# Ray0089/geometric-aware-dense-matching

Hardware: AMD Instinct MI355X
Metric: rgbd_crops_per_sec_geomatch_fwd (higher is better)
Workload: dtype bf16x3/f32acc

## Files before the change

### geometric_aware_dense_matching_amd/_lib.py

```python
import ctypes
import os
import subprocess

_PKG = os.path.dirname(os.path.abspath(__file__))
LIB_PATH = os.path.join(_PKG, "libgdm_hip.so")
CSRC = os.path.join(_PKG, "csrc")

_vp = ctypes.c_void_p
_i = ctypes.c_int
_f = ctypes.c_float
_sz = ctypes.c_size_t

GDM_RANSAC_MAX_H = 4096


class KnnJob(ctypes.Structure):
    _fields_ = [("support", _vp), ("query", _vp), ("idx", _vp), ("d2", _vp),
                ("support_bstride", ctypes.c_int64), ("query_bstride", ctypes.c_int64),
                ("S", ctypes.c_int32), ("Q", ctypes.c_int32), ("K", ctypes.c_int32), ("grid_w", ctypes.c_int32)]


class PwSeg(ctypes.Structure):
    _fields_ = [("x", _vp), ("idx", _vp), ("C", ctypes.c_int32), ("n_src", ctypes.c_int32)]


class PwJob(ctypes.Structure):
    _fields_ = [("x", _vp), ("wt", _vp), ("out", _vp), ("n", ctypes.c_int32)]


class CopyJob(ctypes.Structure):
    _fields_ = [("dst", _vp), ("src", _vp), ("sb", ctypes.c_int64), ("s1", ctypes.c_int64), ("s2", ctypes.c_int64),
                ("B", ctypes.c_int32), ("R1", ctypes.c_int32), ("R2", ctypes.c_int32), ("E", ctypes.c_int32)]


SIGNATURES = {
    "gdm_last_error": (ctypes.c_char_p, []),
    "gdm_version": (_i, []),
    "gdm_knn_batch": (None, [_vp, _sz, _sz, _sz, _vp, _sz, _sz, _vp]),
    "gdm_knn_batch_hip": (_i, [_vp, _vp, _i, _i, _i, _i, _vp, _vp, _vp]),
    "gdm_knn_jobs_workspace_bytes": (_sz, [ctypes.POINTER(KnnJob), _i, _i]),
    "gdm_knn_jobs_ws_hip": (_i, [ctypes.POINTER(KnnJob), _i, _i, _vp, _sz, _vp]),
    "gdm_ballquery_hip": (_i, [_i, _i, _i, _f, _i, _vp, _vp, _vp, _vp]),
    "gdm_furthestsampling_hip": (_i, [_i, _i, _i, _vp, _vp, _vp, _vp]),
    "gdm_interpolation_forward_hip": (_i, [_i, _i, _i, _i, _vp, _vp, _vp, _vp, _vp]),
    "gdm_interpolation_backward_hip": (_i, [_i, _i, _i, _i, _vp, _vp, _vp, _vp, _vp]),
    "gdm_labelstat_ballrange_hip": (_i, [_i, _i, _i, _f, _i, _vp, _vp, _vp, _vp, _vp]),
    "gdm_labelstat_idx_hip": (_i, [_i, _i, _i, _i, _i, _vp, _vp, _vp, _vp]),
    "gdm_group_gather_hip": (_i, [_vp, _vp, _i, _i, _i, _i, _i, _vp, _vp]),
    "gdm_group_gather_bwd2_hip": (_i, [_vp, ctypes.c_long, _vp, _i, _i, _i, _i, _i, _vp, _vp]),
    "gdm_gather_max_hip": (_i, [_vp, _vp, _i, _i, _i, _i, _i, _vp, _vp, _vp]),
    "gdm_gather_max_bwd_hip": (_i, [_vp, _vp, _i, _i, _i, _i, _vp, _vp]),
    "gdm_rel_pos_enc_hip": (_i, [_vp, _vp, _i, _i, _i, _vp, _vp]),
    "gdm_att_pool_hip": (_i, [_vp, _vp, _i, _i, _i, _i, _vp, _vp]),
    "gdm_att_pool_bwd_hip": (_i, [_vp, _vp, _vp, _i, _i, _i, _i, _vp, _vp, _vp]),
    "gdm_match_workspace_bytes": (_sz, [_i, _i, _i]),
    "gdm_match_hip": (_i, [_vp, _vp, _i, _i, _i, _i, _i, _vp, _vp, _vp, _vp, _sz, _vp]),
    "gdm_match_rows_bytes": (_sz, [_i]),
    "gdm_match_partial_bytes": (_sz, [_i, _i]),
    "gdm_match_pack_hip": (_i, [_vp, _i, _i, _i, _i, _vp, _vp]),
    "gdm_match_pack2_hip": (_i, [_vp, _i, _i, _vp, _vp, _i, _i, _vp, _i, _i, _vp]),
    "gdm_match_packed_hip": (_i, [_vp, _vp, _i, _i, _i, _vp, _vp, _vp, _vp, _sz, _vp]),
    "gdm_seg_mask_hip": (_i, [_vp, _i, _i, _vp, _vp, _vp]),
    "gdm_spline_aggregate_hip": (_i, [_vp, _vp, _vp, _vp, _vp, _vp, _i, _i, _i, _i, _vp, _vp]),
    "gdm_spline_aggregate_bwd_hip": (_i, [_vp, _vp, _vp, _vp, _i, _i, _i, _vp, _vp]),
    "gdm_spline_direct3_hip": (_i, [_vp, _vp, _vp, _vp, _vp, _vp, _vp, _i, _i, _i, _i, _i, _vp, _vp, _vp, _vp]),
    "gdm_gemm_grouped_hip": (_i, [_vp, _vp, _vp, _vp, _i, _i, _i, _i, _vp, _vp]),
    "gdm_spline_pairs_aggregate3_hip": (_i, [_vp, _vp, _vp, _vp, _vp, _vp, _i, _i, _i, _vp, _vp, _vp, _vp]),
    "gdm_upsample_bilinear_hip": (_i, [_vp, ctypes.c_long, _i, _i, _i, _i, _vp, _vp]),
    "gdm_upsample_bilinear_bwd_hip": (_i, [_vp, ctypes.c_long, _i, _i, _i, _i, _vp, _vp]),
    "gdm_topk_rows_hip": (_i, [_vp, ctypes.c_long, _i, _i, _vp, _vp, _vp]),
    "gdm_topk_negdist_hip": (_i, [_vp, _vp, _i, _i, _i, _vp, _vp]),
    "gdm_edge_feature_hip": (_i, [_vp, _vp, _i, _i, _i, _i, _vp, _vp]),
    "gdm_edge_feature_bwd_hip": (_i, [_vp, _vp, _i, _i, _i, _i, _vp, _vp]),
    "gdm_circle_rows_fwd_hip": (_i, [_vp, _i, _i, _vp, _vp, _vp, _vp, _f, _f, _f, _vp, _vp, _vp, _vp]),
    "gdm_circle_rows_bwd_hip": (_i, [_vp, _i, _i, _vp, _vp, _vp, _vp, _f, _f, _f, _vp, _vp, _vp, _vp, _vp]),
    "gdm_circle_match_rows_bytes": (_sz, [_i]),
    "gdm_circle_match_tp_bytes": (_sz, [_i]),
    "gdm_circle_match_pack_hip": (_i, [_vp, _i, _vp, _vp, _vp, _vp]),
    "gdm_circle_match_nbr_hip": (_i, [_vp, _i, _f, _vp, _vp]),
    "gdm_circle_match_visbits_hip": (_i, [_vp, _i, _i, _vp, _vp]),
    "gdm_circle_match_nbr_items_hip": (_i, [_vp, _i, _vp, _i, _vp, _vp]),
    "gdm_circle_match_fwd2_hip": (_i, [_vp, _vp, _vp, _vp, _vp, _i, _i, _vp, _vp, _vp, _vp, _i, _vp, _i, _f, _f, _vp, _vp, _vp, _vp]),
    "gdm_circle_match_bwd2_hip": (_i, [_vp, _vp, _vp, _vp, _vp, _i, _i, _vp, _vp, _vp, _vp, _i, _vp, _i, _f, _f, _vp, _vp, _vp, _vp, _vp, _vp]),
    "gdm_circle_match_bwd_parts": (_i, [_i, _i]),
    "gdm_lfa_stage_hip": (_i, [_vp] * 13 + [_i, _i, _i, _i, _i, _f, _vp, _vp]),
    "gdm_kabsch_stats_hip": (_i, [_vp, ctypes.c_long, _i, _i, _vp, _vp, _vp, _i, _i, _i, _vp, _vp]),
    "gdm_kabsch_solve_hip": (_i, [_vp, _i, _i, _vp, _vp, _vp]),
    "gdm_ransac_workspace_bytes": (_sz, [_i, _i, _i]),
    "gdm_ransac_pose_hip": (_i, [_vp, ctypes.c_long, _i, _i, _vp, _vp, _vp, _vp, _i, _i, _i, _i, _f, ctypes.c_double, ctypes.c_uint32, _i,
                                 _vp, _sz, _vp, _vp, _vp, _vp, _vp]),
    "gdm_icp_transform_hip": (_i, [_vp, ctypes.c_long, _i, _i, _vp, _i, _i, _vp, _vp]),
    "gdm_icp_update_hip": (_i, [_vp, ctypes.c_long, _i, _i, _vp, _vp, _vp, _vp, _i, _i, _i, _f, ctypes.c_double, _i, _vp, _vp, _vp, _vp,
                                _vp]),
    "gdm_targets_workspace_bytes": (_sz, [_i, _i, _i]),
    "gdm_hpr_visible_hip": (_i, [_vp, ctypes.c_long, _vp, _vp, _i, _i, _vp, _sz, _vp, _vp, _vp]),
    "gdm_pose_targets_hip": (_i, [_vp, ctypes.c_long, _i, _i, _vp, _vp, _vp, ctypes.c_long, _vp, _i, _i, _i, ctypes.c_double, _vp, _sz,
                                  _vp, _vp, _vp, _vp, _vp]),
    "gdm_affine_act_maxk_hip": (_i, [_vp, _vp, _vp, ctypes.c_long, _i, ctypes.c_long, _i, _i, _f, _vp, _vp]),
    "gdm_prelu1_hip": (_i, [_vp, _vp, ctypes.c_long, _vp, _vp]),
    "gdm_prelu1_bwd_hip": (_i, [_vp, _vp, _vp, ctypes.c_long, _vp, _vp, _vp]),
    "gdm_affine_act_hip": (_i, [_vp, _vp, _vp, _vp, _vp, _vp, ctypes.c_long, _i, ctypes.c_long, _i, _f, _vp, _vp]),
    "gdm_upconv3x3_gather_hip": (_i, [_vp, _vp, _vp, _i, _i, _i, _i, _i, _i, _i, _f, _vp, _vp]),
    "gdm_upconv3x3_gather2_hip": (_i, [_vp, _vp, _vp, _i, _i, _i, _i, _i, _i, _i, _f, _vp, _vp, _vp]),
    "gdm_upconv3x3_gather_bwd_hip": (_i, [_vp, _i, _i, _i, _i, _i, _i, _vp, _vp]),
    "gdm_upconv_fused64_weight_bytes": (_sz, []),
    "gdm_upconv_fused64_pack_weight_hip": (_i, [_vp, _vp, _vp]),
    "gdm_upconv_fused64_hip": (_i, [_vp, _vp, _vp, _vp, _i, _i, _i, _i, _i, _i, _i, _f, _vp, _vp]),
    "gdm_psp_combine2_hip": (_i, [_vp, _vp, _i, _vp, _i, _vp, _i, _vp, _i, _vp, _i, _i, _i, _i, _vp, _vp, _vp]),
    "gdm_gather_add_affine_act2_hip": (_i, [_vp, _vp, _vp, _vp, _vp, _i, _i, _i, _i, _i, _f, _vp, _vp, _i, _vp]),
    "gdm_conv1x1_gather_add_act2_hip": (_i, [_vp, _vp, _vp, _vp, _vp, _vp, _i, _i, _i, ctypes.c_long, _i, _f, _i, _vp, _vp]),
    "gdm_conv64_gather_add_act_mfma2_hip": (_i, [_vp, _vp, _vp, _vp, _vp, _vp, _i, _i, ctypes.c_long, _i, _f, _i, _i, _vp, _vp, _i, _vp]),
    "gdm_conv3x3_act_bytes": (_sz, [_i, _i, _i, _i]),
    "gdm_conv3x3_weight_bytes": (_sz, [_i, _i]),
    "gdm_conv3x3_pack_weight_hip": (_i, [_vp, _i, _i, _vp, _vp]),
    "gdm_conv3x3_pack_act_hip": (_i, [_vp, _i, _i, _i, _i, _vp, _vp]),
    "gdm_conv3x3_packed_hip": (_i, [_vp, _vp, _vp, _vp, _vp, _i, _i, _i, _i, _i, _i, _vp, _vp]),
    "gdm_conv3x3_strided_hip": (_i, [_vp, _vp, _vp, _vp, _vp, _i, _i, _i, _i, _i, _i, _i, _vp, _vp, _vp]),
    "gdm_conv1x1_strided_hip": (_i, [_vp, _vp, _vp, _vp, _i, _i, _i, _i, _i, _i, _i, _vp, _vp]),
    "gdm_affine_relu_maxpool_hip": (_i, [_vp, _vp, _vp, _i, _i, _i, _i, _vp, _vp]),
    "gdm_conv1x1_logsoftmax_hip": (_i, [_vp, _vp, _vp, _i, _i, ctypes.c_long, _vp, _vp]),
    "gdm_pack_rows64_hip": (_i, [_vp, _i, _vp, _vp]),
    "gdm_upconv_final_points_hip": (_i, [_vp, _vp, _vp, _vp, _vp, _i, _f, _vp, _vp, _i, _i, _i, _i, _i, _i, _vp, _vp]),
    "gdm_psp_pools_hip": (_i, [_vp, ctypes.c_long, _i, _i, _vp, _vp, _vp, _vp, _vp]),
    "gdm_psp_pools_bwd_hip": (_i, [_vp, _vp, _vp, _vp, ctypes.c_long, _i, _i, _vp, _vp]),
    "gdm_conv1x1_weight_bytes": (_sz, [_i, _i]),
    "gdm_conv1x1_pack_weight_hip": (_i, [_vp, _i, _i, _vp, _vp]),
    "gdm_conv_pack_weight_dgrad_hip": (_i, [_vp, _i, _i, _i, _vp, _vp]),
    "gdm_conv1x1_packed_hip": (_i, [_vp, _vp, _vp, _vp, _i, _i, _i, _i, _i, _i, _i, _vp, _vp]),
    "gdm_depth_to_xyz_hip": (_i, [_vp, _vp, _vp, _i, _i, _i, _i, _vp, _vp]),
    "gdm_bn_sums_len": (ctypes.c_long, [_i, _i, ctypes.c_long]),
    "gdm_bn_stats_hip": (_i, [_vp, _i, _i, ctypes.c_long, _vp, _vp]),
    "gdm_bn_fwd_apply_hip": (_i, [_vp, _vp, _i, _vp, _vp, _i, _i, ctypes.c_long, _f, _f, _i, _f, _vp, _vp, _vp, _vp, _vp]),
    "gdm_bn_bwd_reduce_hip": (_i, [_vp, _vp, _vp, _i, _i, ctypes.c_long, _i, _f, _vp, _vp]),
    "gdm_bn_bwd_apply_hip": (_i, [_vp, _vp, _vp, _i, _vp, _vp, _i, _i, ctypes.c_long, _i, _f, _vp, _vp, _vp, _vp]),
    "gdm_point_heads2_hip": (_i, [_vp, _vp, _i, _vp, _vp, _i, _i, _i, _i, _vp, _vp, _vp, _vp, _i, _i, _vp, _vp, _i, _vp, _vp, _vp]),
    "gdm_pointwise2_hip": (_i, [ctypes.POINTER(PwSeg), _i, _vp, _i, _vp, _vp, _i, _i, _i, _i, _f, _vp, _i, _i, _i, _vp]),
    "gdm_pointwise_jobs_hip": (_i, [ctypes.POINTER(PwJob), _i, _i, _i, _i, _vp]),
    "gdm_pointwise_chain2_hip": (_i, [_vp, _vp, _vp, _vp, _i, _f, _vp, _vp, _vp, _i, _f, _i, _i, _i, _i, _i, _vp, _vp, _vp]),
    "gdm_stem_weight_bytes": (_sz, []),
    "gdm_stem_pack_weight_hip": (_i, [_vp, _vp, _vp]),
    "gdm_stem_hip": (_i, [_vp, _vp, _vp, _vp, _i, _i, _i, _vp, _vp, _vp]),
    "gdm_wgrad_x_bytes": (_sz, [_i, _i, _i, _i]),
    "gdm_wgrad_go_bytes": (_sz, [_i, _i, _i, _i]),
    "gdm_wgrad_pack_x_hip": (_i, [_vp, _i, _i, _i, _i, _vp, _vp]),
    "gdm_wgrad_pack_go_hip": (_i, [_vp, _i, _i, _i, _i, _vp, _vp]),
    "gdm_wgrad_x1_bytes": (_sz, [_i, _i, _i]),
    "gdm_wgrad_pack_x1_hip": (_i, [_vp, _i, _i, _i, _vp, _vp]),
    "gdm_mfma_probe_hip": (_i, [_i, _i, _i, _vp, _vp]),
    "gdm_mfma_probe_lds_hip": (_i, [_i, _i, _i, _vp, _vp]),
    "gdm_wgrad_direct_hip": (_i, [_vp, ctypes.c_long, _vp, ctypes.c_long, _i, _i, _i, _i, _i, _vp, _vp, _vp]),
    "gdm_conv1x1_packed_wb_hip": (_i, [_vp, _vp, ctypes.c_long, _i, _i, _i, _i, _i, _vp, _vp]),
    "gdm_copy_jobs_hip": (_i, [ctypes.POINTER(CopyJob), _i, _vp]),
}

_lib = None


def _objects_state():
    st = {}
    for f in sorted(os.listdir(CSRC)):
        if f.endswith(".o"):
            st[f] = os.stat(os.path.join(CSRC, f)).st_mtime_ns
    return st


def build(verbose=False):
    import hashlib
    import json
    import time
    before = _objects_state()
    out = None if verbose else subprocess.DEVNULL
    t0 = time.time()
    subprocess.check_call(["make", "-C", CSRC, "-j4"], stdout=out)
    after = _objects_state()
    rebuilt = sorted(f for f, m in after.items() if before.get(f) != m)
    with open(LIB_PATH, "rb") as f:
        digest = hashlib.sha256(f.read()).hexdigest()[:16]
    rec = {"mode": "hipcc --offload-arch=gfx950 via csrc/Makefile (in-tree, ahead of time)", "recompiled": rebuilt,
           "up_to_date": sorted(set(after) - set(rebuilt)), "lib": os.path.basename(LIB_PATH), "lib_bytes": os.path.getsize(LIB_PATH),
           "lib_sha256_16": digest, "seconds": round(time.time() - t0, 1), "when": time.strftime("%Y-%m-%dT%H:%M:%S")}
    try:
        with open(os.path.join(CSRC, "build_record.json"), "w") as f:
            json.dump(rec, f, indent=1)
    except OSError:
        pass
    print("[gdm build] recompiled %d of %d translation units%s; %s %d bytes sha256 %s" %
          (len(rebuilt), len(after), (": " + " ".join(rebuilt)) if rebuilt else "", rec["lib"], rec["lib_bytes"], digest))
    return LIB_PATH


def build_record():
    import hashlib
    import json
    rec = {}
    try:
        with open(os.path.join(CSRC, "build_record.json")) as f:
            rec = json.load(f)
    except (OSError, ValueError):
        rec = {"mode": "prebuilt library (no build record travelled)"}
    try:
        with open(LIB_PATH, "rb") as f:
            rec["loaded_lib_sha256_16"] = hashlib.sha256(f.read()).hexdigest()[:16]
    except OSError:
        rec["loaded_lib_sha256_16"] = None
    rec.pop("up_to_date", None)
    if rec.get("lib_sha256_16") is not None:
        rec["record_matches_loaded_lib"] = rec["lib_sha256_16"] == rec["loaded_lib_sha256_16"]
    return rec


def lib():
    global _lib
    if _lib is None:
        if not os.path.exists(LIB_PATH):
            raise RuntimeError(
                "libgdm_hip.so is not built (%s). Run `python -c 'import __graft_entry__ as g; g.build()'` "
                "or `make -C geometric_aware_dense_matching_amd/csrc`. There is no CPU fallback." % LIB_PATH)
        import torch
        l = ctypes.CDLL(LIB_PATH)
        for name, (res, args) in SIGNATURES.items():
            fn = getattr(l, name)
            fn.restype = res
            fn.argtypes = args
        _lib = l
    return _lib


class GdmError(RuntimeError):
    pass


def check(rc, what):
    if rc != 0:
        msg = lib().gdm_last_error()
        raise GdmError("%s failed (rc=%d): %s" % (what, rc, msg.decode() if msg else "?"))
```

### geometric_aware_dense_matching_amd/cnn.py

```python
import math
import os

import torch
import torch.nn as nn
import torch.nn.functional as F

from . import ops, settings
from .layers import act_code, cached_gemm_weight, folded_bn, fused_eval




def bn_act(bn, x, relu=None):
    if ops.bn_train_supported(x, bn):
        return ops.batch_norm_act_train(x, bn, ops.ACT_RELU if relu is not None else ops.ACT_NONE)
    y = bn(x)
    return relu(y) if relu is not None else y


def _conv3x3(cin, cout, stride=1, dilation=1):
    return nn.Conv2d(cin, cout, kernel_size=3, stride=stride, padding=dilation, dilation=dilation, bias=False)


class BasicBlock(nn.Module):
    def __init__(self, inplanes, planes, stride=1, downsample=None, dilation=1):
        super().__init__()
        self.conv1 = _conv3x3(inplanes, planes, stride=stride, dilation=dilation)
        self.bn1 = nn.BatchNorm2d(planes)
        self.relu = nn.ReLU(inplace=True)
        self.conv2 = _conv3x3(planes, planes, stride=1, dilation=dilation)
        self.bn2 = nn.BatchNorm2d(planes)
        self.downsample = downsample

    @staticmethod
    def _packed_weight(conv):
        w = conv.weight
        key = (w._version, w.data_ptr())
        cache = conv.__dict__.get("_gdm_wpk")
        if cache is None or cache[0] != key:
            cache = (key, ops.conv3x3_pack_weight(w))
            conv.__dict__["_gdm_wpk"] = cache
        return cache[1]

    @staticmethod
    def _train_conv(conv, x):
        if (settings.USE_MFMA_CONV_TRAIN and conv.bias is None and tuple(conv.stride) == (1, 1)
                and ops.conv3x3_supported(x, conv.weight, conv.stride, conv.padding, conv.dilation)):
            return ops.conv3x3_train(x, conv.weight)
        return conv(x)

    def _mfma_ok(self, x):
        if tuple(self.conv1.stride) != (1, 1) and not settings.USE_MFMA_STRIDED:
            return False
        return (settings.USE_MFMA_CONV and ops.conv3x3_supported(x, self.conv1.weight, self.conv1.stride, self.conv1.padding, self.conv1.dilation)
                and ops.conv3x3_supported(x, self.conv2.weight, self.conv2.stride, self.conv2.padding, self.conv2.dilation)
                and self.conv2.weight.shape[1] == self.conv1.weight.shape[0])

    def forward(self, x):
        if fused_eval(x, self) and self._mfma_ok(x):
            s1, b1 = folded_bn(self.bn1)
            planes = self.conv1.weight.shape[0]
            stride = self.conv1.stride[0]
            xin = getattr(x, "_gdm_packed", None)
            if xin is None or xin.shape != tuple(x.shape):
                xin = x
            dconv = self.downsample[0] if self.downsample is not None else None
            own_ds = (settings.USE_MFMA_STRIDED and dconv is not None and isinstance(dconv, nn.Conv2d) and dconv.kernel_size == (1, 1) and dconv.bias is None
                      and dconv.stride == self.conv1.stride and dconv.padding == (0, 0)
                      and ops.gemm_supported(dconv.in_channels, dconv.out_channels, 64))
            if own_ds and not isinstance(xin, ops.PackedAct):
                xin = ops.conv3x3_pack_act(x)
            chain = (x.shape[0] * (x.shape[2] // stride) * (x.shape[3] // stride)) % 256 == 0
            mid = ops.conv3x3_bf16x3(xin, self._packed_weight(self.conv1), planes, s1, b1, ops.ACT_RELU, out_f32=not chain, out_packed=chain,
                                     stride=stride)
            mid = mid[1] if chain else mid
            s2, b2 = folded_bn(self.bn2)
            if self.downsample is None:
                res = x
            else:
                sd, bd = folded_bn(self.downsample[1])
                if own_ds:
                    wd, _ = cached_gemm_weight(dconv, "ds", lambda: dconv.weight.reshape(dconv.out_channels, dconv.in_channels), (dconv.weight,))
                    res = ops.conv1x1_packed2d(xin, wd, dconv.out_channels, sd, bd, ops.ACT_NONE, stride=stride)
                else:
                    res = ops.affine_act(dconv(x), sd, bd, ops.ACT_NONE)
            if not chain:
                return ops.conv3x3_bf16x3(mid, self._packed_weight(self.conv2), planes, s2, b2, ops.ACT_RELU, res)
            out, opk = ops.conv3x3_bf16x3(mid, self._packed_weight(self.conv2), planes, s2, b2, ops.ACT_RELU, res, out_packed=True)
            out._gdm_packed = opk
            return out
        if fused_eval(x, self):
            s1, b1 = folded_bn(self.bn1)
            out = ops.affine_act(self.conv1(x), s1, b1, ops.ACT_RELU)
            s2, b2 = folded_bn(self.bn2)
            if self.downsample is None:
                return ops.affine_act(self.conv2(out), s2, b2, ops.ACT_RELU, res=x)
            sd, bd = folded_bn(self.downsample[1])
            return ops.affine_act(self.conv2(out), s2, b2, ops.ACT_RELU, res=self.downsample[0](x), res_scale=sd, res_shift=bd)
        out = bn_act(self.bn1, self._train_conv(self.conv1, x), self.relu)
        out = bn_act(self.bn2, self._train_conv(self.conv2, out))
        residual = x if self.downsample is None else bn_act(self.downsample[1], self.downsample[0](x))
        out = out + residual
        return self.relu(out)


class ResNet18Trunk(nn.Module):
    def __init__(self):
        super().__init__()
        self.inplanes = 64
        self.conv1 = nn.Conv2d(3, 64, kernel_size=7, stride=2, padding=3, bias=False)
        self.bn1 = nn.BatchNorm2d(64)
        self.relu = nn.ReLU(inplace=True)
        self.maxpool = nn.MaxPool2d(kernel_size=3, stride=2, padding=1)
        self.layer1 = self._make_layer(64, 2, stride=1)
        self.layer2 = self._make_layer(128, 2, stride=2)
        self.layer3 = self._make_layer(256, 2, stride=1)
        self.layer4 = self._make_layer(512, 2, stride=1)
        self.fc = nn.Linear(512, 1000)
        for m in self.modules():
            if isinstance(m, nn.Conv2d):
                n = m.kernel_size[0] * m.kernel_size[1] * m.out_channels
                m.weight.data.normal_(0, math.sqrt(2.0 / n))
            elif isinstance(m, nn.BatchNorm2d):
                m.weight.data.fill_(1)
                m.bias.data.zero_()

    def _make_layer(self, planes, blocks, stride):
        downsample = None
        if stride != 1 or self.inplanes != planes:
            downsample = nn.Sequential(nn.Conv2d(self.inplanes, planes, kernel_size=1, stride=stride, bias=False),
                                       nn.BatchNorm2d(planes))
        layers = [BasicBlock(self.inplanes, planes, stride, downsample)]
        self.inplanes = planes
        for _ in range(1, blocks):
            layers.append(BasicBlock(self.inplanes, planes))
        return nn.Sequential(*layers)


class PSPModule(nn.Module):
    def __init__(self, features, out_features=1024, sizes=(1, 2, 3, 6)):
        super().__init__()
        self.stages = nn.ModuleList([nn.Sequential(nn.AdaptiveAvgPool2d(output_size=(s, s)),
                                                   nn.Conv2d(features, features, kernel_size=1, bias=False))
                                     for s in sizes])
        self.bottleneck = nn.Conv2d(features * (len(sizes) + 1), out_features, kernel_size=1)
        self.relu = nn.ReLU()

    def _split_weights(self):
        w = self.bottleneck.weight
        vs = [st[1].weight for st in self.stages]
        key = tuple((t._version, t.data_ptr()) for t in [w] + vs)
        cache = self.__dict__.get("_gdm_split")
        if cache is None or cache[0] != key:
            with torch.no_grad():
                F_ = vs[0].shape[0]
                w2 = w.view(w.shape[0], -1)
                ms = [(w2[:, k * F_:(k + 1) * F_] @ v.view(F_, F_)).contiguous() for k, v in enumerate(vs)]
                wf = w2[:, len(vs) * F_:].contiguous()
            cache = (key, ms, wf)
            self.__dict__["_gdm_split"] = cache
        return cache[1], cache[2]

    def _split_weights_t(self, ms):
        cache = self.__dict__.get("_gdm_split_t")
        if cache is None or cache[0] is not ms:
            with torch.no_grad():
                cache = (ms, [m.t().contiguous() for m in ms])
            self.__dict__["_gdm_split_t"] = cache
        return cache[1]

    def forward(self, feats):
        h, w = feats.size(2), feats.size(3)
        if fused_eval(feats, self) and len(self.stages) == 4 and feats.shape[0] * self.bottleneck.out_channels <= 65535:
            ms, wf = self._split_weights()
            B, Cin = feats.shape[0], feats.shape[1]
            def full_res():
                if settings.USE_MFMA_GEMM and ops.gemm_supported(Cin, wf.shape[0], h * w):
                    wpk, co = cached_gemm_weight(self, "wf", wf, (self.bottleneck.weight,))
                    return ops.gemm_bf16x3_map(feats, wpk, co)
                return ops.wx(wf, feats.reshape(B, Cin, h * w)).view(B, -1, h, w)

            def priors():
                sizes = [st[0].output_size[0] if isinstance(st[0].output_size, (tuple, list)) else st[0].output_size for st in self.stages]
                pools = ops.psp_pools(feats) if sizes == [1, 2, 3, 6] and ops.psp_pools_supported(h, w) else None
                ys = []
                mts = self._split_weights_t(ms) if settings.USE_POINTWISE else None
                if mts is not None and pools is not None and settings.USE_PSP_JOBS and Cin >= 32:
                    outs = ops.pointwise_jobs([p.reshape(B, Cin, -1) for p in pools], mts)
                    return [o.view(B, -1, p.shape[2], p.shape[3]) for o, p in zip(outs, pools)]
                for k, (st, m) in enumerate(zip(self.stages, ms)):
                    p = pools[k] if pools is not None else st[0](feats)
                    s_ = p.shape[2]
                    if mts is not None:
                        ys.append(ops.pointwise([p.reshape(B, Cin, s_ * s_)], mts[k]).view(B, -1, s_, s_))
                    else:
                        ys.append(ops.wx(m, p.reshape(B, Cin, s_ * s_)).view(B, -1, s_, s_))
                return ys

            if settings.USE_SIDE_STREAMS and "psp" in settings.SIDE_PARTS and not torch.is_grad_enabled():
                with ops.fork(feats.device, 3) as f:
                    f.use(feats)
                    ys = priors()
                g = full_res()
                f.join(*ys)
            else:
                g = full_res()
                ys = priors()
            return ops.psp_combine(g, ys, self.bottleneck.bias, packed=settings.USE_MFMA_GEMM and settings.USE_PACKED_PRODUCERS)
        sizes = [st[0].output_size[0] if isinstance(st[0].output_size, (tuple, list)) else st[0].output_size for st in self.stages]
        if (settings.USE_SPLIT_PSP_TRAIN and feats.is_cuda and feats.dtype == torch.float32 and sizes == [1, 2, 3, 6] and ops.psp_pools_supported(h, w)
                and (h * w) % 4 == 0 and feats.shape[0] * self.bottleneck.out_channels <= 65535 and h <= 64 and w <= 64):
            B, F_ = feats.shape[0], feats.shape[1]
            w2 = self.bottleneck.weight.view(self.bottleneck.out_channels, -1)
            g = ops.wx(w2[:, 4 * F_:], feats.reshape(B, F_, h * w)).view(B, -1, h, w)
            pools = ops.psp_pools(feats)
            ys = []
            for k, st in enumerate(self.stages):
                m = w2[:, k * F_:(k + 1) * F_] @ st[1].weight.view(F_, F_)
                ys.append(ops.wx(m, pools[k].reshape(B, F_, sizes[k] * sizes[k])).view(B, -1, sizes[k], sizes[k]))
            return ops.psp_combine_train(g, ys, self.bottleneck.bias)
        priors = [ops.upsample_bilinear(stage(feats), (h, w)) for stage in self.stages] + [feats]
        return self.relu(self.bottleneck(torch.cat(priors, 1)))


class Upsample2x(nn.Module):

    def forward(self, x):
        return ops.upsample_bilinear(x, (x.shape[2] * 2, x.shape[3] * 2))


class PSPUpsample(nn.Module):
    def __init__(self, cin, cout):
        super().__init__()
        self.conv = nn.Sequential(Upsample2x(), nn.Conv2d(cin, cout, 3, padding=1), nn.BatchNorm2d(cout), nn.PReLU())

    def _tap_major_weight(self):
        w = self.conv[1].weight
        key = (w._version, w.data_ptr())
        cache = self.__dict__.get("_gdm_wt")
        if cache is None or cache[0] != key:
            with torch.no_grad():
                wt = w.permute(2, 3, 0, 1).reshape(9 * w.shape[0], w.shape[1]).contiguous()
            cache = (key, wt)
            self.__dict__["_gdm_wt"] = cache
        return cache[1]

    def forward(self, x):
        if fused_eval(x, self):
            code = act_code(self.conv[3])
            conv = self.conv[1]
            if code is not None and x.shape[0] * conv.out_channels <= 65535 and conv.in_channels >= settings.UPCONV_MIN_CIN:
                Bx, Cin, Hx, Wx = x.shape
                if settings.USE_FUSED_UPCONV and Cin == 64 and conv.out_channels == 64 and Hx >= 2 and Wx >= 2 and Bx <= 65535:
                    w = conv.weight
                    key = (w._version, w.data_ptr())
                    cache = self.__dict__.get("_gdm_fused64")
                    if cache is None or cache[0] != key:
                        cache = (key, ops.upconv_fused64_pack_weight(w))
                        self.__dict__["_gdm_fused64"] = cache
                    scale, shift = folded_bn(self.conv[2], conv.bias)
                    return ops.upconv_fused64(x, cache[1], scale, shift, (Hx * 2, Wx * 2), code[0], code[1])
                if settings.USE_MFMA_GEMM and ops.gemm_supported(Cin, 9 * conv.out_channels, Hx * Wx):
                    wpk, c9 = cached_gemm_weight(self, "tap", self._tap_major_weight, (conv.weight,))
                    z = ops.gemm_bf16x3_map(x, wpk, c9)
                else:
                    z = ops.wx(self._tap_major_weight(), x.reshape(Bx, Cin, Hx * Wx)).view(Bx, -1, Hx, Wx)
                scale, shift = folded_bn(self.conv[2], conv.bias)
                return ops.upconv3x3_gather(z, scale, shift, conv.out_channels, (x.shape[2] * 2, x.shape[3] * 2), code[0], code[1],
                                            packed=settings.USE_MFMA_GEMM and settings.USE_PACKED_PRODUCERS and conv.out_channels % 128 == 0)
        act = self.conv[3]
        if x.is_cuda and isinstance(act, nn.PReLU) and act.weight.numel() == 1 and x.dtype == torch.float32:
            conv = self.conv[1]
            if settings.USE_LOWRES_UPCONV_TRAIN and ops.upconv_train_supported(x.shape[0], conv.out_channels) and conv.in_channels >= settings.UPCONV_MIN_CIN:
                Bx, Cin, Hx, Wx = x.shape
                w9 = conv.weight.permute(2, 3, 0, 1).reshape(9 * conv.out_channels, Cin)
                z = ops.wx(w9, x.reshape(Bx, Cin, Hx * Wx)).view(Bx, -1, Hx, Wx)
                y = bn_act(self.conv[2], ops.upconv3x3_gather_train(z, conv.bias, conv.out_channels, (Hx * 2, Wx * 2)))
            else:
                y = bn_act(self.conv[2], conv(self.conv[0](x)))
            if y.numel() % 4 == 0:
                return ops.prelu1(y, act.weight)
            return act(y)
        return self.conv(x)


class FinalStage(nn.Sequential):

    def forward(self, x):
        conv = self[0]
        if fused_eval(x, self) and conv.in_channels == 64 and conv.out_channels == 64 and x.shape[0] <= 65535:
            return ops.conv1x1_logsoftmax(x, conv.weight, conv.bias)
        if self.training and ops.conv1x1_train_supported(conv, x):
            return self[1](ops.conv1x1_train(conv, x))
        return nn.Sequential.forward(self, x)


class PSPNet(nn.Module):

    def __init__(self):
        super().__init__()
        self.feats = ResNet18Trunk()
        self.psp = PSPModule(512, 1024, (1, 2, 3, 6))
        self.drop_1 = nn.Dropout2d(p=0.3)
        self.up_1 = PSPUpsample(1024, 256)
        self.up_2 = PSPUpsample(256, 64)
        self.up_3 = PSPUpsample(64, 64)
        self.drop_2 = nn.Dropout2d(p=0.15)
        self.final = FinalStage(nn.Conv2d(64, 64, kernel_size=1), nn.LogSoftmax(dim=1))
```

### geometric_aware_dense_matching_amd/csrc/gdm_conv.hip

```cpp
#include "gdm_common.h"
#include <math.h>
#include <stdlib.h>

namespace {

typedef __attribute__((ext_vector_type(16))) float f32x16;
typedef __attribute__((ext_vector_type(8))) __bf16 bf16x8;
typedef __attribute__((ext_vector_type(4))) unsigned u32x4;

constexpr int ROWB = 512;
constexpr int CV_PIX = 256;
constexpr int CV_CO = 128;
constexpr int CV_PANEL = CV_CO * ROWB;
#ifndef GDM_CONV_TAP_INNER
#define GDM_CONV_TAP_INNER 1
#endif
#ifndef GDM_CONV16_PF
#define GDM_CONV16_PF 2
#endif
#ifndef GDM_CONV_GLDS
#define GDM_CONV_GLDS 1
#endif

__device__ __forceinline__ void split8(const float* v, unsigned (&hi)[4], unsigned (&lo)[4])
{
#pragma unroll
    for (int j = 0; j < 4; ++j) gdm_split2(v[2 * j], v[2 * j + 1], hi[j], lo[j]);
}

__global__ __launch_bounds__(256) void conv_pack_act_kernel(const float* __restrict__ x, int C, int H, int W,
                                                            unsigned char* __restrict__ out)
{
    __shared__ float t[128][65];
    const int b = blockIdx.z, chunk = blockIdx.y;
    const int nchunk = (C + 127) / 128;
    const int cvalid = min(128, C - chunk * 128);
    const int hw = H * W;
    const long plane = (long)(H + 2) * (W + 2);
    const int p0 = blockIdx.x * 64;
    const int lane = threadIdx.x & 63, w = threadIdx.x >> 6;
    const int p = min(p0 + lane, hw - 1);
    const float* xb = x + ((long)b * C + chunk * 128) * hw;
    for (int c = w; c < cvalid; c += 4) t[c][lane] = xb[(long)c * hw + p];
    __syncthreads();
    const int pp = p0 + lane;
    if (pp >= hw) return;
    const int y = pp / W, xx = pp - y * W;
    unsigned char* o = out + (((long)(b * nchunk + chunk) * 32) * plane + (long)(y + 1) * (W + 2) + xx + 1) * 16;
    for (int q = w; q * 8 < cvalid; q += 4) {
        float v[8];
#pragma unroll
        for (int j = 0; j < 8; ++j) v[j] = t[q * 8 + j][lane];
        unsigned hi[4], lo[4];
        split8(v, hi, lo);
        *reinterpret_cast<uint4*>(o + (long)q * plane * 16) = make_uint4(hi[0], hi[1], hi[2], hi[3]);
        *reinterpret_cast<uint4*>(o + (long)(16 + q) * plane * 16) = make_uint4(lo[0], lo[1], lo[2], lo[3]);
    }
}

__global__ __launch_bounds__(256) void conv_pack_w_kernel(const float* __restrict__ w, int Cout, int Cin, int taps, unsigned char* __restrict__ out,
                                                          int dgrad = 0)
{
    const int nchunk = (Cin + 127) / 128;
    const int CoutP = (Cout + 127) & ~127;
    const long item = (long)blockIdx.x * 256 + threadIdx.x;
    const long rows = (long)taps * nchunk * CoutP;
    if (item >= rows * 16) return;
    const int ch = (int)(item & 15);
    const long row = item >> 4;
    const int co = (int)(row % CoutP);
    const int tc = (int)(row / CoutP);
    const int chunk = tc % nchunk, tap = tc / nchunk;
    float v[8];
#pragma unroll
    for (int j = 0; j < 8; ++j) {
        const int ci = chunk * 128 + ch * 8 + j;
        const bool in = co < Cout && ci < Cin;
        v[j] = !in ? 0.f : dgrad ? w[((long)ci * Cout + co) * taps + (taps - 1 - tap)] : w[((long)co * Cin + ci) * taps + tap];
    }
    unsigned hi[4], lo[4];
    split8(v, hi, lo);
    unsigned char* r = out + row * ROWB;
    *reinterpret_cast<uint4*>(r + ch * 16) = make_uint4(hi[0], hi[1], hi[2], hi[3]);
    *reinterpret_cast<uint4*>(r + 256 + ch * 16) = make_uint4(lo[0], lo[1], lo[2], lo[3]);
}

__device__ __forceinline__ int swz(int col, int ch) { return col * ROWB + (((ch & 16) | ((ch ^ col) & 15)) << 4); }

typedef __attribute__((ext_vector_type(4))) float f32x4;

#ifndef GDM_CONV_NPH
#define GDM_CONV_NPH 2
#endif
#ifndef GDM_CONV16_LATE
#define GDM_CONV16_LATE 1
#endif
#ifndef GDM_CONV_MFMA_ORDER
#define GDM_CONV_MFMA_ORDER 0
#endif
constexpr int MF_NPH = GDM_CONV_NPH;
constexpr int MF_WPIX = 16 * MF_NPH;
constexpr int MF_WAVES = CV_PIX / MF_WPIX;
constexpr int MF_THREADS = MF_WAVES * 64;
constexpr int MF_TSTRIDE = 132;
constexpr int MF_SMEM = 2 * CV_PANEL > CV_PIX * MF_TSTRIDE * 4 ? 2 * CV_PANEL : CV_PIX * MF_TSTRIDE * 4;

template <int ACT, bool HAS_RES, int TAPS = 9, bool PIXMAJOR = false, int NKS = 8, int NCB = 8, int WV = MF_WAVES>
__global__ __launch_bounds__(MF_THREADS) void conv_mfma16_kernel(const unsigned char* __restrict__ xpk, const unsigned char* __restrict__ wpk,
                                                                 const float* __restrict__ scale, const float* __restrict__ shift,
                                                                 const float* __restrict__ res, int B, int Cin, int Cout, int H, int W,
                                                                 float* __restrict__ out, const int32_t* __restrict__ rowidx = nullptr,
                                                                 const int32_t* __restrict__ tile_co0 = nullptr,
                                                                 unsigned char* __restrict__ outpk = nullptr, int stride = 1,
                                                                 long wbstride = 0)
{
    extern __shared__ __attribute__((aligned(16))) unsigned char smem[];
    constexpr int NS = NKS / 2;
    constexpr int UG = (NCB % 2 == 0) ? 2 : 3;
    constexpr int NPR = NCB / UG;
    constexpr int PANEL = NCB * 16 * ROWB;
    constexpr int TST = NCB * 16 + 4;
    static_assert(NCB == 8 || (NCB == 4 && !PIXMAJOR) || (NCB == 9 && !PIXMAJOR && WV == 8),
                  "64-channel tiles: NCHW / packed output only; 144-channel tiles: NCHW fp32 output only (no packed output: a tile straddles 128-channel chunks)");
    constexpr int NPH = MF_NPH;
    const int tid = threadIdx.x, lane = tid & 63;
    const int wave = __builtin_amdgcn_readfirstlane(tid >> 6);
    const int l16 = lane & 15, kg = lane >> 4;
    const int nchunk = (Cin + 127) / 128;
    const int npanel = TAPS * nchunk;
    const int hw = H * W;
    const long ptot = rowidx ? (long)B : (long)B * hw;
    const unsigned bx = blockIdx.x, by = blockIdx.y;
    const long pix0 = (long)bx * (WV * MF_WPIX) + wave * MF_WPIX;
    const int co0 = tile_co0 ? __builtin_amdgcn_readfirstlane(tile_co0[bx]) : by * (NCB * 16);
    const long pc = min(pix0, ptot - MF_WPIX);
    const int b = (int)(pc / hw);
    const int prem = (int)(pc - (long)b * hw);
    const int Wi = W * stride;
    const long plane = (long)(H * stride + 2) * (Wi + 2);
    const long oplane = (long)(H + 2) * (W + 2);
    const __amdgpu_buffer_rsrc_t xr = __builtin_amdgcn_make_buffer_rsrc(const_cast<unsigned char*>(xpk), (short)0, 0x7ffffff0, 0x00020000);
    int avoff[NPH];
#pragma unroll
    for (int ph = 0; ph < NPH; ++ph) {
        const int pr = prem + 16 * ph;
        const int yy = pr / W, xx = pr - yy * W;
        const long pixbase = rowidx ? (long)max(rowidx[pc + l16 + 16 * ph], 0) : (long)(yy * stride) * (Wi + 2) + (long)(xx + l16) * stride;
        avoff[ph] = (int)(((long)kg * plane + pixbase) * 16);
    }

    u32x4 ahi[NS][NPH], alo[NS][NPH];
    struct Pan { int chunk, ky, kx; };
    auto pan_next = [&](Pan p) -> Pan {
        if (TAPS == 1) { ++p.chunk; return p; }
        if (GDM_CONV_TAP_INNER) {
            if (++p.kx == 3) { p.kx = 0; if (++p.ky == 3) { p.ky = 0; ++p.chunk; } }
        } else {
            if (++p.chunk == nchunk) { p.chunk = 0; if (++p.kx == 3) { p.kx = 0; ++p.ky; } }
        }
        return p;
    };
    const int a_base = (int)(((long)(rowidx ? 0 : b) * nchunk * 32) * plane * 16);
    const int a_chunk = (int)(32 * plane * 16), a_rowb = (Wi + 2) * 16;
    auto pan_a = [&](Pan p) -> int { return a_base + p.chunk * a_chunk + p.ky * a_rowb + p.kx * 16; };
    const int sstride = (int)(4 * plane * 16);
    const int lostride = (int)(16 * plane * 16);
    auto load_a = [&](int r, int S) {
#pragma unroll
        for (int ph = 0; ph < NPH; ++ph) {
            ahi[S][ph] = __builtin_bit_cast(u32x4, __builtin_amdgcn_raw_buffer_load_b128(xr, avoff[ph], r + S * sstride, 0));
            alo[S][ph] = __builtin_bit_cast(u32x4, __builtin_amdgcn_raw_buffer_load_b128(xr, avoff[ph], r + S * sstride + lostride, 0));
        }
    };
    constexpr int THREADS = WV * 64, WGPIX = WV * MF_WPIX;
    constexpr int HS = (NCB * 512 / THREADS) / 2;
    u32x4 stage[HS];
    const __amdgpu_buffer_rsrc_t wr = __builtin_amdgcn_make_buffer_rsrc(const_cast<unsigned char*>(wpk), (short)0, 0x7ffffff0, 0x00020000);
    const int w_base = (wbstride ? (int)(((long)bx * WGPIX / hw) * wbstride) : 0) + co0 * ROWB;
    const int w_panel = ((Cout + 127) & ~127) * ROWB;
    auto pan_w = [&](Pan p) -> int { return w_base + ((TAPS == 1) ? p.chunk : (p.ky * 3 + p.kx) * nchunk + p.chunk) * w_panel; };
    auto stage_load = [&](int src, int half) {
#pragma unroll
        for (int i = 0; i < HS; ++i)
            stage[i] = __builtin_bit_cast(u32x4, __builtin_amdgcn_raw_buffer_load_b128(wr, tid * 16, src + (half * HS + i) * THREADS * 16, 0));
    };
    auto stage_store = [&](int buf, int half) {
        unsigned char* base = smem + buf * PANEL;
#pragma unroll
        for (int i = 0; i < HS; ++i) {
            const int g = (half * HS + i) * THREADS + tid;
            *reinterpret_cast<u32x4*>(base + swz(g >> 5, g & 31)) = stage[i];
        }
    };
    constexpr bool GLDS = GDM_CONV_GLDS && WV == 8;
    constexpr int NPIECE = PANEL / 1024 / 8;
    int glds_voff = 0;
    if (GLDS) {
        const int hrow = lane >> 5, sl = lane & 31;
        const int col15 = (2 * wave + hrow) & 15;
        glds_voff = wave * 1024 + hrow * 512 + (((sl & 16) | ((sl ^ col15) & 15)) << 4);
    }
    typedef __attribute__((address_space(3))) void* lds_void_ptr;
    auto stage_glds = [&](int src, int buf) {
#pragma unroll
        for (int i = 0; i < NPIECE; ++i)
            __builtin_amdgcn_raw_ptr_buffer_load_lds(wr, (lds_void_ptr)(smem + buf * PANEL + (i * 8 + wave) * 1024), 16, glds_voff, src + i * 8192, 0, 0);
    };

    f32x4 acc[NPH][NCB];
#pragma unroll
    for (int ph = 0; ph < NPH; ++ph)
#pragma unroll
        for (int cb = 0; cb < NCB; ++cb)
#pragma unroll
            for (int i = 0; i < 4; ++i) acc[ph][cb][i] = 0.f;

    constexpr int LATE = GDM_CONV16_LATE < NS ? GDM_CONV16_LATE : NS;
    Pan pcur = {0, (TAPS == 1) ? 1 : 0, (TAPS == 1) ? 1 : 0};
    if (GLDS) {
        stage_glds(pan_w(pcur), 0);
    } else {
        stage_load(pan_w(pcur), 0);
        stage_store(0, 0);
        stage_load(pan_w(pcur), 1);
        stage_store(0, 1);
    }
    int rcur = pan_a(pcur);
#pragma unroll
    for (int S = 0; S < NS - LATE; ++S) load_a(rcur, S);
    Pan pnxt = npanel > 1 ? pan_next(pcur) : pcur;
    int rnext = pan_a(pnxt), wnext = pan_w(pnxt);
    for (int it = 0; it < npanel; ++it) {
        __syncthreads();
        const bool more = it + 1 < npanel;
        const unsigned char* base = smem + (it & 1) * PANEL;
        constexpr int PF = GDM_CONV16_PF;
        constexpr int NU = NPR * NS;
        u32x4 fh[PF + 1][UG], fl[PF + 1][UG];
        auto frag_load = [&](int un) {
            const int S = un / NPR, pr = un % NPR, slot = un % (PF + 1);
#pragma unroll
            for (int j = 0; j < UG; ++j) {
                const int col = (UG * pr + j) * 16 + l16;
                fh[slot][j] = *reinterpret_cast<const u32x4*>(base + swz(col, 4 * S + kg));
                fl[slot][j] = *reinterpret_cast<const u32x4*>(base + swz(col, 16 + 4 * S + kg));
            }
        };
#pragma unroll
        for (int un = 0; un < PF; ++un) frag_load(un);
#pragma unroll
        for (int u = 0; u < NU; ++u) {
            const int S = u / NPR, pr = u % NPR, slot = u % (PF + 1);
            if (u + PF < NU) frag_load(u + PF);
#if GDM_CONV_MFMA_ORDER == 0
#pragma unroll
            for (int ph = 0; ph < NPH; ++ph) {
                const bf16x8 ah = __builtin_bit_cast(bf16x8, ahi[S][ph]);
                const bf16x8 al = __builtin_bit_cast(bf16x8, alo[S][ph]);
#pragma unroll
                for (int j = 0; j < UG; ++j) {
                    f32x4 c = acc[ph][UG * pr + j];
                    c = __builtin_amdgcn_mfma_f32_16x16x32_bf16(ah, __builtin_bit_cast(bf16x8, fl[slot][j]), c, 0, 0, 0);
                    c = __builtin_amdgcn_mfma_f32_16x16x32_bf16(al, __builtin_bit_cast(bf16x8, fh[slot][j]), c, 0, 0, 0);
                    c = __builtin_amdgcn_mfma_f32_16x16x32_bf16(ah, __builtin_bit_cast(bf16x8, fh[slot][j]), c, 0, 0, 0);
                    acc[ph][UG * pr + j] = c;
                }
            }
#else
#pragma unroll
            for (int prod = 0; prod < 3; ++prod)
#pragma unroll
                for (int ph = 0; ph < NPH; ++ph)
#pragma unroll
                    for (int j = 0; j < UG; ++j) {
                        const bf16x8 av = __builtin_bit_cast(bf16x8, prod == 1 ? alo[S][ph] : ahi[S][ph]);
                        const bf16x8 bv = __builtin_bit_cast(bf16x8, prod == 0 ? fl[slot][j] : fh[slot][j]);
                        acc[ph][UG * pr + j] = __builtin_amdgcn_mfma_f32_16x16x32_bf16(av, bv, acc[ph][UG * pr + j], 0, 0, 0);
                    }
#endif
            if (pr == NPR - 1 && S < NS - LATE) load_a(rnext, S);
            if (!GLDS && u == NU / 2 && more) {
                stage_store((it + 1) & 1, 0);
                stage_load(wnext, 1);
            }
            if (u == 0) {
                if (more) { if (GLDS) stage_glds(wnext, (it + 1) & 1); else stage_load(wnext, 0); }
#pragma unroll
                for (int S2 = NS - LATE; S2 < NS; ++S2) load_a(rcur, S2);
            }
#pragma unroll
            for (int i = 0; i < 3 * UG * NPH; ++i) {
                __builtin_amdgcn_sched_group_barrier(0x008, 1, 0);
                if (u + PF < NU && (i % NPH) == 0 && i < 2 * UG * NPH) __builtin_amdgcn_sched_group_barrier(0x100, 1, 0);
            }
            __builtin_amdgcn_sched_barrier(0);
        }
        if (!GLDS && more) stage_store((it + 1) & 1, 1);
        rcur = rnext;
        if (it + 2 < npanel) pnxt = pan_next(pnxt);
        rnext = pan_a(pnxt);
        wnext = pan_w(pnxt);
    }

    if (pix0 >= ptot) return;
    if (PIXMAJOR) {
#pragma unroll
        for (int cb = 0; cb < NCB; ++cb) {
            const int co = co0 + cb * 16 + l16;
            if (co >= Cout) continue;
            const float sc = scale ? scale[co] : 1.f, sh = shift ? shift[co] : 0.f;
            const int ocol = tile_co0 ? cb * 16 + l16 : co;
            const int ostride = tile_co0 ? CV_CO : Cout;
#pragma unroll
            for (int ph = 0; ph < NPH; ++ph)
#pragma unroll
                for (int r = 0; r < 4; ++r) {
                    float v = acc[ph][cb][r] * sc + sh;
                    if (ACT == 1) v = fmaxf(v, 0.f);
                    out[(pix0 + 16 * ph + 4 * kg + r) * ostride + ocol] = v;
                }
        }
        return;
    }
    float* tl = reinterpret_cast<float*>(smem) + wave * MF_WPIX * TST;
    if (outpk) __syncthreads();
#pragma unroll
    for (int cb = 0; cb < NCB; ++cb) {
        const int co = co0 + cb * 16 + l16;
        const bool live = co < Cout;
        const float sc = (live && scale) ? scale[co] : 1.f, sh = (live && shift) ? shift[co] : 0.f;
        float* op = out ? out + ((long)b * Cout + (live ? co : 0)) * hw + prem : nullptr;
        const float* rp = (HAS_RES && live) ? res + ((long)b * Cout + co) * hw + prem : nullptr;
#pragma unroll
        for (int ph = 0; ph < NPH; ++ph) {
            const int poff = 16 * ph + 4 * kg;
            float v[4];
#pragma unroll
            for (int j = 0; j < 4; ++j) v[j] = acc[ph][cb][j] * sc + sh;
            if (HAS_RES && live) {
                const float4 r4 = *reinterpret_cast<const float4*>(rp + poff);
                v[0] += r4.x; v[1] += r4.y; v[2] += r4.z; v[3] += r4.w;
            }
            if (ACT == 1) {
#pragma unroll
                for (int j = 0; j < 4; ++j) v[j] = fmaxf(v[j], 0.f);
            }
            if (op && live) *reinterpret_cast<float4*>(op + poff) = make_float4(v[0], v[1], v[2], v[3]);
            if (outpk) {
#pragma unroll
                for (int j = 0; j < 4; ++j) tl[(poff + j) * TST + cb * 16 + l16] = live ? v[j] : 0.f;
            }
        }
    }
    if (outpk) {
        __builtin_amdgcn_fence(__ATOMIC_ACQ_REL, "wavefront");
        const int lr = lane & 31, h = lane >> 5;
        const int ochunks = (Cout + 127) / 128;
        const int ochunk = co0 / 128;
#pragma unroll
        for (int half = 0; half < MF_WPIX / 32; ++half) {
            const int pp = prem + 32 * half + lr;
            const int yy = pp / W, xx = pp - yy * W;
            unsigned char* ob = outpk + (((long)(b * ochunks + ochunk) * 32) * oplane + (long)(yy + 1) * (W + 2) + xx + 1) * 16;
            const float* row = tl + (32 * half + lr) * TST;
#pragma unroll
            for (int it = 0; it < NCB; ++it) {
                const int ql = 2 * it + h;
                if (co0 + ql * 8 >= Cout) continue;
                const int q = (co0 % 128) / 8 + ql;
                const float4 a0 = *reinterpret_cast<const float4*>(row + ql * 8);
                const float4 a1 = *reinterpret_cast<const float4*>(row + ql * 8 + 4);
                const float v[8] = {a0.x, a0.y, a0.z, a0.w, a1.x, a1.y, a1.z, a1.w};
                unsigned hi[4], lo[4];
                split8(v, hi, lo);
                *reinterpret_cast<uint4*>(ob + (long)q * oplane * 16) = make_uint4(hi[0], hi[1], hi[2], hi[3]);
                *reinterpret_cast<uint4*>(ob + (long)(16 + q) * oplane * 16) = make_uint4(lo[0], lo[1], lo[2], lo[3]);
            }
        }
    }
}

#define CONV_KERNEL conv_mfma16_kernel
constexpr int CONV_THREADS = MF_THREADS, CONV_WPIX = MF_WPIX, CONV_SMEM = MF_SMEM;

}

namespace {
template <int CHAIN>
__global__ __launch_bounds__(512) void mfma_probe_kernel(int iters, float* __restrict__ sink)
{
    typedef __attribute__((ext_vector_type(8))) __bf16 pb_bf16x8;
    typedef __attribute__((ext_vector_type(4))) float pb_f32x4;
    const int lane = threadIdx.x & 63;
    pb_f32x4 acc[8];
#pragma unroll
    for (int i = 0; i < 8; ++i) acc[i] = pb_f32x4{0.f, 0.f, 0.f, 0.f};
    const unsigned seed = 0x3f803f80u + (unsigned)lane;
    u32x4 av = {seed, seed ^ 1u, seed ^ 2u, seed ^ 3u}, bv = {seed ^ 4u, seed ^ 5u, seed ^ 6u, seed ^ 7u};
    const pb_bf16x8 a = __builtin_bit_cast(pb_bf16x8, av), b = __builtin_bit_cast(pb_bf16x8, bv);
    for (int it = 0; it < iters; it += CHAIN) {
#pragma unroll
        for (int i = 0; i < 8; ++i)
#pragma unroll
            for (int c = 0; c < CHAIN; ++c) acc[i] = __builtin_amdgcn_mfma_f32_16x16x32_bf16(a, b, acc[i], 0, 0, 0);
    }
    float t = 0.f;
#pragma unroll
    for (int i = 0; i < 8; ++i) t += acc[i][0] + acc[i][1] + acc[i][2] + acc[i][3];
    if (t == 12345.678f) sink[0] = t;
}
template <int RPU>
__global__ __launch_bounds__(512) void mfma_probe_lds_kernel(int iters, float* __restrict__ sink)
{
    typedef __attribute__((ext_vector_type(8))) __bf16 pb_bf16x8;
    typedef __attribute__((ext_vector_type(4))) float pb_f32x4;
    extern __shared__ __attribute__((aligned(16))) unsigned char pl[];
    const int tid = threadIdx.x, lane = tid & 63;
    for (int i = tid; i < 4096; i += 512) reinterpret_cast<u32x4*>(pl)[i] = u32x4{0x3f803f80u, 0x3f803f80u, 0x3f803f80u, 0x3f803f80u + (unsigned)i};
    __syncthreads();
    pb_f32x4 acc[4];
#pragma unroll
    for (int i = 0; i < 4; ++i) acc[i] = pb_f32x4{0.f, 0.f, 0.f, 0.f};
    const unsigned seed = 0x3f803f80u + (unsigned)lane;
    u32x4 a0 = {seed, seed ^ 1u, seed ^ 2u, seed ^ 3u}, a1 = {seed ^ 4u, seed ^ 5u, seed ^ 6u, seed ^ 7u};
    u32x4 f[4] = {a0, a1, a0, a1};
    int off = lane * 16;
    for (int it = 0; it < iters; ++it) {
#pragma unroll
        for (int r = 0; r < RPU; ++r) f[r] = *reinterpret_cast<const u32x4*>(pl + ((off + r * 1024) & 0xffff));
        off += 4096;
#pragma unroll
        for (int prod = 0; prod < 3; ++prod)
#pragma unroll
            for (int i = 0; i < 4; ++i)
                acc[i] = __builtin_amdgcn_mfma_f32_16x16x32_bf16(__builtin_bit_cast(pb_bf16x8, prod == 1 ? a1 : a0),
                                                                 __builtin_bit_cast(pb_bf16x8, f[(i + prod) & 3]), acc[i], 0, 0, 0);
    }
    float t = 0.f;
#pragma unroll
    for (int i = 0; i < 4; ++i) t += acc[i][0] + acc[i][1] + acc[i][2] + acc[i][3];
    if (t == 12345.678f) sink[0] = t;
}
}

extern "C" int gdm_mfma_probe_lds_hip(int blocks, int iters, int rpu, float* sink, void* stream)
{
    GDM_CHECK_ARG(blocks >= 1 && blocks <= 65535 && iters >= 1 && (rpu == 1 || rpu == 2 || rpu == 4) && sink, "gdm_mfma_probe_lds_hip: bad arguments");
    if (rpu == 4) hipLaunchKernelGGL(mfma_probe_lds_kernel<4>, dim3(blocks), dim3(512), 65536, (hipStream_t)stream, iters, sink);
    else if (rpu == 2) hipLaunchKernelGGL(mfma_probe_lds_kernel<2>, dim3(blocks), dim3(512), 65536, (hipStream_t)stream, iters, sink);
    else hipLaunchKernelGGL(mfma_probe_lds_kernel<1>, dim3(blocks), dim3(512), 65536, (hipStream_t)stream, iters, sink);
    return gdm_launch_status("mfma_probe_lds_kernel");
}

extern "C" int gdm_mfma_probe_hip(int blocks, int iters, int chain, float* sink, void* stream)
{
    GDM_CHECK_ARG(blocks >= 1 && blocks <= 65535 && iters >= 3 && iters % 3 == 0 && (chain == 1 || chain == 3) && sink,
                  "gdm_mfma_probe_hip: bad arguments (iters a multiple of 3, chain 1 or 3)");
    if (chain == 3) hipLaunchKernelGGL(mfma_probe_kernel<3>, dim3(blocks), dim3(512), 0, (hipStream_t)stream, iters, sink);
    else hipLaunchKernelGGL(mfma_probe_kernel<1>, dim3(blocks), dim3(512), 0, (hipStream_t)stream, iters, sink);
    return gdm_launch_status("mfma_probe_kernel");
}

static bool cin_ok(int Cin) { return Cin == 64 || (Cin >= 128 && Cin % 128 == 0); }

static bool narrow_tiles(unsigned pixel_tiles, int Cout)
{
    return Cout <= 64 || (long)pixel_tiles * ((Cout + 127) / 128) < 256;
}

extern "C" size_t gdm_conv3x3_act_bytes(int B, int Cin, int H, int W)
{
    if (B < 1 || !cin_ok(Cin) || H < 1 || W < 1) return 0;
    return (size_t)B * (H + 2) * (W + 2) * ((Cin + 127) / 128) * ROWB;
}

extern "C" size_t gdm_conv3x3_weight_bytes(int Cout, int Cin)
{
    if (Cout < 1 || !cin_ok(Cin)) return 0;
    return (size_t)9 * ((Cin + 127) / 128) * ((Cout + 127) & ~127) * ROWB;
}

extern "C" size_t gdm_conv1x1_weight_bytes(int Cout, int Cin)
{
    if (Cout < 1 || !cin_ok(Cin)) return 0;
    return (size_t)((Cin + 127) / 128) * ((Cout + 127) & ~127) * ROWB;
}

static int pack_weight(const float* w, int Cout, int Cin, int taps, void* wpk, void* stream, const char* who, int dgrad = 0)
{
    GDM_CHECK_ARG(w && wpk, "%s: NULL pointer", who);
    GDM_CHECK_ARG(Cout >= 1 && cin_ok(Cin), "%s: Cout=%d Cin=%d (Cin a multiple of 128, or 64)", who, Cout, Cin);
    const long items = (long)taps * ((Cin + 127) / 128) * ((Cout + 127) & ~127) * 16;
    hipLaunchKernelGGL(conv_pack_w_kernel, dim3(gdm_cdiv(items, 256)), dim3(256), 0, (hipStream_t)stream, w, Cout, Cin, taps, (unsigned char*)wpk, dgrad);
    return gdm_launch_status("conv_pack_w_kernel");
}

extern "C" int gdm_conv_pack_weight_dgrad_hip(const float* w, int Cout, int Cin, int taps, void* wpk, void* stream)
{
    GDM_CHECK_ARG(taps == 9 || taps == 1, "gdm_conv_pack_weight_dgrad_hip: taps=%d (9 or 1)", taps);
    return pack_weight(w, Cin, Cout, taps, wpk, stream, "gdm_conv_pack_weight_dgrad_hip", 1);
}

extern "C" int gdm_conv3x3_pack_weight_hip(const float* w, int Cout, int Cin, void* wpk, void* stream)
{
    return pack_weight(w, Cout, Cin, 9, wpk, stream, "gdm_conv3x3_pack_weight_hip");
}

extern "C" int gdm_conv1x1_pack_weight_hip(const float* w, int Cout, int Cin, void* wpk, void* stream)
{
    return pack_weight(w, Cout, Cin, 1, wpk, stream, "gdm_conv1x1_pack_weight_hip");
}

extern "C" int gdm_conv3x3_pack_act_hip(const float* x, int B, int Cin, int H, int W, void* xpk, void* stream)
{
    GDM_CHECK_ARG(x && xpk, "gdm_conv3x3_pack_act_hip: NULL pointer");
    GDM_CHECK_ARG(B >= 1 && B <= 65535 && cin_ok(Cin) && H >= 1 && W >= 1, "gdm_conv3x3_pack_act_hip: bad shape (Cin=%d: a multiple of 128, or 64)", Cin);
    dim3 grid(gdm_cdiv((long)H * W, 64), (Cin + 127) / 128, B);
    hipLaunchKernelGGL(conv_pack_act_kernel, grid, dim3(256), 0, (hipStream_t)stream, x, Cin, H, W, (unsigned char*)xpk);
    return gdm_launch_status("conv_pack_act_kernel");
}

static int conv3x3_launch(const void* xpk, const void* wpk, const float* scale, const float* shift, const float* res,
                          int B, int Cin, int Cout, int H, int W, int stride, int act, float* out, void* outpk, void* stream,
                          const char* who);

extern "C" int gdm_conv3x3_packed_hip(const void* xpk, const void* wpk, const float* scale, const float* shift, const float* res,
                                      int B, int Cin, int Cout, int H, int W, int act, float* out, void* stream)
{
    return conv3x3_launch(xpk, wpk, scale, shift, res, B, Cin, Cout, H, W, 1, act, out, nullptr, stream, "gdm_conv3x3_packed_hip");
}

extern "C" int gdm_conv3x3_strided_hip(const void* xpk, const void* wpk, const float* scale, const float* shift, const float* res,
                                       int B, int Cin, int Cout, int H, int W, int stride, int act, float* out, void* outpk, void* stream)
{
    return conv3x3_launch(xpk, wpk, scale, shift, res, B, Cin, Cout, H, W, stride, act, out, outpk, stream, "gdm_conv3x3_strided_hip");
}

static int conv3x3_launch(const void* xpk, const void* wpk, const float* scale, const float* shift, const float* res,
                          int B, int Cin, int Cout, int H, int W, int stride, int act, float* out, void* outpk, void* stream,
                          const char* who)
{
    GDM_CHECK_ARG(stride == 1 || stride == 2, "%s: stride=%d (1 or 2)", who, stride);
    GDM_CHECK_ARG(xpk && wpk && (out || outpk), "%s: NULL pointer", who);
    GDM_CHECK_ARG(B >= 1 && cin_ok(Cin) && Cout >= 1, "%s: Cin=%d Cout=%d (Cin a multiple of 128, or 64)", who, Cin, Cout);
    GDM_CHECK_ARG(W % 32 == 0 && H >= 1 && (H * W) % CONV_WPIX == 0,
                  "%s: W=%d must be a multiple of 32 and H*W=%d of %d", who, W, H * W, CONV_WPIX);
    GDM_CHECK_ARG(act == 0 || act == 1, "%s: act=%d", who, act);
    GDM_CHECK_ARG(!outpk || (Cout % 8 == 0 && ((long)B * H * W) % CV_PIX == 0),
                  "%s: packed output needs Cout %% 8 == 0 and B*H*W %% 256 == 0 (got Cout=%d, B*H*W=%ld)", who, Cout, (long)B * H * W);
    const long ptot = (long)B * H * W;
    dim3 grid(gdm_cdiv(ptot, CV_PIX), gdm_cdiv(Cout, CV_CO));
    hipStream_t s = (hipStream_t)stream;
    constexpr int SMEM = CONV_SMEM;
    static bool attr = false;
    if (!attr) {
        (void)hipFuncSetAttribute((const void*)CONV_KERNEL<0, false>, hipFuncAttributeMaxDynamicSharedMemorySize, SMEM);
        (void)hipFuncSetAttribute((const void*)CONV_KERNEL<1, false>, hipFuncAttributeMaxDynamicSharedMemorySize, SMEM);
        (void)hipFuncSetAttribute((const void*)CONV_KERNEL<0, true>, hipFuncAttributeMaxDynamicSharedMemorySize, SMEM);
        (void)hipFuncSetAttribute((const void*)CONV_KERNEL<1, true>, hipFuncAttributeMaxDynamicSharedMemorySize, SMEM);
        (void)hipFuncSetAttribute((const void*)CONV_KERNEL<0, false, 9, false, 4>, hipFuncAttributeMaxDynamicSharedMemorySize, SMEM);
        (void)hipFuncSetAttribute((const void*)CONV_KERNEL<1, false, 9, false, 4>, hipFuncAttributeMaxDynamicSharedMemorySize, SMEM);
        (void)hipFuncSetAttribute((const void*)CONV_KERNEL<0, true, 9, false, 4>, hipFuncAttributeMaxDynamicSharedMemorySize, SMEM);
        (void)hipFuncSetAttribute((const void*)CONV_KERNEL<1, true, 9, false, 4>, hipFuncAttributeMaxDynamicSharedMemorySize, SMEM);
        attr = true;
    }
#define CV(A, R, NK) hipLaunchKernelGGL((CONV_KERNEL<A, R, 9, false, NK>), grid, dim3(CONV_THREADS), SMEM, s, (const unsigned char*)xpk, (const unsigned char*)wpk, scale, shift, res, B, Cin, Cout, H, W, out, (const int32_t*)nullptr, (const int32_t*)nullptr, (unsigned char*)outpk, stride)
    if (narrow_tiles(grid.x, Cout)) {
        constexpr int SMEM4 = 2 * 64 * ROWB > CV_PIX * 68 * 4 ? 2 * 64 * ROWB : CV_PIX * 68 * 4;
        const dim3 grid4(grid.x, gdm_cdiv(Cout, 64));
        static bool attr4 = false;
#define CV4(A, R, NK) hipLaunchKernelGGL((CONV_KERNEL<A, R, 9, false, NK, 4>), grid4, dim3(CONV_THREADS), SMEM4, s, (const unsigned char*)xpk, (const unsigned char*)wpk, scale, shift, res, B, Cin, Cout, H, W, out, (const int32_t*)nullptr, (const int32_t*)nullptr, (unsigned char*)outpk, stride)
#define AT4(A, R, NK) (void)hipFuncSetAttribute((const void*)CONV_KERNEL<A, R, 9, false, NK, 4>, hipFuncAttributeMaxDynamicSharedMemorySize, SMEM4)
        if (!attr4) {
            AT4(0, false, 4); AT4(1, false, 4); AT4(0, true, 4); AT4(1, true, 4);
            AT4(0, false, 8); AT4(1, false, 8); AT4(0, true, 8); AT4(1, true, 8);
            attr4 = true;
        }
        if (Cin != 64 && (long)grid4.x * grid4.y < 256 && ptot % (CV_PIX / 2) == 0) {
            const dim3 grid4h(gdm_cdiv(ptot, CV_PIX / 2), grid4.y);
            static bool attr4h = false;
#define CV4H(A, R) hipLaunchKernelGGL((CONV_KERNEL<A, R, 9, false, 8, 4, MF_WAVES / 2>), grid4h, dim3(CONV_THREADS / 2), SMEM4, s, (const unsigned char*)xpk, (const unsigned char*)wpk, scale, shift, res, B, Cin, Cout, H, W, out, (const int32_t*)nullptr, (const int32_t*)nullptr, (unsigned char*)outpk, stride)
#define AT4H(A, R) (void)hipFuncSetAttribute((const void*)CONV_KERNEL<A, R, 9, false, 8, 4, MF_WAVES / 2>, hipFuncAttributeMaxDynamicSharedMemorySize, SMEM4)
            if (!attr4h) {
                AT4H(0, false); AT4H(1, false); AT4H(0, true); AT4H(1, true);
                attr4h = true;
            }
            if (act == 0) { if (res) CV4H(0, true); else CV4H(0, false); }
            else { if (res) CV4H(1, true); else CV4H(1, false); }
#undef CV4H
#undef AT4H
            return gdm_launch_status("conv_mfma16_kernel (3x3, 64-channel tiles, 128 pixels)");
        }
        if (Cin == 64) {
            if (act == 0) { if (res) CV4(0, true, 4); else CV4(0, false, 4); }
            else { if (res) CV4(1, true, 4); else CV4(1, false, 4); }
        } else {
            if (act == 0) { if (res) CV4(0, true, 8); else CV4(0, false, 8); }
            else { if (res) CV4(1, true, 8); else CV4(1, false, 8); }
        }
#undef CV4
#undef AT4
        return gdm_launch_status("conv_mfma16_kernel (3x3, 64-channel tiles)");
    }
    if (Cin == 64) {
        if (act == 0) { if (res) CV(0, true, 4); else CV(0, false, 4); }
        else { if (res) CV(1, true, 4); else CV(1, false, 4); }
    } else {
        if (act == 0) { if (res) CV(0, true, 8); else CV(0, false, 8); }
        else { if (res) CV(1, true, 8); else CV(1, false, 8); }
    }
#undef CV
    return gdm_launch_status("conv_mfma16_kernel (3x3)");
}

extern "C" int gdm_gemm_grouped_hip(const void* xpk, const void* wpk, const int32_t* rowidx, const int32_t* tile_co0, int R, int M,
                                    int Cin, int Cout_total, float* out, void* stream)
{
    GDM_CHECK_ARG(xpk && wpk && rowidx && tile_co0 && out, "gdm_gemm_grouped_hip: NULL pointer");
    GDM_CHECK_ARG(R >= 256 && R % 256 == 0 && M >= 1 && Cin >= 128 && Cin % 128 == 0 && Cout_total >= 128 && Cout_total % 128 == 0,
                  "gdm_gemm_grouped_hip: R=%d (multiple of 256) M=%d Cin=%d Cout_total=%d (multiples of 128)", R, M, Cin, Cout_total);
    static bool attr = false;
    if (!attr) {
        (void)hipFuncSetAttribute((const void*)CONV_KERNEL<0, false, 1, true>, hipFuncAttributeMaxDynamicSharedMemorySize, 2 * CV_PANEL);
        attr = true;
    }
    hipLaunchKernelGGL((CONV_KERNEL<0, false, 1, true>), dim3(R / CV_PIX, 1), dim3(CONV_THREADS), 2 * CV_PANEL, (hipStream_t)stream,
                       (const unsigned char*)xpk, (const unsigned char*)wpk, (const float*)nullptr, (const float*)nullptr, (const float*)nullptr,
                       R, Cin, Cout_total, 1, M, out, rowidx, tile_co0);
    return gdm_launch_status("gemm_grouped_kernel");
}

static int conv1x1_launch(const void* xpk, const void* wpk, const float* scale, const float* shift,
                          int B, int Cin, int Cout, int H, int W, int stride, int act, int pixel_major, float* out, void* stream,
                          const char* who);

extern "C" int gdm_conv1x1_packed_hip(const void* xpk, const void* wpk, const float* scale, const float* shift,
                                      int B, int Cin, int Cout, int H, int W, int act, int pixel_major, float* out, void* stream)
{
    return conv1x1_launch(xpk, wpk, scale, shift, B, Cin, Cout, H, W, 1, act, pixel_major, out, stream, "gdm_conv1x1_packed_hip");
}

extern "C" int gdm_conv1x1_packed_wb_hip(const void* xpk, const void* wpk, long w_bstride, int B, int Cin, int Cout, int H, int W, float* out,
                                         void* stream)
{
    GDM_CHECK_ARG(xpk && wpk && out, "gdm_conv1x1_packed_wb_hip: NULL pointer");
    GDM_CHECK_ARG(B >= 1 && Cin >= 128 && Cin % 128 == 0 && Cout >= 1, "gdm_conv1x1_packed_wb_hip: Cin=%d Cout=%d (Cin a multiple of 128)", Cin, Cout);
    GDM_CHECK_ARG(W % 32 == 0 && H >= 1 && (H * W) % CV_PIX == 0, "gdm_conv1x1_packed_wb_hip: W=%d must be a multiple of 32 and H*W=%d of %d",
                  W, H * W, CV_PIX);
    GDM_CHECK_ARG(w_bstride >= 0 && w_bstride % 16 == 0, "gdm_conv1x1_packed_wb_hip: w_bstride=%ld", w_bstride);
    const long ptot = (long)B * H * W;
    dim3 grid(gdm_cdiv(ptot, CV_PIX), gdm_cdiv(Cout, CV_CO));
    static bool attr = false;
    if (!attr) {
        (void)hipFuncSetAttribute((const void*)CONV_KERNEL<0, false, 1, false>, hipFuncAttributeMaxDynamicSharedMemorySize, 2 * CV_PANEL);
        attr = true;
    }
    hipLaunchKernelGGL((CONV_KERNEL<0, false, 1, false>), grid, dim3(CONV_THREADS), 2 * CV_PANEL, (hipStream_t)stream, (const unsigned char*)xpk,
                       (const unsigned char*)wpk, (const float*)nullptr, (const float*)nullptr, (const float*)nullptr, B, Cin, Cout, H, W, out,
                       (const int32_t*)nullptr, (const int32_t*)nullptr, (unsigned char*)nullptr, 1, w_bstride);
    return gdm_launch_status("conv1x1_bf16x3_kernel (per-image weights)");
}

extern "C" int gdm_conv1x1_strided_hip(const void* xpk, const void* wpk, const float* scale, const float* shift,
                                       int B, int Cin, int Cout, int H, int W, int stride, int act, float* out, void* stream)
{
    return conv1x1_launch(xpk, wpk, scale, shift, B, Cin, Cout, H, W, stride, act, 0, out, stream, "gdm_conv1x1_strided_hip");
}

static int conv1x1_launch(const void* xpk, const void* wpk, const float* scale, const float* shift,
                          int B, int Cin, int Cout, int H, int W, int stride, int act, int pixel_major, float* out, void* stream,
                          const char* who)
{
    GDM_CHECK_ARG(stride == 1 || stride == 2, "%s: stride=%d (1 or 2)", who, stride);
    GDM_CHECK_ARG(xpk && wpk && out, "%s: NULL pointer", who);
    GDM_CHECK_ARG(B >= 1 && cin_ok(Cin) && Cout >= 1, "%s: Cin=%d Cout=%d (Cin a multiple of 128, or 64)", who, Cin, Cout);
    GDM_CHECK_ARG(Cin != 64 || !pixel_major, "%s: Cin=64 is built for the NCHW output only", who);
    GDM_CHECK_ARG(W % 32 == 0 && H >= 1 && (H * W) % CONV_WPIX == 0,
                  "%s: W=%d must be a multiple of 32 and H*W=%d of %d", who, W, H * W, CONV_WPIX);
    GDM_CHECK_ARG(act == 0 || act == 1, "%s: act=%d", who, act);
    const long ptot = (long)B * H * W;
    const unsigned ptiles = gdm_cdiv(ptot, CV_PIX);
    if (Cin != 64 && !pixel_major && stride == 1 && Cout % 144 == 0 && GDM_CONV_GLDS) {
        const long r128 = gdm_cdiv((long)ptiles * gdm_cdiv(Cout, 128), 256) * 128, r144 = gdm_cdiv((long)ptiles * (Cout / 144), 256) * 144;
        if (r144 < r128) {
            constexpr int PANEL9 = 9 * 16 * ROWB, TILE9 = CV_PIX * (9 * 16 + 4) * 4;
            constexpr int SMEM9 = 2 * PANEL9 > TILE9 ? 2 * PANEL9 : TILE9;
            static bool attr9 = false;
            if (!attr9) {
                (void)hipFuncSetAttribute((const void*)CONV_KERNEL<0, false, 1, false, 8, 9>, hipFuncAttributeMaxDynamicSharedMemorySize, SMEM9);
                (void)hipFuncSetAttribute((const void*)CONV_KERNEL<1, false, 1, false, 8, 9>, hipFuncAttributeMaxDynamicSharedMemorySize, SMEM9);
                attr9 = true;
            }
            const dim3 grid9(ptiles, Cout / 144);
#define C19(A) hipLaunchKernelGGL((CONV_KERNEL<A, false, 1, false, 8, 9>), grid9, dim3(CONV_THREADS), SMEM9, (hipStream_t)stream, (const unsigned char*)xpk, (const unsigned char*)wpk, scale, shift, (const float*)nullptr, B, Cin, Cout, H, W, out, (const int32_t*)nullptr, (const int32_t*)nullptr, (unsigned char*)nullptr, stride)
            if (act == 0) C19(0); else C19(1);
#undef C19
            return gdm_launch_status("conv1x1_bf16x3_kernel (144-channel tiles)");
        }
    }
    const bool narrow = Cin != 64 && !pixel_major && narrow_tiles(ptiles, Cout);
    const unsigned ctiles = gdm_cdiv(Cout, narrow ? 64 : CV_CO);
    const dim3 grid(ptiles, ctiles);
    hipStream_t s = (hipStream_t)stream;
    static bool attr = false;
    if (!attr) {
        (void)hipFuncSetAttribute((const void*)CONV_KERNEL<0, false, 1, false>, hipFuncAttributeMaxDynamicSharedMemorySize, 2 * CV_PANEL);
        (void)hipFuncSetAttribute((const void*)CONV_KERNEL<1, false, 1, false>, hipFuncAttributeMaxDynamicSharedMemorySize, 2 * CV_PANEL);
        (void)hipFuncSetAttribute((const void*)CONV_KERNEL<0, false, 1, true>, hipFuncAttributeMaxDynamicSharedMemorySize, 2 * CV_PANEL);
        (void)hipFuncSetAttribute((const void*)CONV_KERNEL<1, false, 1, true>, hipFuncAttributeMaxDynamicSharedMemorySize, 2 * CV_PANEL);
        (void)hipFuncSetAttribute((const void*)CONV_KERNEL<0, false, 1, false, 4>, hipFuncAttributeMaxDynamicSharedMemorySize, 2 * CV_PANEL);
        (void)hipFuncSetAttribute((const void*)CONV_KERNEL<1, false, 1, false, 4>, hipFuncAttributeMaxDynamicSharedMemorySize, 2 * CV_PANEL);
        attr = true;
    }
    if (Cin == 64) {
#define C1TAIL , (const int32_t*)nullptr, (const int32_t*)nullptr, (unsigned char*)nullptr, stride
#define C1H(A) hipLaunchKernelGGL((CONV_KERNEL<A, false, 1, false, 4>), grid, dim3(CONV_THREADS), 2 * CV_PANEL, s, (const unsigned char*)xpk, (const unsigned char*)wpk, scale, shift, (const float*)nullptr, B, Cin, Cout, H, W, out C1TAIL)
        if (act == 0) C1H(0); else C1H(1);
#undef C1H
        return gdm_launch_status("conv1x1_bf16x3_kernel");
    }
    if (narrow) {
        const dim3 grid4 = grid;
        static bool attr4 = false;
        if (!attr4) {
            (void)hipFuncSetAttribute((const void*)CONV_KERNEL<0, false, 1, false, 8, 4>, hipFuncAttributeMaxDynamicSharedMemorySize, 2 * 64 * ROWB);
            (void)hipFuncSetAttribute((const void*)CONV_KERNEL<1, false, 1, false, 8, 4>, hipFuncAttributeMaxDynamicSharedMemorySize, 2 * 64 * ROWB);
            attr4 = true;
        }
#define C14(A) hipLaunchKernelGGL((CONV_KERNEL<A, false, 1, false, 8, 4>), grid4, dim3(CONV_THREADS), 2 * 64 * ROWB, s, (const unsigned char*)xpk, (const unsigned char*)wpk, scale, shift, (const float*)nullptr, B, Cin, Cout, H, W, out C1TAIL)
        if (act == 0) C14(0); else C14(1);
#undef C14
        return gdm_launch_status("conv1x1_bf16x3_kernel (64-channel tiles)");
    }
#define C1(A, P) hipLaunchKernelGGL((CONV_KERNEL<A, false, 1, P>), grid, dim3(CONV_THREADS), 2 * CV_PANEL, s, (const unsigned char*)xpk, (const unsigned char*)wpk, scale, shift, (const float*)nullptr, B, Cin, Cout, H, W, out C1TAIL)
    if (act == 0) { if (pixel_major) C1(0, true); else C1(0, false); }
    else { if (pixel_major) C1(1, true); else C1(1, false); }
#undef C1
    return gdm_launch_status("conv1x1_bf16x3_kernel");
}
```

### geometric_aware_dense_matching_amd/ffb6d.py

```python
import torch
import torch.nn as nn

from . import ops, settings
from .cnn import PSPNet, bn_act
from .layers import act_code, cached_gemm_weight, folded_bn, fused_eval, pt_conv2d, rl_conv1d, rl_conv2d
from .randla import DilatedResBlock


class FFB6DEmb(nn.Module):
    def __init__(self, cfg):
        super().__init__()
        cnn = PSPNet()
        d_outs = list(cfg.d_out)
        n_layers = cfg.num_layers

        self.cnn_pre_stages = nn.Sequential(cnn.feats.conv1, cnn.feats.bn1, cnn.feats.relu, cnn.feats.maxpool)
        self.rndla_pre_stages = rl_conv1d(cfg.in_c, 8, bn=True)

        self.cnn_ds_stages = nn.ModuleList([
            cnn.feats.layer1,
            cnn.feats.layer2,
            nn.Sequential(cnn.feats.layer3, cnn.feats.layer4),
            nn.Sequential(cnn.psp, cnn.drop_1),
        ])
        self.ds_sr = [4, 8, 8, 8]

        blocks = nn.ModuleList()
        d_in = 8
        for i in range(n_layers):
            blocks.append(DilatedResBlock(d_in, d_outs[i]))
            d_in = 2 * d_outs[i]
        self.rndla_ds_stages = blocks

        self.ds_rgb_oc = [64, 128, 512, 1024]
        self.ds_rndla_oc = [c * 2 for c in d_outs]
        self.ds_fuse_r2p_pre_layers = nn.ModuleList()
        self.ds_fuse_r2p_fuse_layers = nn.ModuleList()
        self.ds_fuse_p2r_pre_layers = nn.ModuleList()
        self.ds_fuse_p2r_fuse_layers = nn.ModuleList()
        for i in range(4):
            self.ds_fuse_r2p_pre_layers.append(pt_conv2d(self.ds_rgb_oc[i], self.ds_rndla_oc[i], bn=True))
            self.ds_fuse_r2p_fuse_layers.append(pt_conv2d(self.ds_rndla_oc[i] * 2, self.ds_rndla_oc[i], bn=True))
            self.ds_fuse_p2r_pre_layers.append(pt_conv2d(self.ds_rndla_oc[i], self.ds_rgb_oc[i], bn=True))
            self.ds_fuse_p2r_fuse_layers.append(pt_conv2d(self.ds_rgb_oc[i] * 2, self.ds_rgb_oc[i], bn=True))

        self.cnn_up_stages = nn.ModuleList([
            nn.Sequential(cnn.up_1, cnn.drop_2),
            nn.Sequential(cnn.up_2, cnn.drop_2),
            nn.Sequential(cnn.final),
            nn.Sequential(cnn.up_3, cnn.final),
        ])
        self.up_rgb_oc = [256, 64, 64]
        self.up_rndla_oc = []
        for j in range(n_layers):
            self.up_rndla_oc.append(self.ds_rndla_oc[-j - 2] if j < 3 else self.ds_rndla_oc[0])

        dec = nn.ModuleList()
        d_out = 2 * d_outs[-1]
        for j in range(n_layers):
            if j < 3:
                d_in = d_out + 2 * d_outs[-j - 2]
                d_out = 2 * d_outs[-j - 2]
            else:
                d_in = 4 * d_outs[-4]
                d_out = 2 * d_outs[-4]
            dec.append(rl_conv2d(d_in, d_out, bn=True))
        self.rndla_up_stages = dec

        self.up_fuse_r2p_pre_layers = nn.ModuleList()
        self.up_fuse_r2p_fuse_layers = nn.ModuleList()
        self.up_fuse_p2r_pre_layers = nn.ModuleList()
        self.up_fuse_p2r_fuse_layers = nn.ModuleList()
        for i in range(3):
            self.up_fuse_r2p_pre_layers.append(pt_conv2d(self.up_rgb_oc[i], self.up_rndla_oc[i], bn=True))
            self.up_fuse_r2p_fuse_layers.append(pt_conv2d(self.up_rndla_oc[i] * 2, self.up_rndla_oc[i], bn=True))
            self.up_fuse_p2r_pre_layers.append(pt_conv2d(self.up_rndla_oc[i], self.up_rgb_oc[i], bn=True))
            self.up_fuse_p2r_fuse_layers.append(pt_conv2d(self.up_rgb_oc[i] * 2, self.up_rgb_oc[i], bn=True))

    @staticmethod
    def random_sample(feature, pool_idx):
        return ops.gather_max(feature, pool_idx).unsqueeze(3)

    @staticmethod
    def nearest_interpolation(feature, interp_idx):
        return ops.gather_nn(feature, interp_idx).unsqueeze(3)

    @staticmethod
    def _split_fuse_weight(layer, c_first):
        w = layer.conv.weight
        key = (w._version, w.data_ptr(), c_first)
        cache = layer.__dict__.get("_gdm_split")
        if cache is None or cache[0] != key:
            with torch.no_grad():
                w2 = w.view(w.shape[0], -1)
                cache = (key, w2[:, :c_first].contiguous(), w2[:, c_first:].contiguous())
            layer.__dict__["_gdm_split"] = cache
        return cache[1], cache[2]

    @staticmethod
    def _fuse_weight_t(layer, wa, tag="a"):
        slot = "_gdm_w%s_t" % tag
        cache = layer.__dict__.get(slot)
        if cache is None or cache[0] is not wa:
            cache = (wa, wa.t().contiguous())
            layer.__dict__[slot] = cache
        return cache[1]

    def _p2r_point_term(self, pre_layer, fuse_layer, c, p_emb0):
        if not fused_eval(p_emb0, self) or act_code(getattr(fuse_layer, "activation", None)) is None or not settings.USE_POINTWISE:
            return None
        bs = p_emb0.shape[0]
        wa, wb = self._split_fuse_weight(fuse_layer, c)
        pp = pre_layer(p_emb0).reshape(bs, wb.shape[1], -1)
        if c == 64 and wa.shape[0] == 64 and settings.USE_MFMA_GEMM:
            return ops.pointwise([pp], self._fuse_weight_t(fuse_layer, wb, "b"), point_major=True)
        return ops.pointwise([pp], self._fuse_weight_t(fuse_layer, wb, "b"))

    def _p2r_fuse(self, pre_layer, fuse_layer, rgb_emb0, p_emb0, idx, pixel_major=False, point_term=None, want_packed=False):
        bs, c, hr, wr = rgb_emb0.shape
        if fused_eval(rgb_emb0, self):
            code = act_code(getattr(fuse_layer, "activation", None))
            if code is not None:
                wa, wb = self._split_fuse_weight(fuse_layer, c)
                if c == 64 and wa.shape[0] == 64 and settings.USE_MFMA_GEMM:
                    scale, shift = folded_bn(fuse_layer.normlayer.bn)
                    if point_term is not None:
                        t_pm = point_term
                    else:
                        pp = pre_layer(p_emb0).reshape(bs, wb.shape[1], -1)
                        if settings.USE_POINTWISE:
                            t_pm = ops.pointwise([pp], self._fuse_weight_t(fuse_layer, wb, "b"), point_major=True)
                        else:
                            t_pm = torch.matmul(pp.transpose(1, 2), wb.t())
                    cache = fuse_layer.__dict__.get("_gdm_wa_pk")
                    if cache is None or cache[0] is not wa:
                        cache = (wa, ops.pack_rows64(wa))
                        fuse_layer.__dict__["_gdm_wa_pk"] = cache
                    y = ops.conv64_gather_add_act_mfma(rgb_emb0.reshape(bs, c, hr * wr), cache[1], t_pm, idx.reshape(bs, -1), scale, shift,
                                                       code[0], code[1], pixel_major=pixel_major, t_point_major=True,
                                                       hw=(hr, wr) if (want_packed and settings.USE_PACKED_PRODUCERS and not pixel_major) else None)
                    if pixel_major:
                        return y
                    out = y.view(bs, -1, hr, wr)
                    if getattr(y, "_gdm_packed", None) is not None:
                        out._gdm_packed = y._gdm_packed
                    return out
                if point_term is not None:
                    t = point_term
                else:
                    pp = pre_layer(p_emb0).reshape(bs, wb.shape[1], -1)
                    if settings.USE_POINTWISE:
                        t = ops.pointwise([pp], self._fuse_weight_t(fuse_layer, wb, "b"))
                    else:
                        t = ops.wx(wb, pp)
                if c == 64 and wa.shape[0] == 64:
                    scale, shift = folded_bn(fuse_layer.normlayer.bn)
                    y = ops.conv1x1_gather_add_act(rgb_emb0.reshape(bs, c, hr * wr), self._fuse_weight_t(fuse_layer, wa), t,
                                                   idx.reshape(bs, -1), scale, shift, code[0], code[1], pixel_major=pixel_major)
                    return y if pixel_major else y.view(bs, -1, hr, wr)
                if pixel_major:
                    raise RuntimeError("pixel-major fusion output is the 64-channel kernel's; _sparse_final_ok() guards the caller")
                if settings.USE_MFMA_GEMM and ops.gemm_supported(c, wa.shape[0], hr * wr):
                    wpk, co = cached_gemm_weight(fuse_layer, "wa", wa, (fuse_layer.conv.weight,))
                    x = ops.gemm_bf16x3_map(rgb_emb0, wpk, co).view(bs, co, hr * wr)
                else:
                    x = ops.wx(wa, rgb_emb0.reshape(bs, c, hr * wr))
                scale, shift = folded_bn(fuse_layer.normlayer.bn)
                y, ypk = ops.gather_add_affine_act(x, t, idx.reshape(bs, -1), scale, shift, code[0], code[1], hw=(hr, wr))
                y = y.view(bs, -1, hr, wr)
                if ypk is not None:
                    y._gdm_packed = ypk
                return y
        if pixel_major:
            raise RuntimeError("pixel-major fusion output is the eval kernel's; _sparse_final_ok() guards the caller")
        p2r_emb = self.nearest_interpolation(pre_layer(p_emb0), idx).view(bs, -1, hr, wr)
        return fuse_layer(torch.cat((rgb_emb0, p2r_emb), dim=1))

    def forward(self, inputs, end_points=None, parts=False):
        if fused_eval(inputs["rgb"], self):
            pre = self.cnn_pre_stages
            s0, b0 = folded_bn(pre[1])
            mp = pre[3]
            conv = pre[0]
            plain_pool = (isinstance(mp, nn.MaxPool2d) and mp.kernel_size in (3, (3, 3)) and mp.stride in (2, (2, 2)) and mp.padding in (1, (1, 1))
                          and mp.dilation in (1, (1, 1)) and not mp.ceil_mode and isinstance(pre[2], nn.ReLU))
            if (settings.USE_OWN_STEM and plain_pool and tuple(conv.weight.shape) == (64, 3, 7, 7) and conv.bias is None
                    and tuple(conv.stride) == (2, 2) and tuple(conv.padding) == (3, 3) and tuple(conv.dilation) == (1, 1)
                    and inputs["rgb"].shape[0] <= 65535):
                key = (conv.weight._version, conv.weight.data_ptr())
                cache = conv.__dict__.get("_gdm_stem_pk")
                if cache is None or cache[0] != key:
                    cache = (key, ops.stem_pack_weight(conv.weight))
                    conv.__dict__["_gdm_stem_pk"] = cache
                rgb_emb = ops.stem(inputs["rgb"], cache[1], s0, b0)
            else:
                y0 = conv(inputs["rgb"])
                if plain_pool and y0.shape[0] * y0.shape[1] <= 65535:
                    rgb_emb = ops.affine_relu_maxpool(y0, s0, b0)
                else:
                    rgb_emb = mp(ops.affine_act(y0, s0, b0, ops.ACT_RELU))
        else:
            pre = self.cnn_pre_stages
            rgb_emb = pre[3](bn_act(pre[1], pre[0](inputs["rgb"]), pre[2]))
        from . import pyramid as _pyr
        overlap = settings.USE_SIDE_STREAMS and "point" in settings.SIDE_PARTS and fused_eval(inputs["rgb"], self)
        if overlap and settings.USE_TWO_STREAM_PIPELINE:
            return self._forward_two_streams(inputs, rgb_emb, parts)
        if not overlap:
            _pyr.wait_ready(inputs)
        p_emb, f_pc0 = self._stem_and_mlp1(inputs["cld_rgb_nrm"])

        ds_emb = []
        for i_ds in range(4):
            if overlap:
                xyz_i, nei_i, sub_i = inputs["cld_xyz%d" % i_ds], inputs["cld_nei_idx%d" % i_ds], inputs["cld_sub_idx%d" % i_ds]
                with ops.fork(inputs["rgb"].device, 0) as f:
                    if i_ds == 0:
                        _pyr.wait_ready(inputs)
                    f.use(p_emb, xyz_i, nei_i, sub_i)
                    f_encoder_i = self.rndla_ds_stages[i_ds](p_emb, xyz_i, nei_i, f_pc=f_pc0 if i_ds == 0 else None)
                    p_emb0 = self.random_sample(f_encoder_i, sub_i)
                rgb_emb0 = self.cnn_ds_stages[i_ds](rgb_emb)
                if i_ds == 0:
                    _pyr.wait_ready(inputs)
                f.join(f_encoder_i, p_emb0)
            else:
                rgb_emb0 = self.cnn_ds_stages[i_ds](rgb_emb)
                f_encoder_i = self.rndla_ds_stages[i_ds](p_emb, inputs["cld_xyz%d" % i_ds], inputs["cld_nei_idx%d" % i_ds],
                                                         f_pc=f_pc0 if i_ds == 0 else None)
                p_emb0 = self.random_sample(f_encoder_i, inputs["cld_sub_idx%d" % i_ds])
            bs, c, hr, wr = rgb_emb0.size()
            if i_ds == 0:
                ds_emb.append(f_encoder_i)

            rgb_emb = self._p2r_fuse(self.ds_fuse_p2r_pre_layers[i_ds], self.ds_fuse_p2r_fuse_layers[i_ds], rgb_emb0, p_emb0,
                                     inputs["p2r_ds_nei_idx%d" % i_ds], want_packed=True)

            r2p_emb = self.random_sample(rgb_emb0.reshape(bs, c, hr * wr), inputs["r2p_ds_nei_idx%d" % i_ds])
            r2p_emb = self.ds_fuse_r2p_pre_layers[i_ds](r2p_emb)
            p_emb = self.ds_fuse_r2p_fuse_layers[i_ds].forward_segs([p_emb0, r2p_emb])
            ds_emb.append(p_emb)

        n_up = len(self.rndla_up_stages)
        sparse_final = self._sparse_final_ok(inputs["rgb"])
        for i_up in range(n_up - 1):
            rgb_emb0 = self.cnn_up_stages[i_up](rgb_emb)
            bs, c, hr, wr = rgb_emb0.size()

            p_emb0 = self.rndla_up_stages[i_up].forward_segs([ds_emb[-i_up - 2], (p_emb, inputs["cld_interp_idx%d" % (n_up - i_up - 1)])])

            rgb_emb = self._p2r_fuse(self.up_fuse_p2r_pre_layers[i_up], self.up_fuse_p2r_fuse_layers[i_up], rgb_emb0, p_emb0,
                                     inputs["p2r_up_nei_idx%d" % i_up], pixel_major=sparse_final and i_up == n_up - 2)

            r2p_emb = self.random_sample(rgb_emb0.reshape(bs, c, hr * wr), inputs["r2p_up_nei_idx%d" % i_up])
            r2p_emb = self.up_fuse_r2p_pre_layers[i_up](r2p_emb)
            p_emb = self.up_fuse_r2p_fuse_layers[i_up].forward_segs([p_emb0, r2p_emb])

        p_emb = self.rndla_up_stages[n_up - 1].forward_segs([ds_emb[0], (p_emb, inputs["cld_interp_idx0"])]).squeeze(-1)
        if sparse_final:
            rgb_emb_c = self._final_at_choose(rgb_emb, (hr, wr), inputs["choose"])
        elif self._gathered_final_ok():
            last = self.cnn_up_stages[n_up - 1]
            rgb_emb = last[0](rgb_emb)
            bs, di, _, _ = rgb_emb.size()
            rgb_emb_c = ops.gather_nn(rgb_emb.view(bs, di, -1), inputs["choose"].reshape(bs, -1, 1))
            rgb_emb_c = last[1](rgb_emb_c.unsqueeze(-1)).squeeze(-1)
        else:
            rgb_emb = self.cnn_up_stages[n_up - 1](rgb_emb)
            bs, di, _, _ = rgb_emb.size()
            rgb_emb_c = ops.gather_nn(rgb_emb.view(bs, di, -1), inputs["choose"].reshape(bs, -1, 1))
        if parts:
            return rgb_emb_c, p_emb
        return torch.cat([rgb_emb_c, p_emb], dim=1)

    def _stem_and_mlp1(self, x):
        blk = self.rndla_ds_stages[0]
        if settings.USE_POINT_CHAIN and settings.USE_POINTWISE and fused_eval(x, self) and x.dim() == 3:
            p0, p1 = self.rndla_pre_stages._pointwise_params(), blk.mlp1._pointwise_params()
            if (p0 is not None and p1 is not None and p0[0].shape[0] <= 16 and p0[0].shape[1] <= 16 and p1[0].shape[1] <= 32
                    and p1[0].shape[0] == p0[0].shape[1]):
                y0, y1 = ops.pointwise_chain2(x, p0, p1)
                return y0.unsqueeze(3), y1.unsqueeze(3)
        return self.rndla_pre_stages(x).unsqueeze(3), None

    def _forward_two_streams(self, inputs, rgb_emb, parts):
        from . import pyramid as _pyr
        dev = inputs["rgb"].device
        M = torch.cuda.current_stream(dev)
        S = ops.side_stream(dev, 0)

        def to(stream, *ts):
            for t in ts:
                if torch.is_tensor(t) and t.is_cuda:
                    t.record_stream(stream)

        def event(stream):
            e = torch.cuda.Event()
            e.record(stream)
            return e

        S.wait_stream(M)
        to(S, inputs["cld_rgb_nrm"])
        with torch.cuda.stream(S):
            _pyr.wait_ready(inputs, cloud_only=True)
            p_emb, f_pc0 = self._stem_and_mlp1(inputs["cld_rgb_nrm"])
        ds_emb = []
        for i_ds in range(4):
            rgb_emb0 = self.cnn_ds_stages[i_ds](rgb_emb)
            ev_rgb0 = event(M)
            bs, c, hr, wr = rgb_emb0.size()
            with torch.cuda.stream(S):
                f_encoder_i = self.rndla_ds_stages[i_ds](p_emb, inputs["cld_xyz%d" % i_ds], inputs["cld_nei_idx%d" % i_ds],
                                                         f_pc=f_pc0 if i_ds == 0 else None)
                p_emb0 = self.random_sample(f_encoder_i, inputs["cld_sub_idx%d" % i_ds])
                pt = self._p2r_point_term(self.ds_fuse_p2r_pre_layers[i_ds], self.ds_fuse_p2r_fuse_layers[i_ds], c, p_emb0)
                ev_p0 = event(S)
                S.wait_event(ev_rgb0)
                to(S, rgb_emb0)
                if i_ds == 0:
                    _pyr.wait_ready(inputs)
                r2p_emb = self.random_sample(rgb_emb0.reshape(bs, c, hr * wr), inputs["r2p_ds_nei_idx%d" % i_ds])
                r2p_emb = self.ds_fuse_r2p_pre_layers[i_ds](r2p_emb)
                p_emb = self.ds_fuse_r2p_fuse_layers[i_ds].forward_segs([p_emb0, r2p_emb])
            if i_ds == 0:
                ds_emb.append(f_encoder_i)
            ds_emb.append(p_emb)
            if i_ds == 0:
                _pyr.wait_ready(inputs)
            M.wait_event(ev_p0)
            to(M, p_emb0, pt)
            rgb_emb = self._p2r_fuse(self.ds_fuse_p2r_pre_layers[i_ds], self.ds_fuse_p2r_fuse_layers[i_ds], rgb_emb0, p_emb0,
                                     inputs["p2r_ds_nei_idx%d" % i_ds], point_term=pt, want_packed=True)
        n_up = len(self.rndla_up_stages)
        sparse_final = self._sparse_final_ok(inputs["rgb"])
        for i_up in range(n_up - 1):
            rgb_emb0 = self.cnn_up_stages[i_up](rgb_emb)
            ev_rgb0 = event(M)
            bs, c, hr, wr = rgb_emb0.size()
            with torch.cuda.stream(S):
                p_emb0 = self.rndla_up_stages[i_up].forward_segs([ds_emb[-i_up - 2], (p_emb, inputs["cld_interp_idx%d" % (n_up - i_up - 1)])])
                pt = self._p2r_point_term(self.up_fuse_p2r_pre_layers[i_up], self.up_fuse_p2r_fuse_layers[i_up], c, p_emb0)
                ev_p0 = event(S)
                S.wait_event(ev_rgb0)
                to(S, rgb_emb0)
                r2p_emb = self.random_sample(rgb_emb0.reshape(bs, c, hr * wr), inputs["r2p_up_nei_idx%d" % i_up])
                r2p_emb = self.up_fuse_r2p_pre_layers[i_up](r2p_emb)
                p_emb = self.up_fuse_r2p_fuse_layers[i_up].forward_segs([p_emb0, r2p_emb])
            M.wait_event(ev_p0)
            to(M, p_emb0, pt)
            rgb_emb = self._p2r_fuse(self.up_fuse_p2r_pre_layers[i_up], self.up_fuse_p2r_fuse_layers[i_up], rgb_emb0, p_emb0,
                                     inputs["p2r_up_nei_idx%d" % i_up], pixel_major=sparse_final and i_up == n_up - 2, point_term=pt)
        with torch.cuda.stream(S):
            p_emb = self.rndla_up_stages[n_up - 1].forward_segs([ds_emb[0], (p_emb, inputs["cld_interp_idx0"])]).squeeze(-1)
        if sparse_final:
            rgb_emb_c = self._final_at_choose(rgb_emb, (hr, wr), inputs["choose"])
        else:
            rgb_emb = self.cnn_up_stages[n_up - 1](rgb_emb)
            bs, di, _, _ = rgb_emb.size()
            rgb_emb_c = ops.gather_nn(rgb_emb.view(bs, di, -1), inputs["choose"].reshape(bs, -1, 1))
        M.wait_stream(S)
        to(M, p_emb)
        if parts:
            return rgb_emb_c, p_emb
        return torch.cat([rgb_emb_c, p_emb], dim=1)

    def _gathered_final_ok(self):
        from .cnn import FinalStage
        last = self.cnn_up_stages[len(self.rndla_up_stages) - 1]
        return settings.USE_GATHERED_FINAL and len(last) == 2 and isinstance(last[1], FinalStage)

    def _sparse_final_ok(self, rgb):
        from .cnn import FinalStage, PSPUpsample
        last = self.cnn_up_stages[len(self.rndla_up_stages) - 1]
        if not (settings.USE_SPARSE_FINAL and settings.USE_FUSED_UPCONV and fused_eval(rgb, self) and len(last) == 2):
            return False
        up, fin = last[0], last[1]
        if not (isinstance(up, PSPUpsample) and isinstance(fin, FinalStage)):
            return False
        conv, fconv = up.conv[1], fin[0]
        fuse = self.up_fuse_p2r_fuse_layers[len(self.rndla_up_stages) - 2]
        return (conv.in_channels == 64 and conv.out_channels == 64 and fconv.in_channels == 64 and fconv.out_channels == 64
                and act_code(up.conv[3]) is not None and act_code(getattr(fuse, "activation", None)) is not None
                and fuse.conv.weight.shape[0] == 64 and fuse.conv.weight.shape[1] == 128 and rgb.shape[0] <= 65535)

    def _final_at_choose(self, x_pm, hw, choose):
        from .layers import folded_bn as _fbn
        last = self.cnn_up_stages[len(self.rndla_up_stages) - 1]
        up, fin = last[0], last[1]
        conv, fconv = up.conv[1], fin[0]
        key = (conv.weight._version, conv.weight.data_ptr(), fconv.weight._version, fconv.weight.data_ptr())
        cache = self.__dict__.get("_gdm_final_pk")
        if cache is None or cache[0] != key:
            cache = (key, ops.upconv_fused64_pack_weight(conv.weight), ops.pack_rows64(fconv.weight.reshape(64, 64)))
            self.__dict__["_gdm_final_pk"] = cache
        scale, shift = _fbn(up.conv[2], conv.bias)
        code = act_code(up.conv[3])
        return ops.upconv_final_points(x_pm, hw, choose, cache[1], scale, shift, code[0], code[1], cache[2], fconv.bias,
                                       (hw[0] * 2, hw[1] * 2))
```

### geometric_aware_dense_matching_amd/ops.py

```python
import ctypes
import os

import torch

from . import _lib, settings
from ._lib import KnnJob, check

MATCH_BF16X3 = 0
MATCH_F32 = 1


def _stream():
    return torch.cuda.current_stream().cuda_stream


_side_streams = {}


def side_stream(device, which=0):
    key = (device.index if device.index is not None else torch.cuda.current_device(), which)
    st = _side_streams.get(key)
    if st is None:
        st = torch.cuda.Stream(device=device)
        _side_streams[key] = st
# ... 1153 lines not shown
    return y


def conv1x1_logsoftmax(x, weight, bias):
    x = _dev(x, torch.float32, "x")
    B, C, H, W = x.shape
    key = (weight._version, weight.data_ptr())
    cache = getattr(weight, "_gdm_final_wt", None)
    if cache is None or cache[0] != key:
        cache = (key, weight.detach().reshape(C, C).t().contiguous())
        weight._gdm_final_wt = cache
    w = cache[1]
    out = torch.empty_like(x)
    check(_lib.lib().gdm_conv1x1_logsoftmax_hip(x.data_ptr(), w.data_ptr(), bias.data_ptr() if bias is not None else None,
                                                B, C, H * W, out.data_ptr(), _stream()), "gdm_conv1x1_logsoftmax_hip")
    return out


def channel_sum(t):
    B, C = t.shape[0], t.shape[1]
    inner = t.numel() // max(B * C, 1)
    if not (t.is_cuda and t.dtype == torch.float32 and t.is_contiguous() and B * C <= 65535 and inner >= 4 and inner % 4 == 0
            and t.data_ptr() % 16 == 0):
        return t.sum(dim=[0] + list(range(2, t.dim())))
    L = _lib.lib()
    sums = torch.empty(L.gdm_bn_sums_len(B, C, inner), dtype=torch.float64, device=t.device)
    check(L.gdm_bn_stats_hip(t.data_ptr(), B, C, inner, sums.data_ptr(), _stream()), "gdm_bn_stats_hip")
    return sums[:-2].view(-1, C, 2)[:, :, 0].sum(0).float()


class _PspPools(torch.autograd.Function):
    @staticmethod
    def forward(ctx, x):
        x = _dev(x, torch.float32, "x")
        B, C, H, W = x.shape
        outs = [torch.empty((B, C, s_, s_), dtype=torch.float32, device=x.device) for s_ in (1, 2, 3, 6)]
        check(_lib.lib().gdm_psp_pools_hip(x.data_ptr(), B * C, H, W, outs[0].data_ptr(), outs[1].data_ptr(), outs[2].data_ptr(),
                                           outs[3].data_ptr(), _stream()), "gdm_psp_pools_hip")
        ctx.shape = (B, C, H, W)
        return tuple(outs)

    @staticmethod
    def backward(ctx, g1, g2, g3, g6):
        B, C, H, W = ctx.shape
        gs = [_dev(g, torch.float32, "grad") for g in (g1, g2, g3, g6)]
        gx = torch.empty((B, C, H, W), dtype=torch.float32, device=gs[0].device)
        check(_lib.lib().gdm_psp_pools_bwd_hip(gs[0].data_ptr(), gs[1].data_ptr(), gs[2].data_ptr(), gs[3].data_ptr(), B * C, H, W,
                                               gx.data_ptr(), _stream()), "gdm_psp_pools_bwd_hip")
        return gx


def psp_pools_supported(h, w):
    return 36 <= h * w <= 4096 and h >= 6 and w >= 6


def psp_pools(x):
    return list(_PspPools.apply(x))


class _PspCombine(torch.autograd.Function):

    @staticmethod
    def forward(ctx, g, bias, y1, y2, y3, y4):
        g = _dev(g, torch.float32, "g")
        ys = [_dev(y, torch.float32, "y") for y in (y1, y2, y3, y4)]
        B, C, H, W = g.shape
        out = torch.empty_like(g)
        check(_lib.lib().gdm_psp_combine2_hip(g.data_ptr(), ys[0].data_ptr(), ys[0].shape[2], ys[1].data_ptr(), ys[1].shape[2],
                                              ys[2].data_ptr(), ys[2].shape[2], ys[3].data_ptr(), ys[3].shape[2],
                                              bias.data_ptr() if bias is not None else None, B, C, H, W, out.data_ptr(), None, _stream()),
              "gdm_psp_combine2_hip")
        ctx.save_for_backward(out)
        ctx.sizes = [y.shape[2] for y in ys]
        ctx.has_bias = bias is not None
        return out

    @staticmethod
    def backward(ctx, go):
        (out,) = ctx.saved_tensors
        B, C, H, W = out.shape
        gpre = torch.where(out > 0, go, torch.zeros((), dtype=go.dtype, device=go.device)).contiguous()
        gys = []
        L = _lib.lib()
        for s_ in ctx.sizes:
            gy = torch.empty((B, C, s_, s_), dtype=torch.float32, device=go.device)
            check(L.gdm_upsample_bilinear_bwd_hip(gpre.data_ptr(), B * C, s_, s_, H, W, gy.data_ptr(), _stream()), "gdm_upsample_bilinear_bwd_hip")
            gys.append(gy)
        gb = channel_sum(gpre) if ctx.has_bias else None
        return gpre, gb, gys[0], gys[1], gys[2], gys[3]


def psp_combine_train(g, ys, bias):
    assert len(ys) == 4
    return _PspCombine.apply(g, bias, ys[0], ys[1], ys[2], ys[3])


class BufferPool:

    def __init__(self):
        self.packed = {}
        self.workspace = {}


_default_pool = BufferPool()
_pool = _default_pool
_warned_capture = []


class buffer_pool:
    def __init__(self, pool):
        self.pool, self.prev = pool, None

    def __enter__(self):
        global _pool
        self.prev, _pool = _pool, self.pool
        return self.pool

    def __exit__(self, *exc):
        global _pool
        _pool = self.prev
        return False


def _capturing_unscoped():
    if _pool is _default_pool and torch.cuda.is_current_stream_capturing():
        if not _warned_capture:
            _warned_capture.append(1)
            import warnings
            warnings.warn("geometric_aware_dense_matching_amd.ops: hipGraph capture outside ops.buffer_pool(...): scratch buffers "
                          "are allocated per call inside the graph; give the capture a BufferPool of its own")
        return True
    return False




def conv3x3_wgrad_supported(x, go):
    B, Cin, H, W = x.shape
    return (settings.USE_MFMA_WGRAD and x.is_cuda and x.dtype == torch.float32 and go.shape[0] == B and tuple(go.shape[2:]) == (H, W)
            and W in (32, 64) and (H * W) % 128 == 0 and Cin % 256 == 0 and go.shape[1] % 8 == 0)


def conv3x3_wgrad(x, go, parts=None):
    x = _dev(x, torch.float32, "x")
    go = _dev(go, torch.float32, "grad_out")
    B, Cin, H, W = x.shape
    Cout = go.shape[1]
    L = _lib.lib()
    nx, ng = L.gdm_wgrad_x_bytes(B, Cin, H, W), L.gdm_wgrad_go_bytes(B, Cout, H, W)
    if nx == 0 or ng == 0 or (9 * Cin) % 256 != 0:
        raise ValueError("conv3x3_wgrad: unsupported shape x %s grad_out %s" % (tuple(x.shape), tuple(go.shape)))
    xpk = torch.empty(nx, dtype=torch.uint8, device=x.device)
    gpk = torch.empty(ng, dtype=torch.uint8, device=x.device)
    check(L.gdm_wgrad_pack_x_hip(x.data_ptr(), B, Cin, H, W, xpk.data_ptr(), _stream()), "gdm_wgrad_pack_x_hip")
    check(L.gdm_wgrad_pack_go_hip(go.data_ptr(), B, Cout, H, W, gpk.data_ptr(), _stream()), "gdm_wgrad_pack_go_hip")
    nchunk = B * H * W // 128
    if parts is None:
        tiles = (9 * Cin // 256) * ((Cout + 127) // 128)
        parts = 1
        for d in range(1, nchunk + 1):
            if nchunk % d == 0 and d * tiles <= 320 and nchunk // d >= 4:
                parts = d
    if nchunk % parts != 0:
        raise ValueError("conv3x3_wgrad: %d parts do not divide the %d chunks of the contraction" % (parts, nchunk))
    n = nchunk // parts
    coutp = (Cout + 127) // 128 * 128
    out = torch.empty((parts, Cout, 9, Cin), dtype=torch.float32, device=x.device)
    check(L.gdm_conv1x1_packed_wb_hip(xpk.data_ptr(), gpk.data_ptr(), n * coutp * 512, parts, 128 * n, Cout, 9, Cin, out.data_ptr(), _stream()),
          "gdm_conv1x1_packed_wb_hip")
    dw = out[0] if parts == 1 else out.sum(0)
    return dw.view(Cout, 3, 3, Cin).permute(0, 3, 1, 2).contiguous()


def conv3x3_supported(x, weight, stride=(1, 1), padding=(1, 1), dilation=(1, 1)):
    cin = weight.shape[1]
    st = tuple(stride)
    if st not in ((1, 1), (2, 2)):
        return False
    return (x.is_cuda and x.dtype == torch.float32 and x.dim() == 4 and tuple(weight.shape[2:]) == (3, 3)
            and tuple(padding) == (1, 1) and tuple(dilation) == (1, 1)
            and x.shape[2] % st[0] == 0 and x.shape[3] % st[1] == 0 and (x.shape[3] // st[1]) % 32 == 0
            and (cin == 64 or cin % 128 == 0) and weight.shape[0] % 8 == 0 and x.shape[0] <= 65535)


def conv_pack_weight_dgrad(weight):
    weight = _dev(weight.detach(), torch.float32, "weight")
    Cout, Cin = weight.shape[0], weight.shape[1]
    taps = 9 if weight.dim() == 4 else 1
    L = _lib.lib()
    nbytes = L.gdm_conv3x3_weight_bytes(Cin, Cout) if taps == 9 else L.gdm_conv1x1_weight_bytes(Cin, Cout)
    wpk = torch.empty(nbytes, dtype=torch.uint8, device=weight.device)
    check(L.gdm_conv_pack_weight_dgrad_hip(weight.data_ptr(), Cout, Cin, taps, wpk.data_ptr(), _stream()), "gdm_conv_pack_weight_dgrad_hip")
    return wpk


def conv3x3_pack_weight(weight):
    weight = _dev(weight.detach(), torch.float32, "weight")
    Cout, Cin = weight.shape[0], weight.shape[1]
    L = _lib.lib()
    wpk = torch.empty(L.gdm_conv3x3_weight_bytes(Cout, Cin), dtype=torch.uint8, device=weight.device)
    check(L.gdm_conv3x3_pack_weight_hip(weight.data_ptr(), Cout, Cin, wpk.data_ptr(), _stream()), "gdm_conv3x3_pack_weight_hip")
    return wpk


class PackedAct:
    __slots__ = ("buf", "shape")

    def __init__(self, buf, shape):
        self.buf, self.shape = buf, tuple(shape)


def _packed_buffer(B, C, H, W, device, avoid=None):
    nbytes = _lib.lib().gdm_conv3x3_act_bytes(B, C, H, W)
    if _capturing_unscoped():
        return torch.zeros(nbytes, dtype=torch.uint8, device=device)
    key = (B, C, H, W, device.index, _stream_lane(device))
    pool = _pool.packed.setdefault(key, [])
    for buf in pool:
        if avoid is None or buf.data_ptr() != avoid.data_ptr():
            return buf
    buf = torch.zeros(nbytes, dtype=torch.uint8, device=device)
    pool.append(buf)
    return buf


def conv3x3_pack_act(x):
    x = _dev(x, torch.float32, "x")
    B, C, H, W = x.shape
    buf = _packed_buffer(B, C, H, W, x.device)
    check(_lib.lib().gdm_conv3x3_pack_act_hip(x.data_ptr(), B, C, H, W, buf.data_ptr(), _stream()), "gdm_conv3x3_pack_act_hip")
    return PackedAct(buf, (B, C, H, W))


def conv3x3_bf16x3(x, wpk, cout, scale=None, shift=None, act=ACT_NONE, res=None, out_f32=True, out_packed=False, stride=1):
    xp = x if isinstance(x, PackedAct) else conv3x3_pack_act(x)
    B, Cin, H, W = xp.shape
    if stride != 1:
        if stride != 2 or H % 2 or W % 2:
            raise ValueError("conv3x3_bf16x3: stride %r on a %dx%d map" % (stride, H, W))
        H, W = H // 2, W // 2
    L = _lib.lib()
    dev = xp.buf.device
    out = torch.empty((B, cout, H, W), dtype=torch.float32, device=dev) if out_f32 else None
    opk = None
    if out_packed:
        if (B * H * W) % 256 != 0 or cout % 8 != 0:
            raise ValueError("conv3x3_bf16x3: packed output needs B*H*W %% 256 == 0 and Cout %% 8 == 0")
        opk = PackedAct(_packed_buffer(B, cout, H, W, dev, avoid=xp.buf), (B, cout, H, W))
    if res is not None:
        res = _dev(res, torch.float32, "res")
        assert tuple(res.shape) == (B, cout, H, W)
    check(L.gdm_conv3x3_strided_hip(xp.buf.data_ptr(), wpk.data_ptr(), scale.data_ptr() if scale is not None else None,
                                    shift.data_ptr() if shift is not None else None, res.data_ptr() if res is not None else None,
                                    B, Cin, cout, H, W, int(stride), act, out.data_ptr() if out is not None else None,
                                    opk.buf.data_ptr() if opk is not None else None, _stream()), "gdm_conv3x3_strided_hip")
    return (out, opk) if out_packed else out


def gemm_bf16x3_map(x, wpk, cout):
    B, Cin, H, W = x.shape
    xp = getattr(x, "_gdm_packed", None)
    if isinstance(xp, PackedAct) and xp.shape == (B, Cin, H, W) and W % 32 == 0:
        return conv1x1_packed2d(xp, wpk, cout)
    return gemm_bf16x3(x.reshape(B, Cin, H * W), wpk, cout).view(B, cout, H, W)


def conv1x1_packed2d(xp, wpk, cout, scale=None, shift=None, act=ACT_NONE, stride=1):
    B, Cin, H, W = xp.shape
    if stride not in (1, 2) or H % stride or W % stride:
        raise ValueError("conv1x1_packed2d: stride %r on a %dx%d map" % (stride, H, W))
    H, W = H // stride, W // stride
    out = torch.empty((B, cout, H, W), dtype=torch.float32, device=xp.buf.device)
    check(_lib.lib().gdm_conv1x1_strided_hip(xp.buf.data_ptr(), wpk.data_ptr(), scale.data_ptr() if scale is not None else None,
                                             shift.data_ptr() if shift is not None else None, B, Cin, cout, H, W, int(stride), act,
                                             out.data_ptr(), _stream()), "gdm_conv1x1_strided_hip")
    return out


class _Conv3x3Train(torch.autograd.Function):
    @staticmethod
    def forward(ctx, x, weight):
        ctx.save_for_backward(x, weight)
        return conv3x3_bf16x3(x, conv3x3_pack_weight(weight), weight.shape[0])

    @staticmethod
    def backward(ctx, go):
        x, weight = ctx.saved_tensors
        go = _dev(go, torch.float32, "grad")
        gx = gw = None
        if ctx.needs_input_grad[0]:
            gx = conv3x3_bf16x3(go, conv_pack_weight_dgrad(weight), weight.shape[1])
        if ctx.needs_input_grad[1]:
            if conv3x3_wgrad_supported(x, go):
                gw = conv3x3_wgrad(x, go)
            else:
                gw = torch.ops.aten.convolution_backward(go, x, weight, None, [1, 1], [1, 1], [1, 1], False, [0, 0], 1, [False, True, False])[1]
        return gx, gw


def conv3x3_train(x, weight):
    return _Conv3x3Train.apply(x, weight)


def gemm_supported(cin, cout, npix):
    return (cin % 128 == 0 or cin == 64) and (cout % 128 == 0 or cout >= 192) and npix % 32 == 0


def gemm_pack_weight(weight2d):
    w = _dev(weight2d.detach(), torch.float32, "weight")
    Cout, Cin = w.shape
    L = _lib.lib()
    wpk = torch.empty(L.gdm_conv1x1_weight_bytes(Cout, Cin), dtype=torch.uint8, device=w.device)
    check(L.gdm_conv1x1_pack_weight_hip(w.data_ptr(), Cout, Cin, wpk.data_ptr(), _stream()), "gdm_conv1x1_pack_weight_hip")
    return wpk


def gemm_bf16x3(x, wpk, cout, scale=None, shift=None, act=ACT_NONE, pixel_major=False):
    x = _dev(x, torch.float32, "x")
    B, Cin, n = x.shape
    L = _lib.lib()
    xpk = _packed_buffer(B, Cin, 1, n, x.device)
    check(L.gdm_conv3x3_pack_act_hip(x.data_ptr(), B, Cin, 1, n, xpk.data_ptr(), _stream()), "gdm_conv3x3_pack_act_hip")
    out = torch.empty((B * n, cout) if pixel_major else (B, cout, n), dtype=torch.float32, device=x.device)
    check(L.gdm_conv1x1_packed_hip(xpk.data_ptr(), wpk.data_ptr(), scale.data_ptr() if scale is not None else None,
                                   shift.data_ptr() if shift is not None else None, B, Cin, cout, 1, n, act,
                                   1 if pixel_major else 0, out.data_ptr(), _stream()), "gdm_conv1x1_packed_hip")
    return out


def spline_packed_buffer(C, M, device, avoid=None):
    return _packed_buffer(1, C, 1, M, device, avoid=avoid)


def gemm_grouped(x_cm, wpk, rowidx, tile_co0, cout_total, xpk=None):
    x_cm = _dev(x_cm, torch.float32, "x")
    _, Cin, M = x_cm.shape
    R = rowidx.shape[0]
    L = _lib.lib()
    if xpk is None:
        xpk = _packed_buffer(1, Cin, 1, M, x_cm.device)
        check(L.gdm_conv3x3_pack_act_hip(x_cm.data_ptr(), 1, Cin, 1, M, xpk.data_ptr(), _stream()), "gdm_conv3x3_pack_act_hip")
    Y = torch.empty((R, 128), dtype=torch.float32, device=x_cm.device)
    check(L.gdm_gemm_grouped_hip(xpk.data_ptr(), wpk.data_ptr(), rowidx.data_ptr(), tile_co0.data_ptr(), R, M, Cin, cout_total,
                                 Y.data_ptr(), _stream()), "gdm_gemm_grouped_hip")
    return Y


class _UpsampleBilinear(torch.autograd.Function):
    @staticmethod
    def forward(ctx, x, OH, OW):
        x = _dev(x, torch.float32, "x")
        B, C, H, W = x.shape
        out = torch.empty((B, C, OH, OW), dtype=torch.float32, device=x.device)
        check(_lib.lib().gdm_upsample_bilinear_hip(x.data_ptr(), B * C, H, W, OH, OW, out.data_ptr(), _stream()),
              "gdm_upsample_bilinear_hip")
        ctx.hw = (H, W)
        return out

    @staticmethod
    def backward(ctx, go):
        go = go.contiguous()
        B, C, OH, OW = go.shape
        H, W = ctx.hw
        g = torch.empty((B, C, H, W), dtype=torch.float32, device=go.device)
        check(_lib.lib().gdm_upsample_bilinear_bwd_hip(go.data_ptr(), B * C, H, W, OH, OW, g.data_ptr(), _stream()),
              "gdm_upsample_bilinear_bwd_hip")
        return g, None, None


class _PReLU1(torch.autograd.Function):
    @staticmethod
    def forward(ctx, x, slope):
        x = x.contiguous()
        y = torch.empty_like(x)
        check(_lib.lib().gdm_prelu1_hip(x.data_ptr(), slope.data_ptr(), x.numel(), y.data_ptr(), _stream()), "gdm_prelu1_hip")
        ctx.save_for_backward(x, slope)
        return y

    @staticmethod
    def backward(ctx, go):
        x, slope = ctx.saved_tensors
        go = go.contiguous()
        gx = torch.empty_like(x)
        gs = torch.zeros_like(slope)
        check(_lib.lib().gdm_prelu1_bwd_hip(x.data_ptr(), go.data_ptr(), slope.data_ptr(), x.numel(), gx.data_ptr(), gs.data_ptr(), _stream()),
              "gdm_prelu1_bwd_hip")
        return gx, gs


def prelu1(x, slope):
    x = _dev(x, torch.float32, "x")
    return _PReLU1.apply(x, slope)


def upsample_bilinear(x, size):
    return _UpsampleBilinear.apply(x, int(size[0]), int(size[1]))


def _workspace(nbytes, device):
    if _capturing_unscoped():
        return torch.empty(max(int(nbytes), 16), dtype=torch.uint8, device=device)
    key = (device.index, _stream_lane(device))
    ws = _pool.workspace.get(key)
    if ws is None or ws.numel() < nbytes:
        ws = torch.empty(nbytes, dtype=torch.uint8, device=device)
        _pool.workspace[key] = ws
    return ws


def match(scene, model, precision=MATCH_BF16X3, return_sim=False):
    scene = _dev(scene, torch.float32, "scene")
    model = _dev(model, torch.float32, "model")
    if model.dim() == 3:
        assert model.shape[0] == 1
        model = model[0]
    B, D, N = scene.shape
    M = model.shape[1]
    assert model.shape[0] == D
    L = _lib.lib()
    nbytes = L.gdm_match_workspace_bytes(B, N, M)
    ws = _workspace(nbytes, scene.device)
    best_idx = torch.empty((B, N), dtype=torch.int32, device=scene.device)
    best_sim = torch.empty((B, N), dtype=torch.float32, device=scene.device)
    sim = torch.empty((B, N, M), dtype=torch.float32, device=scene.device) if return_sim else None
    check(L.gdm_match_hip(scene.data_ptr(), model.data_ptr(), B, D, N, M, precision, best_idx.data_ptr(),
                          best_sim.data_ptr(), sim.data_ptr() if return_sim else None, ws.data_ptr(), ws.numel(),
                          _stream()), "gdm_match_hip")
    return (best_idx, best_sim, sim) if return_sim else (best_idx, best_sim)


def match_pack(x, precision=MATCH_BF16X3, out=None):
    x = _dev(x, torch.float32, "x")
    if x.dim() == 2:
        x = x.unsqueeze(0)
    R, D, n = x.shape
    L = _lib.lib()
    if out is None:
        out = torch.empty((L.gdm_match_rows_bytes(R * n),), dtype=torch.uint8, device=x.device)
    check(L.gdm_match_pack_hip(x.data_ptr(), R, D, n, precision, out.data_ptr(), _stream()), "gdm_match_pack_hip")
    return out


def match_pack2(x1, x2, precision=MATCH_BF16X3):
    x1 = _dev(x1, torch.float32, "x1")
    x2 = _dev(x2, torch.float32, "x2")
    x1 = x1.unsqueeze(0) if x1.dim() == 2 else x1
    x2 = x2.unsqueeze(0) if x2.dim() == 2 else x2
    (R1, D, n1), (R2, D2, n2) = x1.shape, x2.shape
    if D != D2:
        raise ValueError("match_pack2: %d vs %d channels" % (D, D2))
    L = _lib.lib()
    o1 = torch.empty((L.gdm_match_rows_bytes(R1 * n1),), dtype=torch.uint8, device=x1.device)
    o2 = torch.empty((L.gdm_match_rows_bytes(R2 * n2),), dtype=torch.uint8, device=x1.device)
    check(L.gdm_match_pack2_hip(x1.data_ptr(), R1, n1, o1.data_ptr(), x2.data_ptr(), R2, n2, o2.data_ptr(), D, precision, _stream()),
          "gdm_match_pack2_hip")
    return o1, o2


def match_packed(scene_rows, model_rows, B, N, M, precision=MATCH_BF16X3, return_sim=False, sim_out=None):
    L = _lib.lib()
    dev = scene_rows.device
    part = _workspace(L.gdm_match_partial_bytes(B, N), dev)
    best_idx = torch.empty((B, N), dtype=torch.int32, device=dev)
    best_sim = torch.empty((B, N), dtype=torch.float32, device=dev)
    sim = None
    if return_sim:
        sim = sim_out if sim_out is not None else torch.empty((B, N, M), dtype=torch.float32, device=dev)
    check(L.gdm_match_packed_hip(scene_rows.data_ptr(), model_rows.data_ptr(), B * N, M, precision, best_idx.data_ptr(),
                                 best_sim.data_ptr(), sim.data_ptr() if return_sim else None, part.data_ptr(), part.numel(),
                                 _stream()), "gdm_match_packed_hip")
    return (best_idx, best_sim, sim) if return_sim else (best_idx, best_sim)


def seg_mask(seg):
    seg = _dev(seg, torch.float32, "seg")
    B, two, N = seg.shape
    assert two == 2
    mask = torch.empty((B, N), dtype=torch.uint8, device=seg.device)
    count = torch.empty((B,), dtype=torch.int32, device=seg.device)
    check(_lib.lib().gdm_seg_mask_hip(seg.data_ptr(), B, N, mask.data_ptr(), count.data_ptr(), _stream()),
          "gdm_seg_mask_hip")
    return mask, count
```

### geometric_aware_dense_matching_amd/settings.py

```python
import os


def _flag(name, default="1"):
    return os.environ.get(name, default) != "0"


USE_MFMA_CONV = _flag("GDM_MFMA_CONV")
USE_MFMA_CONV_TRAIN = _flag("GDM_MFMA_CONV_TRAIN")
USE_MFMA_GEMM = _flag("GDM_MFMA_GEMM")
USE_FUSED_UPCONV = _flag("GDM_FUSED_UPCONV")
USE_LOWRES_UPCONV_TRAIN = _flag("GDM_LOWRES_UPCONV_TRAIN")
USE_SPLIT_PSP_TRAIN = _flag("GDM_SPLIT_PSP_TRAIN")
USE_FUSED_LFA = _flag("GDM_FUSED_LFA")
USE_GROUPED_SPLINE = _flag("GDM_GROUPED_SPLINE")
USE_FUSED_BN_TRAIN = _flag("GDM_FUSED_BN_TRAIN")
USE_FUSED_SYNCBN = _flag("GDM_FUSED_SYNCBN")
USE_FUSED_MATCH_LOSS = _flag("GDM_FUSED_MATCH_LOSS")
USE_SIDE_STREAMS = _flag("GDM_SIDE_STREAMS", "0")
USE_SPARSE_FINAL = _flag("GDM_SPARSE_FINAL")
USE_FUSED_HEADS = _flag("GDM_FUSED_HEADS")
USE_MFMA_STRIDED = _flag("GDM_MFMA_STRIDED")
USE_POINTWISE = _flag("GDM_POINTWISE")
USE_OWN_STEM = _flag("GDM_OWN_STEM")
USE_GEMM_CONV1X1_TRAIN = _flag("GDM_GEMM_CONV1X1_TRAIN")
USE_MFMA_WGRAD = _flag("GDM_MFMA_WGRAD")
USE_MFMA_GEMM_TRAIN = _flag("GDM_MFMA_GEMM_TRAIN")
USE_GATHERED_FINAL = _flag("GDM_GATHERED_FINAL")
USE_DIRECT_WGRAD = _flag("GDM_DIRECT_WGRAD")
USE_FUSED_ADAM = _flag("GDM_FUSED_ADAM")
USE_POINTWISE_TRAIN = _flag("GDM_POINTWISE_TRAIN")
USE_POINT_CHAIN = _flag("GDM_POINT_CHAIN")
USE_PSP_JOBS = _flag("GDM_PSP_JOBS")
USE_PACKED_PRODUCERS = _flag("GDM_PACKED_PRODUCERS")
USE_TWO_STREAM_PIPELINE = _flag("GDM_TWO_STREAM_PIPELINE")
MESH_FORK_LATE = os.environ.get("GDM_MESH_FORK_LATE", "1") != "0"
PACK_MESH_ROWS = os.environ.get("GDM_PACK_MESH_ROWS", "1") != "0"
SIDE_PARTS = os.environ.get("GDM_SIDE_PARTS", "mesh,point,pyr").split(",")
STATIC_MATCH_ROWS = _flag("GDM_STATIC_MATCH_ROWS", "0")
UPCONV_MIN_CIN = int(os.environ.get("GDM_UPCONV_MIN_CIN", "0"))
SYNCBN_MIN_WORLD = 2

ALL_SWITCHES = ("USE_MFMA_CONV", "USE_MFMA_CONV_TRAIN", "USE_MFMA_GEMM", "USE_FUSED_UPCONV", "USE_LOWRES_UPCONV_TRAIN",
                "USE_SPLIT_PSP_TRAIN", "USE_FUSED_LFA", "USE_GROUPED_SPLINE", "USE_FUSED_BN_TRAIN", "USE_FUSED_SYNCBN",
                "USE_FUSED_MATCH_LOSS", "USE_SIDE_STREAMS", "USE_SPARSE_FINAL", "USE_FUSED_HEADS", "USE_MFMA_STRIDED", "USE_POINTWISE", "USE_OWN_STEM", "USE_GEMM_CONV1X1_TRAIN", "USE_MFMA_WGRAD", "USE_MFMA_GEMM_TRAIN", "USE_GATHERED_FINAL", "USE_DIRECT_WGRAD", "USE_PSP_JOBS", "USE_POINT_CHAIN", "USE_POINTWISE_TRAIN")
SPLIT_BF16_SWITCHES = ("USE_MFMA_CONV", "USE_MFMA_GEMM", "USE_FUSED_UPCONV", "USE_SPARSE_FINAL", "USE_FUSED_HEADS", "USE_MFMA_STRIDED",
                       "USE_OWN_STEM")
```

### include/gdm.h

```cpp
#ifndef GDM_H
#define GDM_H

#include <stddef.h>
#include <stdint.h>

#ifdef __cplusplus
extern "C" {
#endif

#define GDM_EINVAL (-1)
#define GDM_ENOMEM (-2)

const char* gdm_last_error(void);
int gdm_version(void);


void gdm_knn_batch(const float* batch_data, size_t batch_size, size_t npts, size_t dim,
                   const float* queries, size_t nqueries, size_t K, long* batch_indices);

int gdm_knn_batch_hip(const float* support, const float* query, int B, int S, int Q, int K,
                      int32_t* idx, float* d2, void* stream);

typedef struct gdm_knn_job {
    const float* support;
    const float* query;
    int32_t* idx;
    float* d2;
    int64_t support_bstride;
    int64_t query_bstride;
    int32_t S, Q, K;
    int32_t grid_w;
} gdm_knn_job;
#define GDM_KNN_MAX_JOBS 32
size_t gdm_knn_jobs_workspace_bytes(const gdm_knn_job* jobs, int njobs, int B);
int gdm_knn_jobs_ws_hip(const gdm_knn_job* jobs, int njobs, int B, void* workspace, size_t workspace_bytes, void* stream);

int gdm_ballquery_hip(int B, int n, int m, float radius, int nsample,
                      const float* new_xyz, const float* xyz, int32_t* idx, void* stream);

int gdm_furthestsampling_hip(int B, int n, int m, const float* xyz, float* temp, int32_t* idx, void* stream);

int gdm_interpolation_forward_hip(int B, int c, int m, int n, const float* feat, const int32_t* idx, const float* weight, float* out, void* stream);
int gdm_interpolation_backward_hip(int B, int c, int n, int m, const float* grad_out, const int32_t* idx, const float* weight,
                                   float* grad_feat, void* stream);

int gdm_labelstat_ballrange_hip(int B, int n, int m, float radius, int nclass, const float* new_xyz, const float* xyz,
                                const int32_t* label_stat, int32_t* new_label_stat, void* stream);
int gdm_labelstat_idx_hip(int B, int n, int m, int nsample, int nclass, const int32_t* label_stat, const int32_t* idx,
                          int32_t* new_label_stat, void* stream);


int gdm_group_gather_hip(const float* feat, const int32_t* idx, int B, int C, int n, int m, int K,
                         float* out, void* stream);
int gdm_group_gather_bwd2_hip(const float* grad_out, long go_bstride, const int32_t* idx, int B, int C, int n, int m, int K,
                              float* grad_feat, void* stream);

int gdm_gather_max_hip(const float* feat, const int32_t* idx, int B, int C, int n, int m, int K,
                       float* out, int32_t* arg, void* stream);
int gdm_gather_max_bwd_hip(const float* grad_out, const int32_t* arg, int B, int C, int n, int m,
                           float* grad_feat, void* stream);

int gdm_rel_pos_enc_hip(const float* xyz, const int32_t* idx, int B, int n, int K, float* out, void* stream);

int gdm_att_pool_hip(const float* att, const float* feat, int B, int C, int n, int K, float* out, void* stream);
int gdm_att_pool_bwd_hip(const float* att, const float* feat, const float* grad_out, int B, int C, int n, int K,
                         float* grad_att, float* grad_feat, void* stream);


#define GDM_MATCH_BF16X3 0
#define GDM_MATCH_F32    1

size_t gdm_match_workspace_bytes(int B, int N, int M);

int gdm_match_hip(const float* scene, const float* model, int B, int D, int N, int M, int precision,
                  int32_t* best_idx, float* best_sim, float* sim,
                  void* workspace, size_t workspace_bytes, void* stream);

size_t gdm_match_rows_bytes(int rows);
size_t gdm_match_partial_bytes(int B, int N);
int gdm_match_pack_hip(const float* x, int R, int D, int n, int precision, void* rows, void* stream);
int gdm_match_pack2_hip(const float* x1, int R1, int n1, void* rows1, const float* x2, int R2, int n2, void* rows2,
                        int D, int precision, void* stream);
int gdm_match_packed_hip(const void* scene_rows, const void* model_rows, int R , int M, int precision,
                         int32_t* best_idx, float* best_sim, float* sim,
                         void* partial, size_t partial_bytes, void* stream);

int gdm_seg_mask_hip(const float* seg, int B, int N, uint8_t* mask, int32_t* count, void* stream);

int gdm_spline_aggregate_hip(const float* xw, const int32_t* rowptr, const int32_t* src, const float* attr,
                             const float* root, const float* bias, int M, int C, int kernel_size, int relu,
                             float* out, void* stream);
int gdm_spline_aggregate_bwd_hip(const float* grad_out, const int32_t* rowptr, const int32_t* src, const float* attr,
                                 int M, int C, int kernel_size, float* grad_xw, void* stream);
int gdm_spline_direct3_hip(const float* x, const float* weight, const int32_t* rowptr, const int32_t* src, const float* attr,
                           const float* root_t, const float* bias, int M, int Cin, int C, int kernel_size, int relu,
                           float* out, float* out_t, void* out_packed, void* stream);
int gdm_gemm_grouped_hip(const void* xpk, const void* wpk, const int32_t* rowidx, const int32_t* tile_co0, int R, int M,
                         int Cin, int Cout_total, float* out, void* stream);
int gdm_spline_pairs_aggregate3_hip(const float* Y, const int32_t* rowptr, const int32_t* pos, const float* basis,
                                    const float* root, const float* bias, int M, int C, int relu, float* out, float* out_t,
                                    void* out_packed, void* stream);

int gdm_upsample_bilinear_hip(const float* in, long planes, int H, int W, int OH, int OW, float* out, void* stream);
int gdm_upsample_bilinear_bwd_hip(const float* grad_out, long planes, int H, int W, int OH, int OW, float* grad_in, void* stream);

int gdm_topk_rows_hip(const float* score, long rows, int n, int K, int32_t* idx, float* val, void* stream);
int gdm_topk_negdist_hip(const float* gram, const float* xx, int B, int n, int K, int32_t* idx, void* stream);
int gdm_edge_feature_hip(const float* x, const int32_t* idx, int B, int C, int n, int K, float* out, void* stream);
int gdm_edge_feature_bwd_hip(const float* grad_out, const int32_t* idx, int B, int C, int n, int K, float* grad_x, void* stream);

int gdm_circle_rows_fwd_hip(const float* sim, int R, int Mp, const int32_t* match, const int32_t* item,
                            const float* xyz, const uint8_t* vis, float radius, float gamma, float m,
                            float* lse_p, float* lse_n, float* loss, void* stream);
int gdm_circle_rows_bwd_hip(const float* sim, int R, int Mp, const int32_t* match, const int32_t* item,
                            const float* xyz, const uint8_t* vis, float radius, float gamma, float m,
                            const float* lse_p, const float* lse_n, const float* grad_rows, float* dsim, void* stream);

size_t gdm_circle_match_rows_bytes(int n);
size_t gdm_circle_match_tp_bytes(int n);
int gdm_circle_match_pack_hip(const float* x, int n, void* rows, void* tp, float* rowsum, void* stream);
int gdm_circle_match_nbr_hip(const float* xyz, int M, float radius, uint32_t* nbr, void* stream);
int gdm_circle_match_visbits_hip(const uint8_t* vis, int B, int M, uint32_t* bits, void* stream);
int gdm_circle_match_nbr_items_hip(const float* xyz, int M, const float* rad , int B, uint32_t* nbr, void* stream);
int gdm_circle_match_fwd2_hip(const void* xrows, const void* xtp, const float* xpad, const void* yrows, const void* ytp,
                              int R, int M, const int32_t* g, const int32_t* c2, const int32_t* item,
                              const uint32_t* nbr, int nbr_per_item, const uint32_t* visb, int pad_e0, float gamma, float m,
                              float* lse_p, float* lse_n, float* loss, void* stream);
int gdm_circle_match_bwd2_hip(const void* xrows, const void* xtp, const float* xpad, const void* yrows, const void* ytp,
                              int R, int M, const int32_t* g, const int32_t* c2, const int32_t* item,
                              const uint32_t* nbr, int nbr_per_item, const uint32_t* visb, int pad_e0, float gamma, float m,
                              const float* lse_p, const float* lse_n, const float* coef, float* gx, float* gy_part, void* stream);
int gdm_circle_match_bwd_parts(int R, int M);

int gdm_lfa_stage_hip(const float* xyz, const int32_t* idx, const float* feat, const float* w1t, const float* s1, const float* b1,
                      const float* w2t, const float* s2, const float* b2, const float* wft, const float* wmt, const float* sm,
                      const float* bm, int B, int n, int K, int D, int OUT, float slope, float* out, void* stream);

int gdm_kabsch_stats_hip(const float* scene_xyz, long scene_bstride, int pt_stride, int ch_stride, const float* model_xyz,
                         const int32_t* best_idx, const uint8_t* mask, int B, int N, int M, double* out, void* stream);

int gdm_kabsch_solve_hip(const double* stats, int B, int min_points, float* RT, uint8_t* valid, void* stream);

#define GDM_RANSAC_MAX_H 4096
size_t gdm_ransac_workspace_bytes(int B, int N, int H);
int gdm_ransac_pose_hip(const float* scene_xyz, long scene_bstride, int pt_stride, int ch_stride, const float* model_xyz,
                        const int32_t* best_idx, const uint8_t* mask, const double* stats, int B, int N, int M, int H,
                        float match_err, double fix_percent, uint32_t seed, int min_points, void* workspace, size_t workspace_bytes,
                        float* RT, uint8_t* valid, int32_t* counts, int32_t* winner, void* stream);

int gdm_icp_transform_hip(const float* scene_xyz, long scene_bstride, int pt_stride, int ch_stride, const float* RT, int B, int N,
                          float* query, void* stream);
int gdm_icp_update_hip(const float* scene_xyz, long scene_bstride, int pt_stride, int ch_stride, const float* model_xyz,
                       const int32_t* nn, const float* d2, const uint8_t* mask, int B, int N, int M, float reject_dist,
                       double tolerance, int min_points, float* RT, uint8_t* active, int32_t* iters, double* err, void* stream);

#define GDM_TARGETS_MIN_M 4
size_t gdm_targets_workspace_bytes(int B, int N, int M);
int gdm_hpr_visible_hip(const float* model_xyz, long model_bstride, const float* RT, const float* cam_center, int B, int M,
                        void* workspace, size_t workspace_bytes, double* flipped, uint8_t* visible, void* stream);
int gdm_pose_targets_hip(const float* cld, long cld_bstride, int pt_stride, int ch_stride, const uint8_t* labels, const float* RT,
                         const float* model_xyz, long model_bstride, const uint8_t* visible, int B, int N, int M, double dist_thresh,
                         void* workspace, size_t workspace_bytes, uint8_t* labels_out, int32_t* match_idx, uint8_t* visible_flag,
                         uint8_t* valid, void* stream);

int gdm_affine_act_maxk_hip(const float* x, const float* scale, const float* shift, long planes, int C, long n, int K, int act,
                            float slope, float* out, void* stream);

int gdm_prelu1_hip(const float* x, const float* slope, long n, float* y, void* stream);
int gdm_prelu1_bwd_hip(const float* x, const float* grad_out, const float* slope, long n, float* grad_x, float* grad_slope, void* stream);

int gdm_affine_act_hip(const float* x, const float* scale, const float* shift, const float* res, const float* res_scale,
                       const float* res_shift, long planes, int C, long inner, int act, float slope, float* y, void* stream);

int gdm_upconv3x3_gather_hip(const float* z, const float* scale, const float* shift, int B, int Cout, int H, int W,
                             int OH, int OW, int act, float slope, float* out, void* stream);
int gdm_upconv3x3_gather2_hip(const float* z, const float* scale, const float* shift, int B, int Cout, int H, int W,
                              int OH, int OW, int act, float slope, float* out, void* outpk, void* stream);
int gdm_upconv3x3_gather_bwd_hip(const float* grad_out, int B, int Cout, int H, int W, int OH, int OW, float* grad_z, void* stream);
size_t gdm_upconv_fused64_weight_bytes(void);
int gdm_upconv_fused64_pack_weight_hip(const float* w, void* wpk, void* stream);
int gdm_upconv_fused64_hip(const float* x, const void* wpk, const float* scale, const float* shift, int B, int C, int H, int W,
                           int OH, int OW, int act, float slope, float* out, void* stream);

int gdm_psp_combine2_hip(const float* g, const float* y1, int s1, const float* y2, int s2, const float* y3, int s3,
                         const float* y4, int s4, const float* bias, int B, int C, int H, int W, float* out, void* outpk, void* stream);
int gdm_gather_add_affine_act2_hip(const float* x, const float* t, const int32_t* idx, const float* scale, const float* shift,
                                   int B, int C, int n, int m, int act, float slope, float* y, void* y_packed, int W, void* stream);
int gdm_conv1x1_gather_add_act2_hip(const float* x, const float* wt, const float* t, const int32_t* idx, const float* scale,
                                    const float* shift, int B, int C, int n, long m, int act, float slope, int pixel_major,
                                    float* y, void* stream);
int gdm_conv64_gather_add_act_mfma2_hip(const float* x, const void* wpk, const float* t, const int32_t* idx, const float* scale,
                                        const float* shift, int B, int n, long m, int act, float slope, int pixel_major,
                                        int t_point_major, float* y, void* ypk, int W, void* stream);

size_t gdm_conv3x3_act_bytes(int B, int Cin, int H, int W);
size_t gdm_conv3x3_weight_bytes(int Cout, int Cin);
int gdm_conv3x3_pack_weight_hip(const float* w, int Cout, int Cin, void* wpk, void* stream);
int gdm_conv3x3_pack_act_hip(const float* x, int B, int Cin, int H, int W, void* xpk, void* stream);
int gdm_conv3x3_packed_hip(const void* xpk, const void* wpk, const float* scale, const float* shift, const float* res,
                           int B, int Cin, int Cout, int H, int W, int act, float* out, void* stream);
int gdm_conv3x3_strided_hip(const void* xpk, const void* wpk, const float* scale, const float* shift, const float* res,
                            int B, int Cin, int Cout, int H, int W, int stride, int act, float* out, void* outpk, void* stream);
int gdm_conv1x1_strided_hip(const void* xpk, const void* wpk, const float* scale, const float* shift,
                            int B, int Cin, int Cout, int H, int W, int stride, int act, float* out, void* stream);

int gdm_affine_relu_maxpool_hip(const float* x, const float* scale, const float* shift, int B, int C, int H, int W, float* y, void* stream);
int gdm_conv1x1_logsoftmax_hip(const float* x, const float* w, const float* bias, int B, int C, long hw, float* out, void* stream);
int gdm_pack_rows64_hip(const float* w, int R, void* out, void* stream);
int gdm_upconv_final_points_hip(const float* xpm, const int32_t* choose, const void* wpk, const float* scale, const float* shift,
                                int act, float slope, const void* wfpk, const float* fbias, int B, int H, int W, int OH, int OW,
                                int N, float* out, void* stream);
int gdm_psp_pools_hip(const float* x, long planes, int H, int W, float* o1, float* o2, float* o3, float* o6, void* stream);
int gdm_psp_pools_bwd_hip(const float* g1, const float* g2, const float* g3, const float* g6, long planes, int H, int W,
                          float* grad_x, void* stream);

size_t gdm_conv1x1_weight_bytes(int Cout, int Cin);
int gdm_conv1x1_pack_weight_hip(const float* w, int Cout, int Cin, void* wpk, void* stream);
int gdm_conv_pack_weight_dgrad_hip(const float* w, int Cout, int Cin, int taps, void* wpk, void* stream);
int gdm_conv1x1_packed_hip(const void* xpk, const void* wpk, const float* scale, const float* shift,
                           int B, int Cin, int Cout, int H, int W, int act, int pixel_major, float* out, void* stream);

int gdm_depth_to_xyz_hip(const float* depth, const float* K, const int32_t* origin, int B, int H, int W, int S,
                         float* out, void* stream);

long gdm_bn_sums_len(int B, int C, long inner);
int gdm_bn_stats_hip(const float* x, int B, int C, long inner, double* sums, void* stream);
int gdm_bn_fwd_apply_hip(const float* x, const double* sums, int groups, const float* weight, const float* bias, int B, int C, long inner, float eps,
                         float momentum, int act, float slope, float* saved, float* running_mean, float* running_var, float* y, void* stream);
int gdm_bn_bwd_reduce_hip(const float* x, const float* grad_out, const float* saved, int B, int C, long inner, int act, float slope,
                          double* sums, void* stream);
int gdm_bn_bwd_apply_hip(const float* x, const float* grad_out, const double* sums, int groups, const float* weight, const float* saved, int B, int C,
                         long inner, int act, float slope, float* grad_weight, float* grad_bias, float* grad_x, void* stream);

int gdm_point_heads2_hip(const float* a, const float* b, int Ca, const float* ra, const float* rb, int rCa, int B, int N, int nlayer,
                         const void* const* w, const float* const* scale, const float* const* shift, const int* act, int feat_layer,
                         int res_layer, const void* w_last, const float* shift_last, int c_last, float* out_feat, float* out_last,
                         void* stream);

typedef struct {
    const float* x;
    const int32_t* idx;
    int32_t C, n_src;
} gdm_pw_seg;
int gdm_pointwise2_hip(const gdm_pw_seg* segs, int nseg, const float* wt, int w_rowmajor, const float* scale, const float* shift,
                       int B, int n, int Cout, int act, float slope, float* out, int out_C, int out_c0, int point_major, void* stream);
typedef struct {
    const float* x;
    const float* wt;
    float* out;
    int32_t n;
} gdm_pw_job;
int gdm_pointwise_jobs_hip(const gdm_pw_job* jobs, int njobs, int B, int K, int Cout, void* stream);
int gdm_pointwise_chain2_hip(const float* x, const float* w0t, const float* s0, const float* b0, int act0, float slope0,
                             const float* w1t, const float* s1, const float* b1, int act1, float slope1,
                             int B, int n, int C0, int C1, int C2, float* y0, float* y1, void* stream);

size_t gdm_stem_weight_bytes(void);
int gdm_stem_pack_weight_hip(const float* w, void* wpk, void* stream);
int gdm_stem_hip(const float* x, const void* wpk, const float* scale, const float* shift, int B, int H, int W, float* out,
                 void* out_packed, void* stream);

size_t gdm_wgrad_x_bytes(int B, int Cin, int H, int W);
size_t gdm_wgrad_go_bytes(int B, int Cout, int H, int W);
int gdm_wgrad_pack_x_hip(const float* x, int B, int Cin, int H, int W, void* out, void* stream);
int gdm_wgrad_pack_go_hip(const float* go, int B, int Cout, int H, int W, void* out, void* stream);
size_t gdm_wgrad_x1_bytes(int B, int Cin, int P);
int gdm_wgrad_pack_x1_hip(const float* x, int B, int Cin, int P, void* out, void* stream);
int gdm_mfma_probe_hip(int blocks, int iters, int chain, float* sink, void* stream);
int gdm_mfma_probe_lds_hip(int blocks, int iters, int rpu, float* sink, void* stream);
int gdm_wgrad_direct_hip(const float* go, long go_bstride, const float* x, long x_bstride, int B, int Cout, int Cin, int P,
                         int nsplit, float* partial, float* bias_partial, void* stream);
int gdm_conv1x1_packed_wb_hip(const void* xpk, const void* wpk, long w_bstride, int B, int Cin, int Cout, int H, int W, float* out,
                              void* stream);

typedef struct gdm_copy_job {
    void* dst;
    const void* src;
    int64_t sb, s1, s2;
    int32_t B, R1, R2, E;
} gdm_copy_job;
#define GDM_COPY_MAX_JOBS 16
int gdm_copy_jobs_hip(const gdm_copy_job* jobs , int njobs, void* stream);

#ifdef __cplusplus
}
#endif
#endif
```

Before: 5202.

## Fold PSP combine and point-to-RGB gather-add into MFMA 1x1 GEMM epilogue

Adds two epilogue variants to the MFMA 1x1 conv kernel. One does the PSP prior upsample-add, bias and ReLU; the other does the point-to-pixel gather-add, affine and activation. The full-resolution GEMM output no longer has to be written and then re-read by a separate combine kernel. The PSP priors are computed before the GEMM instead of alongside it on a side stream, which gives up some overlap. The change also adds 2 GiB operand guards, and the fused path only runs when the new GDM_FUSED_GEMM_EPILOGUE flag is on.

```diff
diff --git a/geometric_aware_dense_matching_amd/_lib.py b/geometric_aware_dense_matching_amd/_lib.py
--- a/geometric_aware_dense_matching_amd/_lib.py
+++ b/geometric_aware_dense_matching_amd/_lib.py
@@ -117,6 +117,8 @@
     "gdm_conv3x3_packed_hip": (_i, [_vp, _vp, _vp, _vp, _vp, _i, _i, _i, _i, _i, _i, _vp, _vp]),
     "gdm_conv3x3_strided_hip": (_i, [_vp, _vp, _vp, _vp, _vp, _i, _i, _i, _i, _i, _i, _i, _vp, _vp, _vp]),
     "gdm_conv1x1_strided_hip": (_i, [_vp, _vp, _vp, _vp, _i, _i, _i, _i, _i, _i, _i, _vp, _vp]),
+    "gdm_conv1x1_p2r_hip": (_i, [_vp, _vp, _vp, _vp, _vp, _vp, _i, _i, _i, _i, _i, _i, _i, _f, _vp, _vp, _vp]),
+    "gdm_conv1x1_psp_hip": (_i, [_vp, _vp, _vp, _i, _vp, _i, _vp, _i, _vp, _i, _vp, _i, _i, _i, _i, _i, _vp, _vp, _vp]),
     "gdm_affine_relu_maxpool_hip": (_i, [_vp, _vp, _vp, _i, _i, _i, _i, _vp, _vp]),
     "gdm_conv1x1_logsoftmax_hip": (_i, [_vp, _vp, _vp, _i, _i, ctypes.c_long, _vp, _vp]),
     "gdm_pack_rows64_hip": (_i, [_vp, _i, _vp, _vp]),
diff --git a/geometric_aware_dense_matching_amd/cnn.py b/geometric_aware_dense_matching_amd/cnn.py
--- a/geometric_aware_dense_matching_amd/cnn.py
+++ b/geometric_aware_dense_matching_amd/cnn.py
@@ -175,7 +175,7 @@
             ms, wf = self._split_weights()
             B, Cin = feats.shape[0], feats.shape[1]
             def full_res():
-                if settings.USE_MFMA_GEMM and ops.gemm_supported(Cin, wf.shape[0], h * w):
+                if settings.USE_MFMA_GEMM and ops.gemm_supported(Cin, wf.shape[0], h * w, B):
                     wpk, co = cached_gemm_weight(self, "wf", wf, (self.bottleneck.weight,))
                     return ops.gemm_bf16x3_map(feats, wpk, co)
                 return ops.wx(wf, feats.reshape(B, Cin, h * w)).view(B, -1, h, w)
@@ -197,6 +197,13 @@
                         ys.append(ops.wx(m, p.reshape(B, Cin, s_ * s_)).view(B, -1, s_, s_))
                 return ys
 
+            packed = settings.USE_MFMA_GEMM and settings.USE_PACKED_PRODUCERS
+            if (settings.USE_MFMA_GEMM and settings.USE_FUSED_GEMM_EPILOGUE and ops.gemm_supported(Cin, wf.shape[0], h * w, B)
+                    and ops.gemm_psp_supported(B, Cin, wf.shape[0], h, w, [st[0].output_size[0] if isinstance(st[0].output_size, (tuple, list))
+                                                                          else st[0].output_size for st in self.stages])):
+                ys = priors()
+                wpk, co = cached_gemm_weight(self, "wf", wf, (self.bottleneck.weight,))
+                return ops.gemm_psp_fused(feats, wpk, co, ys, self.bottleneck.bias, packed=packed)
             if settings.USE_SIDE_STREAMS and "psp" in settings.SIDE_PARTS and not torch.is_grad_enabled():
                 with ops.fork(feats.device, 3) as f:
                     f.use(feats)
@@ -206,7 +213,7 @@
             else:
                 g = full_res()
                 ys = priors()
-            return ops.psp_combine(g, ys, self.bottleneck.bias, packed=settings.USE_MFMA_GEMM and settings.USE_PACKED_PRODUCERS)
+            return ops.psp_combine(g, ys, self.bottleneck.bias, packed=packed)
         sizes = [st[0].output_size[0] if isinstance(st[0].output_size, (tuple, list)) else st[0].output_size for st in self.stages]
         if (settings.USE_SPLIT_PSP_TRAIN and feats.is_cuda and feats.dtype == torch.float32 and sizes == [1, 2, 3, 6] and ops.psp_pools_supported(h, w)
                 and (h * w) % 4 == 0 and feats.shape[0] * self.bottleneck.out_channels <= 65535 and h <= 64 and w <= 64):
diff --git a/geometric_aware_dense_matching_amd/csrc/gdm_conv.hip b/geometric_aware_dense_matching_amd/csrc/gdm_conv.hip
--- a/geometric_aware_dense_matching_amd/csrc/gdm_conv.hip
+++ b/geometric_aware_dense_matching_amd/csrc/gdm_conv.hip
@@ -105,15 +105,32 @@
 constexpr int MF_TSTRIDE = 132;
 constexpr int MF_SMEM = 2 * CV_PANEL > CV_PIX * MF_TSTRIDE * 4 ? 2 * CV_PANEL : CV_PIX * MF_TSTRIDE * 4;
 
-template <int ACT, bool HAS_RES, int TAPS = 9, bool PIXMAJOR = false, int NKS = 8, int NCB = 8, int WV = MF_WAVES>
+enum { EPI_PLAIN = 0, EPI_P2R = 1, EPI_PSP = 2 };
+template <int EPI> struct EpiArgs {};
+template <> struct EpiArgs<EPI_P2R> {
+    const float* t;
+    const int32_t* idx;
+    int n;
+    float slope;
+};
+template <> struct EpiArgs<EPI_PSP> {
+    const float* y[4];
+    int s[4];
+    float sy[4], sx[4];
+    const float* bias;
+};
+
+template <int ACT, bool HAS_RES, int TAPS = 9, bool PIXMAJOR = false, int NKS = 8, int NCB = 8, int WV = MF_WAVES, int EPI = EPI_PLAIN>
 __global__ __launch_bounds__(MF_THREADS) void conv_mfma16_kernel(const unsigned char* __restrict__ xpk, const unsigned char* __restrict__ wpk,
                                                                  const float* __restrict__ scale, const float* __restrict__ shift,
                                                                  const float* __restrict__ res, int B, int Cin, int Cout, int H, int W,
                                                                  float* __restrict__ out, const int32_t* __restrict__ rowidx = nullptr,
                                                                  const int32_t* __restrict__ tile_co0 = nullptr,
                                                                  unsigned char* __restrict__ outpk = nullptr, int stride = 1,
-                                                                 long wbstride = 0)
-{
+                                                                 long wbstride = 0, EpiArgs<EPI> ea = EpiArgs<EPI>())
+{
+    static_assert(EPI == EPI_PLAIN || (TAPS == 1 && !PIXMAJOR && !HAS_RES && WV == MF_WAVES && (NCB == 8 || NCB == 4)),
+                  "the folded epilogues: 1x1 form, NCHW / packed output, eight waves");
     extern __shared__ __attribute__((aligned(16))) unsigned char smem[];
     constexpr int NS = NKS / 2;
     constexpr int UG = (NCB % 2 == 0) ? 2 : 3;
@@ -323,7 +340,35 @@
         return;
     }
     float* tl = reinterpret_cast<float*>(smem) + wave * MF_WPIX * TST;
-    if (outpk) __syncthreads();
+    [[maybe_unused]] int toff[NPH][4];
+    if constexpr (EPI == EPI_P2R) {
+#pragma unroll
+        for (int ph = 0; ph < NPH; ++ph) {
+            const int4 iv = *reinterpret_cast<const int4*>(ea.idx + (long)b * hw + prem + 16 * ph + 4 * kg);
+            const int src[4] = {iv.x, iv.y, iv.z, iv.w};
+#pragma unroll
+            for (int j = 0; j < 4; ++j) toff[ph][j] = min(max(src[j], 0), ea.n - 1) * Cout;
+        }
+    }
+    constexpr int PSP_TS = NCB * 16 + 8;
+    [[maybe_unused]] float* pm = reinterpret_cast<float*>(smem + CV_PIX * TST * 4);
+    if constexpr (EPI == EPI_PSP) {
+        int pbase = 0;
+#pragma unroll
+        for (int k = 0; k < 4; ++k) {
+            const int ss = ea.s[k] * ea.s[k];
+            const float* yk = ea.y[k] + ((long)b * Cout + co0) * ss;
+            for (int i = tid; i < NCB * 16 * ss; i += THREADS) {
+                const int ch = i / ss, j = i - ch * ss;
+                pm[(pbase + j) * PSP_TS + ch] = yk[i];
+            }
+            pbase += ss;
+        }
+        if (tid < NCB * 16) pm[pbase * PSP_TS + tid] = ea.bias ? ea.bias[co0 + tid] : 0.f;
+        __syncthreads();
+    } else {
+        if (outpk) __syncthreads();
+    }
 #pragma unroll
     for (int cb = 0; cb < NCB; ++cb) {
         const int co = co0 + cb * 16 + l16;
@@ -335,24 +380,41 @@
         for (int ph = 0; ph < NPH; ++ph) {
             const int poff = 16 * ph + 4 * kg;
             float v[4];
-#pragma unroll
-            for (int j = 0; j < 4; ++j) v[j] = acc[ph][cb][j] * sc + sh;
-            if (HAS_RES && live) {
-                const float4 r4 = *reinterpret_cast<const float4*>(rp + poff);
-                v[0] += r4.x; v[1] += r4.y; v[2] += r4.z; v[3] += r4.w;
-            }
-            if (ACT == 1) {
-#pragma unroll
-                for (int j = 0; j < 4; ++j) v[j] = fmaxf(v[j], 0.f);
-            }
-            if (op && live) *reinterpret_cast<float4*>(op + poff) = make_float4(v[0], v[1], v[2], v[3]);
-            if (outpk) {
+            if constexpr (EPI == EPI_P2R) {
+                const float* tp = ea.t + (long)b * ea.n * Cout + (live ? co : 0);
+                float tv[4];
+#pragma unroll
+                for (int j = 0; j < 4; ++j) tv[j] = tp[toff[ph][j]];
+#pragma unroll
+                for (int j = 0; j < 4; ++j) {
+                    float o = sc * ((acc[ph][cb][j] * 1.f + 0.f) + tv[j]) + sh;
+                    if (ACT == 1) o = fmaxf(o, 0.f);
+                    if (ACT == 2) o = o > 0.f ? o : o * ea.slope;
+                    v[j] = o;
+                }
+            } else if constexpr (EPI == EPI_PSP) {
+#pragma unroll
+                for (int j = 0; j < 4; ++j) v[j] = acc[ph][cb][j] * 1.f + 0.f;
+            } else {
+#pragma unroll
+                for (int j = 0; j < 4; ++j) v[j] = acc[ph][cb][j] * sc + sh;
+                if (HAS_RES && live) {
+                    const float4 r4 = *reinterpret_cast<const float4*>(rp + poff);
+                    v[0] += r4.x; v[1] += r4.y; v[2] += r4.z; v[3] += r4.w;
+                }
+                if (ACT == 1) {
+#pragma unroll
+                    for (int j = 0; j < 4; ++j) v[j] = fmaxf(v[j], 0.f);
+                }
+            }
+            if (EPI != EPI_PSP && op && live) *reinterpret_cast<float4*>(op + poff) = make_float4(v[0], v[1], v[2], v[3]);
+            if (outpk || EPI == EPI_PSP) {
 #pragma unroll
                 for (int j = 0; j < 4; ++j) tl[(poff + j) * TST + cb * 16 + l16] = live ? v[j] : 0.f;
             }
         }
     }
-    if (outpk) {
+    if (outpk || EPI == EPI_PSP) {
         __builtin_amdgcn_fence(__ATOMIC_ACQ_REL, "wavefront");
         const int lr = lane & 31, h = lane >> 5;
         const int ochunks = (Cout + 127) / 128;
@@ -362,7 +424,25 @@
             const int pp = prem + 32 * half + lr;
             const int yy = pp / W, xx = pp - yy * W;
             unsigned char* ob = outpk + (((long)(b * ochunks + ochunk) * 32) * oplane + (long)(yy + 1) * (W + 2) + xx + 1) * 16;
-            const float* row = tl + (32 * half + lr) * TST;
+            float* row = tl + (32 * half + lr) * TST;
+            [[maybe_unused]] int o00[4], o01[4], o10[4], o11[4];
+            [[maybe_unused]] float ly[4], lx[4];
+            [[maybe_unused]] int obias = 0;
+            if constexpr (EPI == EPI_PSP) {
+                int pbase = 0;
+#pragma unroll
+                for (int k = 0; k < 4; ++k) {
+                    const int S = ea.s[k];
+                    const float fy = ea.sy[k] * (float)yy, fx = ea.sx[k] * (float)xx;
+                    const int y0 = min((int)fy, S - 1), x0 = min((int)fx, S - 1);
+                    const int y1 = y0 + (y0 < S - 1 ? 1 : 0), x1 = x0 + (x0 < S - 1 ? 1 : 0);
+                    ly[k] = fy - (float)y0; lx[k] = fx - (float)x0;
+                    o00[k] = (pbase + y0 * S + x0) * PSP_TS; o01[k] = (pbase + y0 * S + x1) * PSP_TS;
+                    o10[k] = (pbase + y1 * S + x0) * PSP_TS; o11[k] = (pbase + y1 * S + x1) * PSP_TS;
+                    pbase += S * S;
+                }
+                obias = pbase * PSP_TS;
+            }
 #pragma unroll
             for (int it = 0; it < NCB; ++it) {
                 const int ql = 2 * it + h;
@@ -370,11 +450,48 @@
                 const int q = (co0 % 128) / 8 + ql;
                 const float4 a0 = *reinterpret_cast<const float4*>(row + ql * 8);
                 const float4 a1 = *reinterpret_cast<const float4*>(row + ql * 8 + 4);
-                const float v[8] = {a0.x, a0.y, a0.z, a0.w, a1.x, a1.y, a1.z, a1.w};
+                float v[8] = {a0.x, a0.y, a0.z, a0.w, a1.x, a1.y, a1.z, a1.w};
+                if constexpr (EPI == EPI_PSP) {
+                    auto ld8 = [&](int off, float (&m)[8]) {
+                        const float4 m0 = *reinterpret_cast<const float4*>(pm + off + ql * 8);
+                        const float4 m1 = *reinterpret_cast<const float4*>(pm + off + ql * 8 + 4);
+                        m[0] = m0.x; m[1] = m0.y; m[2] = m0.z; m[3] = m0.w; m[4] = m1.x; m[5] = m1.y; m[6] = m1.z; m[7] = m1.w;
+                    };
+                    float bc[8];
+                    ld8(obias, bc);
+#pragma unroll
+                    for (int c = 0; c < 8; ++c) v[c] = v[c] + bc[c];
+#pragma unroll
+                    for (int k = 0; k < 4; ++k) {
+                        float m00[8], m01[8], m10[8], m11[8];
+                        ld8(o00[k], m00); ld8(o01[k], m01); ld8(o10[k], m10); ld8(o11[k], m11);
+#pragma unroll
+                        for (int c = 0; c < 8; ++c)
+                            v[c] += (1.f - ly[k]) * ((1.f - lx[k]) * m00[c] + lx[k] * m01[c]) + ly[k] * ((1.f - lx[k]) * m10[c] + lx[k] * m11[c]);
+                    }
+#pragma unroll
+                    for (int c = 0; c < 8; ++c) v[c] = fmaxf(v[c], 0.f);
+                    *reinterpret_cast<float4*>(row + ql * 8) = make_float4(v[0], v[1], v[2], v[3]);
+                    *reinterpret_cast<float4*>(row + ql * 8 + 4) = make_float4(v[4], v[5], v[6], v[7]);
+                    if (!outpk) continue;
+                }
                 unsigned hi[4], lo[4];
                 split8(v, hi, lo);
                 *reinterpret_cast<uint4*>(ob + (long)q * oplane * 16) = make_uint4(hi[0], hi[1], hi[2], hi[3]);
                 *reinterpret_cast<uint4*>(ob + (long)(16 + q) * oplane * 16) = make_uint4(lo[0], lo[1], lo[2], lo[3]);
+            }
+        }
+        if constexpr (EPI == EPI_PSP) {
+            __builtin_amdgcn_fence(__ATOMIC_ACQ_REL, "wavefront");
+#pragma unroll
+            for (int cb = 0; cb < NCB; ++cb) {
+                float* op = out + ((long)b * Cout + co0 + cb * 16 + l16) * hw + prem;
+#pragma unroll
+                for (int ph = 0; ph < NPH; ++ph) {
+                    const int poff = 16 * ph + 4 * kg;
+                    const float* tr = tl + poff * TST + cb * 16 + l16;
+                    *reinterpret_cast<float4*>(op + poff) = make_float4(tr[0], tr[TST], tr[2 * TST], tr[3 * TST]);
+                }
             }
         }
     }
@@ -467,6 +584,15 @@
 {
     return Cout <= 64 || (long)pixel_tiles * ((Cout + 127) / 128) < 256;
 }
+
+static bool operands_below_2g(long B, int Cin, long Hin, long Win, int taps, int Cout, long wbstride = 0)
+{
+    const long nchunk = (Cin + 127) / 128, lim = 1L << 31;
+    const long act = B * (Hin + 2) * (Win + 2) * nchunk * ROWB;
+    const long wset = (long)taps * nchunk * (((long)Cout + 127) & ~127L) * ROWB;
+    return act < lim && wset < lim && (wbstride == 0 || (B - 1) * wbstride + wset < lim);
+}
+#define GDM_CHECK_2G(who, ...) GDM_CHECK_ARG(operands_below_2g(__VA_ARGS__), "%s: a packed operand of 2 GiB or more (the kernel's buffer offsets are 32-bit)", who)
 
 extern "C" size_t gdm_conv3x3_act_bytes(int B, int Cin, int H, int W)
 {
@@ -548,6 +674,7 @@
     GDM_CHECK_ARG(act == 0 || act == 1, "%s: act=%d", who, act);
     GDM_CHECK_ARG(!outpk || (Cout % 8 == 0 && ((long)B * H * W) % CV_PIX == 0),
                   "%s: packed output needs Cout %% 8 == 0 and B*H*W %% 256 == 0 (got Cout=%d, B*H*W=%ld)", who, Cout, (long)B * H * W);
+    GDM_CHECK_2G(who, B, Cin, (long)H * stride, (long)W * stride, 9, Cout);
     const long ptot = (long)B * H * W;
     dim3 grid(gdm_cdiv(ptot, CV_PIX), gdm_cdiv(Cout, CV_CO));
     hipStream_t s = (hipStream_t)stream;
@@ -619,6 +746,7 @@
     GDM_CHECK_ARG(xpk && wpk && rowidx && tile_co0 && out, "gdm_gemm_grouped_hip: NULL pointer");
     GDM_CHECK_ARG(R >= 256 && R % 256 == 0 && M >= 1 && Cin >= 128 && Cin % 128 == 0 && Cout_total >= 128 && Cout_total % 128 == 0,
                   "gdm_gemm_grouped_hip: R=%d (multiple of 256) M=%d Cin=%d Cout_total=%d (multiples of 128)", R, M, Cin, Cout_total);
+    GDM_CHECK_2G("gdm_gemm_grouped_hip", 1, Cin, 1, M, 1, Cout_total);
     static bool attr = false;
     if (!attr) {
         (void)hipFuncSetAttribute((const void*)CONV_KERNEL<0, false, 1, true>, hipFuncAttributeMaxDynamicSharedMemorySize, 2 * CV_PANEL);
@@ -648,6 +776,7 @@
     GDM_CHECK_ARG(W % 32 == 0 && H >= 1 && (H * W) % CV_PIX == 0, "gdm_conv1x1_packed_wb_hip: W=%d must be a multiple of 32 and H*W=%d of %d",
                   W, H * W, CV_PIX);
     GDM_CHECK_ARG(w_bstride >= 0 && w_bstride % 16 == 0, "gdm_conv1x1_packed_wb_hip: w_bstride=%ld", w_bstride);
+    GDM_CHECK_2G("gdm_conv1x1_packed_wb_hip", B, Cin, H, W, 1, Cout, w_bstride);
     const long ptot = (long)B * H * W;
     dim3 grid(gdm_cdiv(ptot, CV_PIX), gdm_cdiv(Cout, CV_CO));
     static bool attr = false;
@@ -678,6 +807,7 @@
     GDM_CHECK_ARG(W % 32 == 0 && H >= 1 && (H * W) % CONV_WPIX == 0,
                   "%s: W=%d must be a multiple of 32 and H*W=%d of %d", who, W, H * W, CONV_WPIX);
     GDM_CHECK_ARG(act == 0 || act == 1, "%s: act=%d", who, act);
+    GDM_CHECK_2G(who, B, Cin, (long)H * stride, (long)W * stride, 1, Cout);
     const long ptot = (long)B * H * W;
     const unsigned ptiles = gdm_cdiv(ptot, CV_PIX);
     if (Cin != 64 && !pixel_major && stride == 1 && Cout % 144 == 0 && GDM_CONV_GLDS) {
@@ -738,3 +868,83 @@
 #undef C1
     return gdm_launch_status("conv1x1_bf16x3_kernel");
 }
+
+static int epi_shape_ok(const char* who, int B, int Cin, int Cout, int H, int W)
+{
+    GDM_CHECK_ARG(B >= 1 && Cin >= 128 && Cin % 128 == 0 && (Cout == 64 || (Cout >= 128 && Cout % 128 == 0)),
+                  "%s: B=%d Cin=%d (a multiple of 128) Cout=%d (64 or a multiple of 128)", who, B, Cin, Cout);
+    GDM_CHECK_ARG(H >= 1 && W >= 32 && W % 32 == 0 && ((long)H * W) % CV_PIX == 0 && (long)B * H * W < (1L << 31),
+                  "%s: W=%d must be a multiple of 32 and H*W=%ld of %d", who, W, (long)H * W, CV_PIX);
+    GDM_CHECK_2G(who, B, Cin, H, W, 1, Cout);
+    return 0;
+}
+
+constexpr int EPI_SMEM4 = 2 * 64 * ROWB > CV_PIX * 68 * 4 ? 2 * 64 * ROWB : CV_PIX * 68 * 4;
+
+extern "C" int gdm_conv1x1_p2r_hip(const void* xpk, const void* wpk, const float* t, const int32_t* idx, const float* scale, const float* shift,
+                                   int B, int Cin, int Cout, int H, int W, int n, int act, float slope, float* out, void* outpk, void* stream)
+{
+    const char* who = "gdm_conv1x1_p2r_hip";
+    GDM_CHECK_ARG(xpk && wpk && t && idx && scale && shift && out, "%s: NULL pointer", who);
+    if (int rc = epi_shape_ok(who, B, Cin, Cout, H, W)) return rc;
+    GDM_CHECK_ARG(n >= 1 && (long)n * Cout < (1L << 31) && act >= 0 && act <= 2, "%s: n=%d act=%d", who, n, act);
+    GDM_CHECK_ARG((((uintptr_t)idx | (uintptr_t)out | (uintptr_t)outpk) & 15) == 0, "%s: idx / out / outpk must be 16-byte aligned", who);
+    const unsigned ptiles = (unsigned)((long)B * H * W / CV_PIX);
+    const bool narrow = narrow_tiles(ptiles, Cout);
+    const dim3 grid(ptiles, Cout / (narrow ? 64 : CV_CO));
+    EpiArgs<EPI_P2R> ea;
+    ea.t = t; ea.idx = idx; ea.n = n; ea.slope = slope;
+    static bool attr = false;
+#define P2R_K(A, NCB_) CONV_KERNEL<A, false, 1, false, 8, NCB_, MF_WAVES, EPI_P2R>
+    if (!attr) {
+        (void)hipFuncSetAttribute((const void*)P2R_K(0, 8), hipFuncAttributeMaxDynamicSharedMemorySize, CONV_SMEM);
+        (void)hipFuncSetAttribute((const void*)P2R_K(1, 8), hipFuncAttributeMaxDynamicSharedMemorySize, CONV_SMEM);
+        (void)hipFuncSetAttribute((const void*)P2R_K(2, 8), hipFuncAttributeMaxDynamicSharedMemorySize, CONV_SMEM);
+        (void)hipFuncSetAttribute((const void*)P2R_K(0, 4), hipFuncAttributeMaxDynamicSharedMemorySize, EPI_SMEM4);
+        (void)hipFuncSetAttribute((const void*)P2R_K(1, 4), hipFuncAttributeMaxDynamicSharedMemorySize, EPI_SMEM4);
+        (void)hipFuncSetAttribute((const void*)P2R_K(2, 4), hipFuncAttributeMaxDynamicSharedMemorySize, EPI_SMEM4);
+        attr = true;
+    }
+#define P2R(A, NCB_, SM) hipLaunchKernelGGL((P2R_K(A, NCB_)), grid, dim3(CONV_THREADS), SM, (hipStream_t)stream, (const unsigned char*)xpk, (const unsigned char*)wpk, scale, shift, (const float*)nullptr, B, Cin, Cout, H, W, out, (const int32_t*)nullptr, (const int32_t*)nullptr, (unsigned char*)outpk, 1, 0L, ea)
+    if (narrow) { if (act == 0) P2R(0, 4, EPI_SMEM4); else if (act == 1) P2R(1, 4, EPI_SMEM4); else P2R(2, 4, EPI_SMEM4); }
+    else { if (act == 0) P2R(0, 8, CONV_SMEM); else if (act == 1) P2R(1, 8, CONV_SMEM); else P2R(2, 8, CONV_SMEM); }
+#undef P2R
+#undef P2R_K
+    return gdm_launch_status("conv_mfma16_kernel (1x1, p2r epilogue)");
+}
+
+extern "C" int gdm_conv1x1_psp_hip(const void* xpk, const void* wpk, const float* y1, int s1, const float* y2, int s2, const float* y3, int s3,
+                                   const float* y4, int s4, const float* bias, int B, int Cin, int Cout, int H, int W, float* out, void* outpk,
+                                   void* stream)
+{
+    const char* who = "gdm_conv1x1_psp_hip";
+    GDM_CHECK_ARG(xpk && wpk && y1 && y2 && y3 && y4 && out, "%s: NULL pointer", who);
+    if (int rc = epi_shape_ok(who, B, Cin, Cout, H, W)) return rc;
+    GDM_CHECK_ARG(Cout % CV_CO == 0, "%s: Cout=%d must be a multiple of 128", who, Cout);
+    constexpr int PSP_ROW = (CV_CO + 8) * 4, PSP_MAXPOS = (160 * 1024 - CONV_SMEM) / PSP_ROW - 1;
+    GDM_CHECK_ARG(s1 >= 1 && s2 >= 1 && s3 >= 1 && s4 >= 1 && s1 <= 8 && s2 <= 8 && s3 <= 8 && s4 <= 8 &&
+                  s1 * s1 + s2 * s2 + s3 * s3 + s4 * s4 <= PSP_MAXPOS,
+                  "%s: prior maps of at most %d positions in all (the reference's 1, 2, 3, 6 have 50)", who, PSP_MAXPOS);
+    const int smem = CONV_SMEM + (s1 * s1 + s2 * s2 + s3 * s3 + s4 * s4 + 1) * PSP_ROW;
+    GDM_CHECK_ARG((((uintptr_t)out | (uintptr_t)outpk) & 15) == 0, "%s: out / outpk must be 16-byte aligned", who);
+    EpiArgs<EPI_PSP> ea;
+    ea.y[0] = y1; ea.y[1] = y2; ea.y[2] = y3; ea.y[3] = y4;
+    ea.s[0] = s1; ea.s[1] = s2; ea.s[2] = s3; ea.s[3] = s4;
+    for (int k = 0; k < 4; ++k) {
+        ea.sy[k] = H > 1 ? (float)(ea.s[k] - 1) / (float)(H - 1) : 0.f;
+        ea.sx[k] = W > 1 ? (float)(ea.s[k] - 1) / (float)(W - 1) : 0.f;
+    }
+    ea.bias = bias;
+    const dim3 grid((unsigned)((long)B * H * W / CV_PIX), Cout / CV_CO);
+#define PSP_K CONV_KERNEL<0, false, 1, false, 8, 8, MF_WAVES, EPI_PSP>
+    static bool attr = false;
+    if (!attr) {
+        (void)hipFuncSetAttribute((const void*)PSP_K, hipFuncAttributeMaxDynamicSharedMemorySize, 160 * 1024);
+        attr = true;
+    }
+    hipLaunchKernelGGL((PSP_K), grid, dim3(CONV_THREADS), smem, (hipStream_t)stream, (const unsigned char*)xpk, (const unsigned char*)wpk,
+                       (const float*)nullptr, (const float*)nullptr, (const float*)nullptr, B, Cin, Cout, H, W, out, (const int32_t*)nullptr,
+                       (const int32_t*)nullptr, (unsigned char*)outpk, 1, 0L, ea);
+#undef PSP_K
+    return gdm_launch_status("conv_mfma16_kernel (1x1, PSP epilogue)");
+}
diff --git a/geometric_aware_dense_matching_amd/ffb6d.py b/geometric_aware_dense_matching_amd/ffb6d.py
--- a/geometric_aware_dense_matching_amd/ffb6d.py
+++ b/geometric_aware_dense_matching_amd/ffb6d.py
@@ -106,13 +106,20 @@
             layer.__dict__[slot] = cache
         return cache[1]
 
-    def _p2r_point_term(self, pre_layer, fuse_layer, c, p_emb0):
+    @staticmethod
+    def _p2r_fold_ok(bs, c, cout, hr, wr, n, pixel_major=False):
+        return (settings.USE_MFMA_GEMM and settings.USE_FUSED_GEMM_EPILOGUE and not pixel_major and not (c == 64 and cout == 64)
+                and ops.gemm_supported(c, cout, hr * wr, bs) and ops.gemm_p2r_supported(bs, c, cout, hr, wr, n))
+
+    def _p2r_point_term(self, pre_layer, fuse_layer, c, p_emb0, hw=None):
         if not fused_eval(p_emb0, self) or act_code(getattr(fuse_layer, "activation", None)) is None or not settings.USE_POINTWISE:
             return None
         bs = p_emb0.shape[0]
         wa, wb = self._split_fuse_weight(fuse_layer, c)
         pp = pre_layer(p_emb0).reshape(bs, wb.shape[1], -1)
         if c == 64 and wa.shape[0] == 64 and settings.USE_MFMA_GEMM:
+            return ops.pointwise([pp], self._fuse_weight_t(fuse_layer, wb, "b"), point_major=True)
+        if hw is not None and self._p2r_fold_ok(bs, c, wa.shape[0], hw[0], hw[1], pp.shape[2]):
             return ops.pointwise([pp], self._fuse_weight_t(fuse_layer, wb, "b"), point_major=True)
         return ops.pointwise([pp], self._fuse_weight_t(fuse_layer, wb, "b"))
 
@@ -145,8 +152,22 @@
                     if getattr(y, "_gdm_packed", None) is not None:
                         out._gdm_packed = y._gdm_packed
                     return out
+                n_pts = p_emb0.numel() // (bs * p_emb0.shape[1])
+                if settings.USE_POINTWISE and self._p2r_fold_ok(bs, c, wa.shape[0], hr, wr, n_pts, pixel_major):
+                    if point_term is not None:
+                        t_pm = point_term
+                    else:
+                        pp = pre_layer(p_emb0).reshape(bs, wb.shape[1], -1)
+                        t_pm = ops.pointwise([pp], self._fuse_weight_t(fuse_layer, wb, "b"), point_major=True)
+                    wpk, co = cached_gemm_weight(fuse_layer, "wa", wa, (fuse_layer.conv.weight,))
+                    scale, shift = folded_bn(fuse_layer.normlayer.bn)
+                    y, ypk = ops.gemm_p2r_fused(rgb_emb0, wpk, co, t_pm, idx.reshape(bs, -1), scale, shift, code[0], code[1])
+                    y._gdm_packed = ypk
+                    return y
                 if point_term is not None:
                     t = point_term
+                    if tuple(t.shape) != (bs, wa.shape[0], n_pts):
+                        raise RuntimeError("p2r point term %s, want [B, Cout, n'] = %s" % (tuple(t.shape), (bs, wa.shape[0], n_pts)))
                 else:
                     pp = pre_layer(p_emb0).reshape(bs, wb.shape[1], -1)
                     if settings.USE_POINTWISE:
@@ -160,7 +181,7 @@
                     return y if pixel_major else y.view(bs, -1, hr, wr)
                 if pixel_major:
                     raise RuntimeError("pixel-major fusion output is the 64-channel kernel's; _sparse_final_ok() guards the caller")
-                if settings.USE_MFMA_GEMM and ops.gemm_supported(c, wa.shape[0], hr * wr):
+                if settings.USE_MFMA_GEMM and ops.gemm_supported(c, wa.shape[0], hr * wr, bs):
                     wpk, co = cached_gemm_weight(fuse_layer, "wa", wa, (fuse_layer.conv.weight,))
                     x = ops.gemm_bf16x3_map(rgb_emb0, wpk, co).view(bs, co, hr * wr)
                 else:
@@ -313,7 +334,7 @@
                 f_encoder_i = self.rndla_ds_stages[i_ds](p_emb, inputs["cld_xyz%d" % i_ds], inputs["cld_nei_idx%d" % i_ds],
                                                          f_pc=f_pc0 if i_ds == 0 else None)
                 p_emb0 = self.random_sample(f_encoder_i, inputs["cld_sub_idx%d" % i_ds])
-                pt = self._p2r_point_term(self.ds_fuse_p2r_pre_layers[i_ds], self.ds_fuse_p2r_fuse_layers[i_ds], c, p_emb0)
+                pt = self._p2r_point_term(self.ds_fuse_p2r_pre_layers[i_ds], self.ds_fuse_p2r_fuse_layers[i_ds], c, p_emb0, hw=(hr, wr))
                 ev_p0 = event(S)
                 S.wait_event(ev_rgb0)
                 to(S, rgb_emb0)
@@ -339,7 +360,8 @@
             bs, c, hr, wr = rgb_emb0.size()
             with torch.cuda.stream(S):
                 p_emb0 = self.rndla_up_stages[i_up].forward_segs([ds_emb[-i_up - 2], (p_emb, inputs["cld_interp_idx%d" % (n_up - i_up - 1)])])
-                pt = self._p2r_point_term(self.up_fuse_p2r_pre_layers[i_up], self.up_fuse_p2r_fuse_layers[i_up], c, p_emb0)
+                pt = self._p2r_point_term(self.up_fuse_p2r_pre_layers[i_up], self.up_fuse_p2r_fuse_layers[i_up], c, p_emb0,
+                                          hw=None if (sparse_final and i_up == n_up - 2) else (hr, wr))
                 ev_p0 = event(S)
                 S.wait_event(ev_rgb0)
                 to(S, rgb_emb0)
diff --git a/geometric_aware_dense_matching_amd/ops.py b/geometric_aware_dense_matching_amd/ops.py
--- a/geometric_aware_dense_matching_amd/ops.py
+++ b/geometric_aware_dense_matching_amd/ops.py
@@ -1479,8 +1479,74 @@
     return _Conv3x3Train.apply(x, weight)
 
 
-def gemm_supported(cin, cout, npix):
-    return (cin % 128 == 0 or cin == 64) and (cout % 128 == 0 or cout >= 192) and npix % 32 == 0
+def packed_below_2g(B, cin, H, W, cout, taps=1):
+    nchunk = (cin + 127) // 128
+    return max(B * (H + 2) * (W + 2) * nchunk * 512, taps * nchunk * ((cout + 127) // 128 * 128) * 512) < (1 << 31)
+
+
+def gemm_supported(cin, cout, npix, batch=1):
+    return (cin % 128 == 0 or cin == 64) and (cout % 128 == 0 or cout >= 192) and npix % 32 == 0 and packed_below_2g(batch, cin, 1, npix, cout)
+
+
+def _gemm_epilogue_shape_ok(B, cin, cout, H, W):
+    return (B >= 1 and cin >= 128 and cin % 128 == 0 and (cout == 64 or (cout >= 128 and cout % 128 == 0)) and H >= 1 and W >= 32 and W % 32 == 0
+            and (H * W) % 256 == 0 and B * H * W < (1 << 31) and packed_below_2g(B, cin, H, W, cout))
+
+
+def gemm_p2r_supported(B, cin, cout, H, W, n):
+    return _gemm_epilogue_shape_ok(B, cin, cout, H, W) and n >= 1 and n * cout < (1 << 31)
+
+
+def gemm_psp_supported(B, cin, cout, H, W, sizes):
+    sizes = list(sizes)
+    return (_gemm_epilogue_shape_ok(B, cin, cout, H, W) and cout % 128 == 0 and len(sizes) == 4 and all(1 <= s <= 8 for s in sizes)
+            and sum(s * s for s in sizes) <= 51)
+
+
+def _packed_operand(x):
+    xp = getattr(x, "_gdm_packed", None)
+    if isinstance(xp, PackedAct) and xp.shape == tuple(x.shape):
+        return xp
+    return conv3x3_pack_act(x)
+
+
+def gemm_p2r_fused(x, wpk, cout, t_pm, idx, scale, shift, act=ACT_NONE, slope=0.0, packed=True):
+    B, Cin, H, W = x.shape
+    t_pm = _dev(t_pm, torch.float32, "t")
+    idx = _idx32(idx, "idx")
+    n = t_pm.shape[1]
+    if tuple(t_pm.shape) != (B, n, cout) or idx.numel() != B * H * W:
+        raise ValueError("gemm_p2r_fused: t %s (want [%d, n, %d]), idx %s for a %dx%d map" % (tuple(t_pm.shape), B, cout, tuple(idx.shape), H, W))
+    if not gemm_p2r_supported(B, Cin, cout, H, W, n):
+        raise ValueError("gemm_p2r_fused: unsupported shape B=%d Cin=%d Cout=%d H=%d W=%d n=%d (ops.gemm_p2r_supported)" % (B, Cin, cout, H, W, n))
+    xp = _packed_operand(x)
+    dev = xp.buf.device
+    y = torch.empty((B, cout, H, W), dtype=torch.float32, device=dev)
+    opk = PackedAct(_packed_buffer(B, cout, H, W, dev, avoid=xp.buf), (B, cout, H, W)) if packed else None
+    check(_lib.lib().gdm_conv1x1_p2r_hip(xp.buf.data_ptr(), wpk.data_ptr(), t_pm.data_ptr(), idx.data_ptr(), scale.data_ptr(), shift.data_ptr(),
+                                         B, Cin, cout, H, W, n, int(act), float(slope), y.data_ptr(),
+                                         opk.buf.data_ptr() if opk is not None else None, _stream()), "gdm_conv1x1_p2r_hip")
+    return y, opk
+
+
+def gemm_psp_fused(x, wpk, cout, ys, bias, packed=False):
+    B, Cin, H, W = x.shape
+    ys = [_dev(y, torch.float32, "y") for y in ys]
+    sizes = [y.shape[2] for y in ys]
+    if not gemm_psp_supported(B, Cin, cout, H, W, sizes) or any(tuple(y.shape) != (B, cout, s, s) for y, s in zip(ys, sizes)):
+        raise ValueError("gemm_psp_fused: unsupported shape B=%d Cin=%d Cout=%d H=%d W=%d priors %r (ops.gemm_psp_supported)"
+                         % (B, Cin, cout, H, W, [tuple(y.shape) for y in ys]))
+    xp = _packed_operand(x)
+    dev = xp.buf.device
+    out = torch.empty((B, cout, H, W), dtype=torch.float32, device=dev)
+    opk = PackedAct(_packed_buffer(B, cout, H, W, dev, avoid=xp.buf), (B, cout, H, W)) if packed else None
+    check(_lib.lib().gdm_conv1x1_psp_hip(xp.buf.data_ptr(), wpk.data_ptr(), ys[0].data_ptr(), sizes[0], ys[1].data_ptr(), sizes[1],
+                                         ys[2].data_ptr(), sizes[2], ys[3].data_ptr(), sizes[3],
+                                         bias.data_ptr() if bias is not None else None, B, Cin, cout, H, W, out.data_ptr(),
+                                         opk.buf.data_ptr() if opk is not None else None, _stream()), "gdm_conv1x1_psp_hip")
+    if opk is not None:
+        out._gdm_packed = opk
+    return out
 
 
 def gemm_pack_weight(weight2d):
diff --git a/geometric_aware_dense_matching_amd/settings.py b/geometric_aware_dense_matching_amd/settings.py
--- a/geometric_aware_dense_matching_amd/settings.py
+++ b/geometric_aware_dense_matching_amd/settings.py
@@ -31,6 +31,7 @@
 USE_POINTWISE_TRAIN = _flag("GDM_POINTWISE_TRAIN")
 USE_POINT_CHAIN = _flag("GDM_POINT_CHAIN")
 USE_PSP_JOBS = _flag("GDM_PSP_JOBS")
+USE_FUSED_GEMM_EPILOGUE = _flag("GDM_FUSED_GEMM_EPILOGUE")
 USE_PACKED_PRODUCERS = _flag("GDM_PACKED_PRODUCERS")
 USE_TWO_STREAM_PIPELINE = _flag("GDM_TWO_STREAM_PIPELINE")
 MESH_FORK_LATE = os.environ.get("GDM_MESH_FORK_LATE", "1") != "0"
@@ -42,6 +43,6 @@
 
 ALL_SWITCHES = ("USE_MFMA_CONV", "USE_MFMA_CONV_TRAIN", "USE_MFMA_GEMM", "USE_FUSED_UPCONV", "USE_LOWRES_UPCONV_TRAIN",
                 "USE_SPLIT_PSP_TRAIN", "USE_FUSED_LFA", "USE_GROUPED_SPLINE", "USE_FUSED_BN_TRAIN", "USE_FUSED_SYNCBN",
-                "USE_FUSED_MATCH_LOSS", "USE_SIDE_STREAMS", "USE_SPARSE_FINAL", "USE_FUSED_HEADS", "USE_MFMA_STRIDED", "USE_POINTWISE", "USE_OWN_STEM", "USE_GEMM_CONV1X1_TRAIN", "USE_MFMA_WGRAD", "USE_MFMA_GEMM_TRAIN", "USE_GATHERED_FINAL", "USE_DIRECT_WGRAD", "USE_PSP_JOBS", "USE_POINT_CHAIN", "USE_POINTWISE_TRAIN")
+                "USE_FUSED_MATCH_LOSS", "USE_SIDE_STREAMS", "USE_SPARSE_FINAL", "USE_FUSED_HEADS", "USE_MFMA_STRIDED", "USE_POINTWISE", "USE_OWN_STEM", "USE_GEMM_CONV1X1_TRAIN", "USE_MFMA_WGRAD", "USE_MFMA_GEMM_TRAIN", "USE_GATHERED_FINAL", "USE_DIRECT_WGRAD", "USE_PSP_JOBS", "USE_POINT_CHAIN", "USE_POINTWISE_TRAIN", "USE_FUSED_GEMM_EPILOGUE")
 SPLIT_BF16_SWITCHES = ("USE_MFMA_CONV", "USE_MFMA_GEMM", "USE_FUSED_UPCONV", "USE_SPARSE_FINAL", "USE_FUSED_HEADS", "USE_MFMA_STRIDED",
                        "USE_OWN_STEM")
diff --git a/include/gdm.h b/include/gdm.h
--- a/include/gdm.h
+++ b/include/gdm.h
@@ -203,6 +203,11 @@
                             int B, int Cin, int Cout, int H, int W, int stride, int act, float* out, void* outpk, void* stream);
 int gdm_conv1x1_strided_hip(const void* xpk, const void* wpk, const float* scale, const float* shift,
                             int B, int Cin, int Cout, int H, int W, int stride, int act, float* out, void* stream);
+int gdm_conv1x1_p2r_hip(const void* xpk, const void* wpk, const float* t, const int32_t* idx, const float* scale, const float* shift,
+                        int B, int Cin, int Cout, int H, int W, int n, int act, float slope, float* out, void* outpk, void* stream);
+int gdm_conv1x1_psp_hip(const void* xpk, const void* wpk, const float* y1, int s1, const float* y2, int s2, const float* y3, int s3,
+                        const float* y4, int s4, const float* bias, int B, int Cin, int Cout, int H, int W, float* out, void* outpk,
+                        void* stream);
 
 int gdm_affine_relu_maxpool_hip(const float* x, const float* scale, const float* shift, int B, int C, int H, int W, float* y, void* stream);
 int gdm_conv1x1_logsoftmax_hip(const float* x, const float* w, const float* bias, int B, int C, long hw, float* out, void* stream);
```

After: 5287, median of 6. +1.6%, better.
